# jiamiya/HOPE

Hardware: AMD Instinct MI355X
Metric: parallel env steps/sec (full CarParking step incl. obs + RS search) (higher is better)
Workload: dtype f64

## Files before the change

### hope_amd/_lib.py

```python
import ctypes as C
import os

from .build import lib_path

LIDAR_NUM, N_ACTION, N_ITER, UPSAMPLE, TARGET_DIM, RS_MAX_SEG = 120, 42, 10, 10, 5, 5
F_OBS_F64, F_ACTION_F64, F_PROFILE, F_IMAGE, F_OVERLAP = 0x1, 0x2, 0x4, 0x8, 0x10
STAGE_MOTION, STAGE_OBS, STAGE_REWARD, STAGE_RS, STAGE_ALL = 0x1, 0x2, 0x4, 0x8, 0xF
ACTION_PHYSICAL = 0x10
ACTION_RESCALE_F32 = 0x80
AUTO_REDRAW = 0x100
DEFER_RS = 0x200
STAGE_IMG = 0x40
STAGE_NO_CULL, STAGE_ONE_SCENE = 0x4000, 0x8000
IMG_SIZE, IMG_CHANNELS, TRAJ_RENDER_LEN = 64, 3, 20
AUTO_RESET = 0x20
KERNELS = ('k_kinematics', 'k_env_step', 'k_rs_words', 'k_rs_validate', 'k_bev_image', 'k_bev_prep', 'k_rs_compact', 'k_post', 'k_rs_segs', 'k_rs_screen')
ABI_VERSION = 8

EXPORTS = ['hope_env_create', 'hope_env_destroy', 'hope_last_error', 'hope_abi_version', 'hope_env_upload_tables',
           'hope_env_set_scenes', 'hope_env_step', 'hope_env_wait_rs', 'hope_env_last_step', 'hope_env_wait_rs_step', 'hope_env_download_n_obst', 'hope_env_queue_check', 'hope_env_reset_obs', 'hope_env_download_state',
           'hope_env_upload_state', 'hope_env_restart', 'hope_env_set_pool', 'hope_env_pool_staging', 'hope_env_commit_pool', 'hope_env_commit_pool_relaxed', 'hope_env_pool_staging_ready', 'hope_env_pool_generation', 'hope_env_redraw', 'hope_env_set_redraw_seed', 'hope_env_download_pool_index', 'hope_env_set_dlp_cases', 'hope_env_pool_overflow', 'hope_env_set_draw_class', 'hope_env_download_scenes', 'hope_env_download_pool_state', 'hope_env_restore_maps', 'hope_env_kernel_ms', 'hope_env_kernel_union_ms', 'hope_env_profile_kernels', 'hope_debug_math', 'hope_debug_traffic', 'hope_debug_mask_lut', 'hope_debug_rs_prof', 'hope_debug_rs_log', 'hope_debug_rs_filter_stats', 'hope_debug_rs_filter_dump', 'hope_debug_step_prof', 'hope_debug_census', 'hope_scenegen_generate', 'hope_scenegen_default_threads', 'hope_scenegen_generate_det', 'hope_scenegen_generate_device', 'hope_scenegen_log_det', 'hope_env_generate_pool', 'hope_env_curriculum_enable', 'hope_env_curriculum_disable', 'hope_env_set_pool_buckets', 'hope_env_curriculum_tally', 'hope_env_curriculum_update', 'hope_env_curriculum_state', 'hope_env_curriculum_set_windows', 'hope_env_curriculum_download_lists', 'hope_curriculum_lists_host', 'hope_curriculum_fold_host', 'hope_map_level_host', 'hope_map_level_device', 'hope_env_map_level', 'hope_env_num_scenes', 'hope_env_max_obstacles', 'hope_env_device_arch']


CURRICULUM_LIST_LEN = 1 << 20
BUCKET_UNLABELLED = 255


class HopeError(RuntimeError):
    pass


class StepOut(C.Structure):
    _fields_ = [('lidar', C.c_void_p), ('action_mask', C.c_void_p), ('target', C.c_void_p), ('reward', C.c_void_p),
                ('reward_info', C.c_void_p), ('status', C.c_void_p), ('done', C.c_void_p), ('pose', C.c_void_p),
                ('rs_word', C.c_void_p), ('rs_lengths', C.c_void_p), ('img', C.c_void_p)]


class CurriculumParams(C.Structure):
    _fields_ = [('target', C.c_double * 4), ('type_window', C.c_double), ('case_window', C.c_double), ('type_fail_min', C.c_double),
                ('case_fail_min', C.c_double), ('worst_share', C.c_double), ('case_uniform', C.c_double), ('type_horizon', C.c_int64),
                ('case_horizon', C.c_int64)]

    def __init__(self, target=(0.95, 0.95, 0.9, 0.99), type_window=250.0, case_window=10.0, type_fail_min=0.01, case_fail_min=0.005,
                 worst_share=0.5, case_uniform=0.2, type_horizon=200, case_horizon=500):
        super().__init__((C.c_double * 4)(*target), type_window, case_window, type_fail_min, case_fail_min, worst_share, case_uniform,
                         type_horizon, case_horizon)


_lib = None


def load_library():
    global _lib
    if _lib is not None:
        return _lib
    try:
        import torch
    except ImportError:
        pass
    path = lib_path()
    if not os.path.exists(path):
        raise HopeError(f'{path} is missing: run `python -c "import __graft_entry__ as g; g.build()"` '
                        '(hipcc --offload-arch=gfx950). There is no CPU fallback.')
    L = C.CDLL(path)
    for name in EXPORTS:
        if not hasattr(L, name):
            raise HopeError(f'{path} does not export {name}')
    L.hope_last_error.restype = C.c_char_p
    L.hope_env_device_arch.restype = C.c_char_p
    L.hope_env_device_arch.argtypes = [C.c_void_p]
    L.hope_env_create.argtypes = [C.POINTER(C.c_void_p), C.c_int, C.c_int, C.c_int, C.c_uint32]
    L.hope_env_destroy.argtypes = [C.c_void_p]
    L.hope_env_upload_tables.argtypes = [C.c_void_p, C.c_void_p, C.c_void_p, C.c_void_p]
    L.hope_env_set_scenes.argtypes = [C.c_void_p, C.c_void_p, C.c_int, C.c_void_p, C.c_void_p, C.c_void_p, C.c_void_p,
                                      C.c_void_p]
    L.hope_env_step.argtypes = [C.c_void_p, C.c_void_p, C.c_void_p, C.c_uint32, C.POINTER(StepOut), C.c_void_p]
    L.hope_env_wait_rs.argtypes = [C.c_void_p, C.c_void_p]
    L.hope_env_last_step.argtypes = [C.c_void_p, C.c_void_p]
    L.hope_env_wait_rs_step.argtypes = [C.c_void_p, C.c_uint64, C.c_void_p]
    L.hope_env_download_n_obst.argtypes = [C.c_void_p, C.c_void_p]
    L.hope_env_queue_check.argtypes = [C.c_void_p, C.c_void_p, C.c_void_p, C.c_void_p]
    L.hope_env_reset_obs.argtypes = [C.c_void_p, C.c_void_p, C.c_uint32, C.POINTER(StepOut), C.c_void_p]
    L.hope_env_download_state.argtypes = [C.c_void_p, C.c_void_p, C.c_void_p, C.c_void_p]
    L.hope_env_upload_state.argtypes = [C.c_void_p, C.c_void_p, C.c_void_p, C.c_void_p]
    L.hope_env_restart.argtypes = [C.c_void_p, C.c_void_p, C.c_void_p]
    L.hope_env_set_pool.argtypes = [C.c_void_p, C.c_int, C.c_void_p, C.c_void_p, C.c_void_p, C.c_void_p, C.c_void_p]
    L.hope_env_pool_staging.argtypes = [C.c_void_p, C.c_int] + [C.POINTER(C.c_void_p)] * 5
    L.hope_env_commit_pool.argtypes = [C.c_void_p, C.c_int, C.c_void_p]
    L.hope_env_commit_pool_relaxed.argtypes = [C.c_void_p, C.c_int]
    L.hope_env_redraw.argtypes = [C.c_void_p, C.c_void_p, C.c_uint64, C.c_void_p]
    L.hope_env_set_redraw_seed.argtypes = [C.c_void_p, C.c_uint64]
    L.hope_env_download_pool_index.argtypes = [C.c_void_p, C.c_void_p]
    L.hope_env_set_dlp_cases.argtypes = [C.c_void_p, C.c_int, C.c_void_p, C.c_void_p, C.c_void_p, C.c_void_p, C.c_int, C.c_void_p, C.c_void_p]
    L.hope_env_set_draw_class.argtypes = [C.c_void_p, C.c_void_p, C.c_int, C.c_void_p]
    L.hope_env_pool_overflow.argtypes = [C.c_void_p, C.c_void_p]
    L.hope_env_download_scenes.argtypes = [C.c_void_p, C.c_void_p, C.c_int, C.c_void_p, C.c_void_p, C.c_void_p, C.c_void_p, C.c_void_p]
    L.hope_env_download_pool_state.argtypes = [C.c_void_p, C.c_void_p, C.c_void_p]
    L.hope_env_restore_maps.argtypes = [C.c_void_p, C.c_void_p, C.c_void_p, C.c_uint64, C.c_uint64]
    L.hope_env_pool_staging_ready.argtypes = [C.c_void_p]
    L.hope_env_pool_generation.argtypes = [C.c_void_p, C.c_void_p]
    L.hope_env_kernel_ms.argtypes = [C.c_void_p, C.c_void_p, C.c_void_p, C.c_int]
    L.hope_env_kernel_union_ms.argtypes = [C.c_void_p, C.c_void_p, C.c_void_p, C.c_int]
    L.hope_env_profile_kernels.argtypes = [C.c_void_p, C.c_uint32]
    L.hope_debug_math.argtypes = [C.c_int, C.c_int, C.c_void_p, C.c_void_p, C.c_void_p, C.c_void_p]
    L.hope_debug_traffic.argtypes = [C.c_int, C.c_size_t, C.c_void_p, C.c_void_p]
    L.hope_debug_mask_lut.argtypes = [C.c_void_p, C.c_void_p, C.c_void_p, C.c_void_p]
    L.hope_scenegen_generate.argtypes = [C.c_int, C.c_int, C.c_int, C.c_uint64, C.c_int64, C.c_int, C.c_void_p, C.c_void_p, C.c_void_p,
                                         C.c_void_p, C.c_void_p, C.c_void_p, C.c_int]
    L.hope_scenegen_generate_det.argtypes = L.hope_scenegen_generate.argtypes
    L.hope_scenegen_generate_device.argtypes = [C.c_int, C.c_int, C.c_int, C.c_int, C.c_uint64, C.c_int64, C.c_int, C.c_void_p, C.c_void_p,
                                                C.c_void_p, C.c_void_p, C.c_void_p, C.c_void_p, C.c_void_p]
    L.hope_scenegen_log_det.argtypes = [C.c_int, C.c_void_p, C.c_void_p]
    L.hope_env_generate_pool.argtypes = [C.c_void_p, C.c_int, C.c_void_p, C.c_uint64, C.c_int64, C.c_int]
    L.hope_env_curriculum_enable.argtypes = [C.c_void_p, C.c_void_p]
    L.hope_env_curriculum_disable.argtypes = [C.c_void_p]
    L.hope_env_set_pool_buckets.argtypes = [C.c_void_p, C.c_int, C.c_void_p]
    L.hope_env_curriculum_tally.argtypes = [C.c_void_p, C.c_void_p, C.c_void_p, C.c_void_p]
    L.hope_env_curriculum_update.argtypes = [C.c_void_p, C.c_void_p]
    L.hope_env_curriculum_state.argtypes = [C.c_void_p] + [C.c_void_p] * 8
    L.hope_env_curriculum_set_windows.argtypes = [C.c_void_p, C.c_int] + [C.c_void_p] * 4
    L.hope_env_curriculum_download_lists.argtypes = [C.c_void_p, C.c_void_p, C.c_void_p, C.c_void_p]
    L.hope_curriculum_lists_host.argtypes = [C.c_void_p, C.c_int, C.c_void_p, C.c_void_p, C.c_int, C.c_int] + [C.c_void_p] * 8
    L.hope_curriculum_fold_host.argtypes = [C.c_void_p, C.c_void_p, C.c_double, C.c_double, C.c_double]
    L.hope_map_level_host.argtypes = [C.c_int, C.c_int] + [C.c_void_p] * 6 + [C.c_int]
    L.hope_map_level_device.argtypes = [C.c_int, C.c_int, C.c_int] + [C.c_void_p] * 7
    L.hope_env_map_level.argtypes = [C.c_void_p] * 5
    L.hope_env_num_scenes.argtypes = [C.c_void_p]
    L.hope_env_max_obstacles.argtypes = [C.c_void_p]
    if L.hope_abi_version() != ABI_VERSION:
        raise HopeError(f'ABI mismatch: library {L.hope_abi_version()} vs binding {ABI_VERSION}')
    _lib = L
    return L


def check(rc, what=''):
    if rc != 0:
        msg = load_library().hope_last_error().decode(errors='replace')
        raise HopeError(f'{what} failed (code {rc}): {msg}')
```

### hope_amd/csrc/hope_env.hip

```cpp
#include <hip/hip_runtime.h>
#include <math.h>
#include <stdio.h>
#include <stdlib.h>
#include <string.h>

#include <algorithm>
#include <chrono>
#include <string>
#include <vector>

#include "hope_dev.h"
#include "hope_env.h"
#include "hope_internal.h"
#include "hope_step_kernel.h"
#include "hope_obs_pair.h"
#include "hope_motion_pair.h"
#include "hope_scenegen_kernel.h"
#include "hope_curriculum_kernel.h"
#include "hope_maplevel_kernel.h"

using namespace hope;

static thread_local std::string g_err;
static int fail(int code, const std::string& msg) {
// ... 481 lines not shown
    return HOPE_OK;
}
static int settle_rs(hope_env_t* h) {
    if (!h || !h->rs_pending) return HOPE_OK;
    DeviceGuard guard(h->device);
    HIPCHK(hipEventSynchronize(h->ev_chain1_done));
    HIPCHK(hipEventSynchronize(h->ev_search0_done));
    h->rs_pending = false;
    return HOPE_OK;
}

const char* hope_last_error(void) { return g_err.c_str(); }
int hope_abi_version(void) { return HOPE_ABI_VERSION; }

static int destroy_impl(hope_env_t* h);
static void cur_free(hope_env_t* h);
int hope_env_create(hope_env_t** out, int n_scenes, int max_obstacles, int device_id, uint32_t flags) {
    if (!out || n_scenes <= 0 || max_obstacles <= 0) return fail(HOPE_EINVAL, "hope_env_create: bad argument");
    if (flags & 0x20)
        return fail(HOPE_EINVAL, "hope_env_create: flag 0x20 (hipGraph replay of the step, ABI <= 6) was removed in ABI 7: it was slower than plain launches at every batch size");
    *out = nullptr;
    int ndev = 0;
    hipError_t e = hipGetDeviceCount(&ndev);
    if (e != hipSuccess || ndev <= 0)
        return fail(HOPE_ENODEV, std::string("hope_env_create: no HIP device (") + hipGetErrorString(e) +
                                     "); libhope_env has no CPU fallback");
    if (device_id < 0 || device_id >= ndev) return fail(HOPE_EINVAL, "hope_env_create: device_id out of range");
    HIPCHK(hipSetDevice(device_id));
    hipDeviceProp_t prop;
    HIPCHK(hipGetDeviceProperties(&prop, device_id));
    size_t lds = step_lds_bytes(max_obstacles);
    size_t lds_rs = rs_lds_bytes(max_obstacles);
    if (max_obstacles > HOPE_MAX_OBSTACLES)
        return fail(HOPE_EINVAL, "hope_env_create: max_obstacles " + std::to_string(max_obstacles) + " exceeds HOPE_MAX_OBSTACLES (" +
                                 std::to_string(HOPE_MAX_OBSTACLES) + "): the Reeds-Shepp queue entry carries the obstacle count in 8 bits");
    if (lds > 160 * 1024 || lds_rs > 160 * 1024)
        return fail(HOPE_EINVAL, "hope_env_create: max_obstacles " + std::to_string(max_obstacles) + " does not fit the 160 KiB LDS tile of the step / search kernels");
    if (n_scenes >= RS_LIST_MAX_SCENES)
        return fail(HOPE_EINVAL, "hope_env_create: more than 2^24 - 1 scenes per handle");
    hope_env* h = new (std::nothrow) hope_env();
    if (!h) return fail(HOPE_ENOMEM, "hope_env_create: host allocation failed");
    h->n = n_scenes; h->max_obst = max_obstacles; h->device = device_id; h->flags = flags;
    h->n_obst_host.assign(n_scenes, 0);
    h->slot_cls_host.assign(n_scenes, 0);
    snprintf(h->arch, sizeof(h->arch), "%s", prop.gcnArchName);
    size_t N = (size_t)n_scenes;
#define ALLOC(ptr, bytes)                                                                          \
    do {                                                                                           \
        hipError_t e2 = hipMalloc((void**)&(ptr), (bytes));                                        \
        if (e2 != hipSuccess) {                                                                    \
            destroy_impl(h);                                                                       \
            return fail(HOPE_ENOMEM, std::string("hipMalloc " #ptr ": ") + hipGetErrorString(e2)); \
        }                                                                                          \
    } while (0)
    ALLOC(h->verts, N * max_obstacles * 8 * sizeof(double));
    ALLOC(h->obb, N * max_obstacles * sizeof(float4));
    ALLOC(h->fverts, N * max_obstacles * 2 * sizeof(float4));
    ALLOC(h->fbox, N * max_obstacles * sizeof(float4));
    ALLOC(h->eflag, N * (size_t)eflag_stride(max_obstacles));
    ALLOC(h->n_obst, N * sizeof(int32_t));
    ALLOC(h->scene_c, N * SC_WORDS * sizeof(double));
    ALLOC(h->state, N * ST_WORDS * sizeof(double));
    ALLOC(h->cs, N * 2 * sizeof(double));
    ALLOC(h->tstep, N * sizeof(int32_t));
    ALLOC(h->tab, (size_t)NL * NITER * NACT * sizeof(double));
    ALLOC(h->pmax, NL * sizeof(double));
    ALLOC(h->mask_lut, MASK_LUT_BYTES);
    ALLOC(h->mask_bsc, NBEAM * sizeof(double));
    ALLOC(h->hull_base, NBEAM * sizeof(double));
    ALLOC(h->beam_ab, 2 * NBEAM * sizeof(double));
    ALLOC(h->rs_count, 2 * hope_env::MAX_CHAIN * sizeof(int32_t));
    ALLOC(h->rs_list, 2 * N * sizeof(int32_t));
    ALLOC(h->rs_in, 2 * N * RS_IN_WORDS * sizeof(double));
    ALLOC(h->rs_flag, N);
    ALLOC(h->kin, N * KIN_WORDS * sizeof(double));
    ALLOC(h->post, N * POST_WORDS * sizeof(double));
    ALLOC(h->cls_list[0], N * sizeof(int32_t));
    ALLOC(h->cls_list[1], N * sizeof(int32_t));
    ALLOC(h->rs_rec, N * rs_rec_bytes_per_scene());
    ALLOC(h->rs_surv_count, hope_env::MAX_CHAIN * sizeof(int32_t));
    ALLOC(h->rs_surv, 2 * N * sizeof(int2));
    ALLOC(h->cur_pool, N * sizeof(int32_t));
    ALLOC(h->episode, N * sizeof(uint32_t));
    ALLOC(h->pool_overflow, sizeof(int32_t));
    ALLOC(h->slot_cls, N);
    ALLOC(h->active_snap, N);
    ALLOC(h->cold_dev, hope_env::COLD_RING * sizeof(StepCold));
    if (flags & HOPE_F_IMAGE) {
        ALLOC(h->traj, N * BEV_TRAJ_LEN * 3 * sizeof(double));
        ALLOC(h->traj_len, N * sizeof(int32_t));
        ALLOC(h->traj_valid, N * sizeof(int32_t));
        ALLOC(h->layer_valid, N * sizeof(int32_t));
        ALLOC(h->bev_layer, N * (size_t)BEV_LAYER_ROWS * BEV_LAYER_STRIDE);
        ALLOC(h->bev_dyn, N * BEV_DYN_BYTES);
        ALLOC(h->bev_list, (N + 1) * sizeof(int32_t));
        ALLOC(h->bev_legacy, (N + 1) * sizeof(int32_t));
        ALLOC(h->bev_scratch, N * BEV_SCENE_INTS * sizeof(int));
    }
#undef ALLOC
    if (h->traj) {
        HIPCHK(hipMemset(h->traj, 0, N * BEV_TRAJ_LEN * 3 * sizeof(double)));
        HIPCHK(hipMemset(h->traj_len, 0, N * sizeof(int32_t)));
        HIPCHK(hipMemset(h->traj_valid, 0, N * sizeof(int32_t)));
        HIPCHK(hipMemset(h->layer_valid, 0, N * sizeof(int32_t)));
        HIPCHK(hipMemset(h->bev_dyn, 0, N * BEV_DYN_BYTES));
        HIPCHK(hipMemset(h->bev_list, 0, (N + 1) * sizeof(int32_t)));
        HIPCHK(hipMemset(h->bev_legacy, 0, (N + 1) * sizeof(int32_t)));
        HIPCHK(hipMemset(h->bev_scratch, 0, N * BEV_SCENE_INTS * sizeof(int)));
    }
    HIPCHK(hipMemset(h->n_obst, 0, N * sizeof(int32_t)));
    HIPCHK(hipMemset(h->scene_c, 0, N * SC_WORDS * sizeof(double)));
    HIPCHK(hipMemset(h->state, 0, N * ST_WORDS * sizeof(double)));
    HIPCHK(hipMemset(h->tstep, 0, N * sizeof(int32_t)));
    HIPCHK(hipMemset(h->rs_count, 0, 2 * hope_env::MAX_CHAIN * sizeof(int32_t)));
    HIPCHK(hipMemset(h->rs_flag, 0, N));
    HIPCHK(hipMemset(h->rs_surv_count, 0, hope_env::MAX_CHAIN * sizeof(int32_t)));
    HIPCHK(hipMemset(h->rs_surv, 0, 2 * N * sizeof(int2)));
    HIPCHK(hipMemset(h->rs_in, 0, 2 * N * RS_IN_WORDS * sizeof(double)));
    HIPCHK(hipMemset(h->rs_list, 0, 2 * N * sizeof(int32_t)));
    HIPCHK(hipMemset(h->cur_pool, 0xFF, N * sizeof(int32_t)));
    HIPCHK(hipMemset(h->episode, 0, N * sizeof(uint32_t)));
    HIPCHK(hipMemset(h->pool_overflow, 0, sizeof(int32_t)));
    HIPCHK(hipMemset(h->slot_cls, 0, N));
    HIPCHK(hipMemset(h->active_snap, 1, N));
    HIPCHK(hipHostMalloc((void**)&h->cold_host, hope_env::COLD_RING * sizeof(StepCold)));
    for (int i = 0; i < hope_env::COLD_RING; i++) HIPCHK(hipEventCreateWithFlags(&h->cold_ev[i], hipEventDisableTiming));
    memset(&h->cold_last, 0, sizeof(h->cold_last));
    HIPCHK(rs_init_tables());
    if (lds > 48 * 1024) {
        for (const void* f : {(const void*)k_env_step<float, float>, (const void*)k_env_step<float, float, true>,
                              (const void*)k_env_step<float, double>, (const void*)k_env_step<double, float>,
                              (const void*)k_env_step<double, double>,
                              (const void*)k_env_step<float, float, false, 0, true>, (const void*)k_env_step<float, double, false, 0, true>,
                              (const void*)k_env_step<double, float, false, 0, true>, (const void*)k_env_step<double, double, false, 0, true>,
                              (const void*)k_env_step<float, float, false, 1>, (const void*)k_env_step<float, double, false, 1>,
                              (const void*)k_env_step<double, float, false, 1>, (const void*)k_env_step<double, double, false, 1>,
                              (const void*)k_env_step<float, float, false, 2>, (const void*)k_env_step<float, double, false, 2>,
                              (const void*)k_env_step<double, float, false, 2>, (const void*)k_env_step<double, double, false, 2>})
            HIPCHK(hipFuncSetAttribute(f, hipFuncAttributeMaxDynamicSharedMemorySize, (int)lds));
    }
    if (flags & HOPE_F_OVERLAP) {
        HIPCHK(hipEventCreateWithFlags(&h->ev_fork, hipEventDisableTiming));
        HIPCHK(hipEventCreateWithFlags(&h->ev_collect, hipEventDisableTiming));
        for (int i = 0; i < 2; i++) HIPCHK(hipEventCreateWithFlags(&h->ev_bev[i], hipEventDisableTiming));
        for (int i = 0; i < 2; i++) { HIPCHK(hipEventCreateWithFlags(&h->ev_step[i], hipEventDisableTiming)); HIPCHK(hipEventCreateWithFlags(&h->ev_segs[i], hipEventDisableTiming)); HIPCHK(hipEventCreateWithFlags(&h->ev_post[i], hipEventDisableTiming)); }
        for (hipEvent_t* e : {&h->ev_chain1_done, &h->ev_image_done, &h->ev_obs_done[0], &h->ev_obs_done[1], &h->ev_search0_done})
            HIPCHK(hipEventCreateWithFlags(e, hipEventDisableTiming));
        static const int perm_plain[N_ROLES] = {0, 1, 6, 3, 2, 5, 4, 7}, perm_image[N_ROLES] = {0, 6, 2, 3, 1, 4, 5, 7};
        int perm[N_ROLES];
        for (int r = 0; r < N_ROLES; r++) perm[r] = (flags & HOPE_F_IMAGE) ? perm_image[r] : perm_plain[r];
        hipStream_t created[N_ROLES] = {};
        for (int c = 1; c < N_ROLES; c++) HIPCHK(hipStreamCreateWithPriority(&created[c], hipStreamNonBlocking, 0));
        int cls[N_ROLES];
        for (int c = 0; c < N_ROLES; c++) cls[c] = -1;
        {
            const auto t_begin = std::chrono::steady_clock::now();
            const long long ticks = 10000;
            long long* stamps = nullptr;
            if (hipHostMalloc((void**)&stamps, 4 * sizeof(long long), hipHostMallocDefault) != hipSuccess) stamps = nullptr;
            bool ok = stamps != nullptr;
            auto pair_overlaps = [&](hipStream_t a, hipStream_t b) -> int {
                for (int rep_ = 0; rep_ < 3; rep_++) {
                    hipStreamSynchronize(a); hipStreamSynchronize(b);
                    hipLaunchKernelGGL(k_spin, dim3(1), dim3(64), 0, a, ticks, stamps);
                    hipLaunchKernelGGL(k_spin, dim3(1), dim3(64), 0, b, ticks, stamps + 2);
                    if (hipStreamSynchronize(a) != hipSuccess || hipStreamSynchronize(b) != hipSuccess) return -1;
                    const long long lo = std::max(stamps[0], stamps[2]), hi = std::min(stamps[1], stamps[3]);
                    if (hi - lo > ticks / 4) return 1;
                    if (std::max(stamps[1], stamps[3]) - std::min(stamps[0], stamps[2]) > 20 * ticks) return -1;
                }
                return 0;
            };
            hipLaunchKernelGGL(k_spin, dim3(1), dim3(64), 0, created[1], 100LL, (long long*)nullptr);
            hipStreamSynchronize(created[1]);
            int rep[N_ROLES], n_cls = 0;
            for (int c = 0; c < N_ROLES && ok; c++) {
                int found = -1;
                for (int k = 0; k < n_cls && found < 0 && ok; k++) {
                    const int ov = pair_overlaps(created[rep[k]], created[c]);
                    if (ov < 0) ok = false;
                    else if (ov == 0) found = k;
                }
                if (found < 0) { rep[n_cls] = c; found = n_cls++; }
                cls[c] = found;
            }
            if (stamps) hipHostFree(stamps);
            HIPCHK(hipGetLastError());
            h->queue_check_ms = std::chrono::duration<double, std::milli>(std::chrono::steady_clock::now() - t_begin).count();
            if (!ok) { for (int c = 0; c < N_ROLES; c++) cls[c] = -1; n_cls = 0; }
            h->n_queues = n_cls;
            if (n_cls >= 2 && !(flags & HOPE_F_IMAGE)) {
                static const int order[N_ROLES - 1] = {ROLE_SEARCH0, ROLE_CHAIN, ROLE_OBS_LARGE, ROLE_OBS_SMALL, ROLE_OBS_SUB, ROLE_IMAGE, ROLE_SPARE};
                static const int conflicts[N_ROLES][4] = {
                     {-1, -1, -1, -1},
                     {ROLE_CALLER, ROLE_SEARCH0, -1, -1},
                     {-1, -1, -1, -1},
                     {ROLE_CALLER, ROLE_SEARCH0, ROLE_CHAIN, -1},
                     {ROLE_CALLER, ROLE_CHAIN, ROLE_OBS_LARGE, -1},
                     {ROLE_CALLER, -1, -1, -1},
                     {-1, -1, -1, -1},
                     {ROLE_SEARCH0, ROLE_CHAIN, ROLE_OBS_LARGE, -1}};
                int newperm[N_ROLES] = {0, 0, 0, 0, 0, 0, 0, 0};
                bool taken[N_ROLES] = {};
                for (const int r : order) {
                    int best = -1, best_cost = 1 << 30;
                    for (int c = 1; c < N_ROLES; c++) {
                        if (taken[c]) continue;
                        int cost = 0;
                        for (const int o : conflicts[r]) {
                            if (o < 0) continue;
                            const int oc = o == ROLE_CALLER ? cls[0] : (newperm[o] ? cls[newperm[o]] : -2);
                            if (oc == cls[c]) cost += 4;
                        }
                        if (c != perm[r]) cost += 1;
                        if (cost < best_cost) { best_cost = cost; best = c; }
                    }
                    newperm[r] = best; taken[best] = true;
                }
                for (int r = 1; r < N_ROLES; r++) perm[r] = newperm[r];
            }
        }
        for (int r = 1; r < N_ROLES; r++) h->side[r] = created[perm[r]];
        h->queue_of_role[ROLE_CALLER] = cls[0];
        for (int r = 1; r < N_ROLES; r++) h->queue_of_role[r] = cls[perm[r]];
    }
    HIPCHK(hipDeviceSynchronize());
    { std::lock_guard<std::mutex> lk(g_live_m); g_live.insert(h); }
    *out = h;
    return HOPE_OK;
}

int hope_env_destroy(hope_env_t* h) {
    if (!h) return HOPE_OK;
    {
        std::lock_guard<std::mutex> lk(g_live_m);
        if (g_live.erase(h) == 0) return fail(HOPE_EINVAL, "hope_env_destroy: not a live handle (destroyed twice?)");
    }
    return destroy_impl(h);
}
static int destroy_impl(hope_env_t* h) {
    settle_rs(h);
    DeviceGuard guard(h->device);
    drain_events(h);
    hipDeviceSynchronize();
    for (hipEvent_t e : {h->ev_collect, h->ev_bev[0], h->ev_bev[1], h->ev_fork, h->ev_step[0], h->ev_step[1], h->ev_segs[0], h->ev_segs[1], h->ev_post[0], h->ev_post[1],
                         h->ev_chain1_done, h->ev_image_done, h->ev_obs_done[0], h->ev_obs_done[1], h->ev_search0_done}) if (e) hipEventDestroy(e);
    for (hipStream_t q : h->side) if (q) hipStreamDestroy(q);
    if (h->pool_stream) hipStreamDestroy(h->pool_stream);
    for (hipEvent_t e : h->cold_ev) if (e) hipEventDestroy(e);
    if (h->cold_host) hipHostFree(h->cold_host);
    for (hipEvent_t e : {h->ev_pool_ready, h->ev_pool_copied, h->ev_last_step}) if (e) hipEventDestroy(e);
    for (void* q : {(void*)h->pstage.start, (void*)h->pstage.dest, (void*)h->pstage.bbox, (void*)h->pstage.verts, (void*)h->pstage.nobst, (void*)h->pstage.list}) if (q) hipHostFree(q);
    for (int i = 0; i < 2; i++) { if (h->gen_nobst[i]) hipHostFree(h->gen_nobst[i]); if (h->ev_gen_copied[i]) hipEventDestroy(h->ev_gen_copied[i]); }
    for (hipEvent_t e : h->free_events) hipEventDestroy(e);
    cur_free(h);
    for (auto& ps : h->pset) for (void* q : {(void*)ps.label, (void*)ps.sorted_own[0], (void*)ps.sorted_own[1]}) if (q) hipFree(q);
    void* ptrs[] = {h->obb, h->fverts, h->fbox, h->eflag, h->verts, h->n_obst, h->scene_c, h->state, h->cs, h->tstep, h->tab, h->pmax, h->mask_lut, h->mask_bsc,
                    h->hull_base, h->beam_ab, h->rs_count, h->rs_surv_count, h->rs_surv, h->rs_list, h->rs_in, h->rs_flag, h->kin, h->post, h->cls_list[0], h->cls_list[1], h->rs_rec, h->cur_pool, h->episode, h->pset[0].verts, h->pset[0].c, h->pset[0].nobst, h->pset[0].list[0], h->pset[0].list[1], h->pset[1].verts, h->pset[1].c, h->pset[1].nobst, h->pset[1].list[0], h->pset[1].list[1], h->pstage_dev, h->pool_overflow, h->slot_cls, h->active_snap, h->cold_dev, h->dlp_mem[0], h->dlp_mem[1], h->dlp_mem[2], h->dlp_mem[3], h->dlp_mem[4], h->dlp_mem[5], h->stage, h->traj, h->traj_len, h->traj_valid, h->layer_valid, h->bev_layer, h->bev_dyn, h->bev_list, h->bev_legacy, h->bev_scratch};
    for (void* q : ptrs)
        if (q) hipFree(q);
    delete h;
    return HOPE_OK;
}

int hope_debug_step_prof(uint64_t* out, int reset) {
    static unsigned long long buf[64 * 16];
    hipError_t e = hipDeviceSynchronize();
    if (e == hipSuccess) e = hipMemcpyFromSymbol(buf, HIP_SYMBOL(g_step_prof), sizeof(buf));
    for (int i = 0; i < 16; i++) { out[i] = 0; for (int sh = 0; sh < 64; sh++) out[i] += buf[sh * 16 + i]; }
    if (e == hipSuccess && reset) {
        for (auto& v : buf) v = 0;
        e = hipMemcpyToSymbol(HIP_SYMBOL(g_step_prof), buf, sizeof(buf));
    }
    return e == hipSuccess ? HOPE_OK : fail(HOPE_EHIP, std::string("hope_debug_step_prof: ") + hipGetErrorString(e));
}

int hope_debug_census(uint64_t* out, int reset) {
    static unsigned long long buf[64 * 16];
    if (!out) return fail(HOPE_EINVAL, "hope_debug_census: null argument");
    hipError_t e = hipDeviceSynchronize();
    if (e == hipSuccess) e = hipMemcpyFromSymbol(buf, HIP_SYMBOL(g_census), sizeof(buf));
    for (int i = 0; i < 16; i++) {
        const bool is_min = i == 1 || i == 3 || i == 7;
        out[i] = is_min ? ~0ull : 0;
        for (int sh = 0; sh < 64; sh++) out[i] = is_min ? std::min<uint64_t>(out[i], buf[sh * 16 + i]) : out[i] + buf[sh * 16 + i];
    }
    if (e == hipSuccess && reset) {
        for (int sh = 0; sh < 64; sh++) for (int i = 0; i < 16; i++) buf[sh * 16 + i] = (i == 1 || i == 3 || i == 7) ? 0x7ff0000000000000ull : 0;
        e = hipMemcpyToSymbol(HIP_SYMBOL(g_census), buf, sizeof(buf));
    }
    return e == hipSuccess ? HOPE_OK : fail(HOPE_EHIP, std::string("hope_debug_census: ") + hipGetErrorString(e));
}

int hope_debug_rs_prof(uint64_t* out, int reset) {
    hipError_t e = rs_prof_read((unsigned long long*)out, reset);
    return e == hipSuccess ? HOPE_OK : fail(HOPE_EHIP, std::string("hope_debug_rs_prof: ") + hipGetErrorString(e));
}

int hope_debug_rs_filter_stats(uint64_t* out, int reset) {
    if (!out) return fail(HOPE_EINVAL, "hope_debug_rs_filter_stats: null argument");
    hipError_t e = rs_fstat_read((unsigned long long*)out, reset);
    return e == hipSuccess ? HOPE_OK : fail(HOPE_EHIP, std::string("hope_debug_rs_filter_stats: ") + hipGetErrorString(e));
}

int hope_debug_rs_filter_dump(double* out) {
    if (!out) return fail(HOPE_EINVAL, "hope_debug_rs_filter_dump: null argument");
    hipError_t e = rs_fdump_read(out);
    return e == hipSuccess ? HOPE_OK : fail(HOPE_EHIP, std::string("hope_debug_rs_filter_dump: ") + hipGetErrorString(e));
}

int hope_debug_rs_log(int32_t* out, int cap, int32_t* n, int reset) {
    if (!out || !n || cap < 0) return fail(HOPE_EINVAL, "hope_debug_rs_log: bad argument");
    hipError_t e = rs_log_read(out, cap, n, reset);
    return e == hipSuccess ? HOPE_OK : fail(HOPE_EHIP, std::string("hope_debug_rs_log: ") + hipGetErrorString(e));
}

int hope_env_queue_check(hope_env_t* h, int32_t* queue_of_role, int32_t* n_queues, double* ms) {
    if (!h) return fail(HOPE_EINVAL, "hope_env_queue_check: null handle");
    if (queue_of_role) for (int r = 0; r < N_ROLES; r++) queue_of_role[r] = h->queue_of_role[r];
    if (n_queues) *n_queues = h->n_queues;
    if (ms) *ms = h->queue_check_ms;
    return HOPE_OK;
}

int hope_env_num_scenes(const hope_env_t* h) { return h ? h->n : HOPE_EINVAL; }
int hope_env_max_obstacles(const hope_env_t* h) { return h ? h->max_obst : HOPE_EINVAL; }
const char* hope_env_device_arch(const hope_env_t* h) { return h ? h->arch : ""; }

static void build_mask_lut(const std::vector<double>& tab, const std::vector<double>& pmax, const double* hull_base,
                           std::vector<uint16_t>& lut, std::vector<double>& bsc) {
    lut.assign((size_t)MASK_LUT_ROWS * MASK_LUT_ROW, (uint16_t)0xAAAA);
    bsc.assign(NBEAM, 0.0);
    for (int i = 0; i < NBEAM; i++) {
        const int l = UPS * i;
        const double lo = hull_base[i] - 1e-6;
        const double scale = (double)MASK_LUT_NB / (pmax[l] + 4e-9 - lo);
        bsc[i] = scale;
        for (int b = 0; b < MASK_LUT_NB; b++) {
            const double e_lo = lo + ((double)b - 1e-6) / scale - 2e-9, e_hi = lo + ((double)b + 1.0 + 1e-6) / scale + 2e-9;
            uint16_t* row = lut.data() + ((size_t)i * MASK_LUT_NB + b) * MASK_LUT_ROW;
            for (int hl = 0; hl < NACT / 2; hl++) {
                int c[2][2];
                for (int d = 0; d < 2; d++) {
                    const int a = hl + d * (NACT / 2);
                    int cl = 0, ch = 0;
                    for (int k = 0; k < NITER; k++) {
                        const double t = tab[((size_t)l * NITER + k) * NACT + a];
                        cl += t <= e_lo; ch += t <= e_hi;
                    }
                    c[d][0] = cl; c[d][1] = ch;
                }
                row[hl] = (uint16_t)(c[0][0] | c[0][1] << 4 | c[1][0] << 8 | c[1][1] << 12);
            }
        }
    }
}

static void build_mask_tab(const double* dist_star, std::vector<double>& tab, std::vector<double>& pmax) {
    tab.assign((size_t)NL * NITER * NACT, 0.0);
    pmax.assign(NL, 0.0);
    for (int l = 0; l < NL; l++) {
        double pm = -INFINITY;
        for (int a = 0; a < NACT; a++) {
            double run = -INFINITY;
            for (int k = 0; k < NITER; k++) {
                double v = dist_star[((size_t)l * NACT + a) * NITER + k];
                run = v > run ? v : run;
                tab[((size_t)l * NITER + k) * NACT + a] = run;
            }
            pm = run > pm ? run : pm;
        }
        pmax[l] = pm;
    }
}

int hope_debug_mask_lut(const double* dist_star, const double* hull_base, uint16_t* lut_out, double* scale_out) {
    if (!dist_star || !hull_base || !lut_out || !scale_out) return fail(HOPE_EINVAL, "hope_debug_mask_lut: null argument");
    std::vector<double> tab, pmax, bsc;
    std::vector<uint16_t> lut;
    build_mask_tab(dist_star, tab, pmax);
    build_mask_lut(tab, pmax, hull_base, lut, bsc);
    memcpy(lut_out, lut.data(), MASK_LUT_BYTES);
    memcpy(scale_out, bsc.data(), NBEAM * sizeof(double));
    return HOPE_OK;
}

int hope_env_upload_tables(hope_env_t* h, const double* dist_star, const double* hull_base, const double* beam_ab) {
    if (!h || !dist_star || !hull_base || !beam_ab) return fail(HOPE_EINVAL, "hope_env_upload_tables: null argument");
    DeviceGuard guard(h->device);
    if (!guard.ok) return fail(HOPE_EHIP, "hipSetDevice failed");
    std::vector<double> tab, pmax;
    build_mask_tab(dist_star, tab, pmax);
    HIPCHK(hipMemcpy(h->tab, tab.data(), tab.size() * sizeof(double), hipMemcpyHostToDevice));
    HIPCHK(hipMemcpy(h->pmax, pmax.data(), pmax.size() * sizeof(double), hipMemcpyHostToDevice));
    {
        std::vector<uint16_t> lut;
        std::vector<double> bsc;
        build_mask_lut(tab, pmax, hull_base, lut, bsc);
        HIPCHK(hipMemcpy(h->mask_lut, lut.data(), MASK_LUT_BYTES, hipMemcpyHostToDevice));
        HIPCHK(hipMemcpy(h->mask_bsc, bsc.data(), NBEAM * sizeof(double), hipMemcpyHostToDevice));
    }
    HIPCHK(hipMemcpy(h->hull_base, hull_base, NBEAM * sizeof(double), hipMemcpyHostToDevice));
    HIPCHK(hipMemcpy(h->beam_ab, beam_ab, 2 * NBEAM * sizeof(double), hipMemcpyHostToDevice));
    h->have_tables = true;
    return HOPE_OK;
}

static int upload_scenes(hope_env_t* h, const int32_t* ids, int n, const double* start, const double* dest, const double* bbox,
                         const double* verts, const int32_t* n_obst, double* d_scene_c, double* d_state, int32_t* d_t,
                         int32_t* d_nobst, double* d_verts, float4* d_obb, double* d_traj, int32_t* d_traj_len, int32_t* d_traj_valid,
                         int32_t* d_layer_valid);
static int apply_pending_pool(hope_env_t* h, bool wait);
static int cur_on_swap(hope_env_t* h);

static int rebuild_class_lists(hope_env_t* h) {
    std::vector<int32_t> l0, l1;
    l0.reserve(h->n); l1.reserve(h->n);
    const bool two = h->max_obst > SMALL_TILE;
    for (int i = 0; i < h->n; i++) (two && h->slot_cls_host[i] ? l1 : l0).push_back(i);
    if (two && (h->flags & HOPE_F_OVERLAP)) {
        const char* fr = getenv("HOPE_CLS1_FRAC");
        const double frac = fr ? atof(fr) : (h->n < 32768 ? 0.42 : 0.0);
        const size_t want1 = (size_t)(frac * h->n);
        if (l1.size() < want1) {
            const size_t move = std::min(l0.size(), want1 - l1.size());
            l1.insert(l1.end(), l0.end() - move, l0.end());
            l0.resize(l0.size() - move);
            std::sort(l1.begin(), l1.end());
        }
    }
    h->cls_count[0] = (int)l0.size(); h->cls_count[1] = (int)l1.size();
    if (!l0.empty()) HIPCHK(hipMemcpy(h->cls_list[0], l0.data(), l0.size() * sizeof(int32_t), hipMemcpyHostToDevice));
    if (!l1.empty()) HIPCHK(hipMemcpy(h->cls_list[1], l1.data(), l1.size() * sizeof(int32_t), hipMemcpyHostToDevice));
    HIPCHK(hipMemcpy(h->slot_cls, h->slot_cls_host.data(), (size_t)h->n, hipMemcpyHostToDevice));
    return HOPE_OK;
}

int hope_env_set_scenes(hope_env_t* h, const int32_t* scene_ids, int n, const double* start, const double* dest,
                        const double* bbox, const double* verts, const int32_t* n_obst) {
    { int rcs = settle_rs(h); if (rcs != HOPE_OK) return rcs; }
    if (!h || n < 0 || (n > 0 && (!scene_ids || !start || !dest || !bbox || !n_obst)))
        return fail(HOPE_EINVAL, "hope_env_set_scenes: null argument");
    if (n == 0) return HOPE_OK;
    for (int k = 0; k < n; k++) {
        if (scene_ids[k] < 0 || scene_ids[k] >= h->n) return fail(HOPE_EINVAL, "hope_env_set_scenes: scene id out of range");
        if (n_obst[k] < 0 || n_obst[k] > h->max_obst) return fail(HOPE_EINVAL, "hope_env_set_scenes: n_obst exceeds max_obstacles");
        if (n_obst[k] > 0 && !verts) return fail(HOPE_EINVAL, "hope_env_set_scenes: verts is null");
    }
    DeviceGuard guard(h->device);
    if (!guard.ok) return fail(HOPE_EHIP, "hipSetDevice failed");
    {
        int rc = upload_scenes(h, scene_ids, n, start, dest, bbox, verts, n_obst, h->scene_c, h->state, h->tstep, h->n_obst,
                               h->verts, h->obb, h->traj, h->traj_len, h->traj_valid, h->layer_valid);
        if (rc != HOPE_OK) return rc;
    }
    for (int k = 0; k < n; k++) {
        h->n_obst_host[scene_ids[k]] = n_obst[k];
        h->slot_cls_host[scene_ids[k]] = (h->max_obst > SMALL_TILE && n_obst[k] > SMALL_TILE) ? 1 : 0;
    }
    { int rc = rebuild_class_lists(h); if (rc != HOPE_OK) return rc; }
    if (h->cur.on) {
        hipLaunchKernelGGL(k_curriculum_forget, dim3((n + 255) / 256), dim3(256), 0, 0, n, (const int32_t*)h->stage, h->cur.scene_bucket,
                           h->episode, h->cur.noted_ep);
        HIPCHK(hipGetLastError());
    }
    HIPCHK(hipDeviceSynchronize());
    h->have_scenes = true;
    return HOPE_OK;
}

static void draw_lists(const hope_env_t* h, const int32_t** lists, int* counts) {
    for (int c = 0; c < 2; c++) {
        const bool weighted = h->cur.on && h->cur.wactive >= 0 && h->pool_cls_n[c] > 0;
        lists[c] = weighted ? h->cur.wl[h->cur.wactive][c] : h->pool_cls[c];
        counts[c] = weighted ? CW_LIST_LEN : h->pool_cls_n[c];
    }
}
static int sync_cold(hope_env_t* h, hipStream_t s) {
    StepCold c;
    memset(&c, 0, sizeof(c));
    c.traj = h->traj; c.traj_len = h->traj_len; c.traj_valid = h->traj_valid; c.layer_valid = h->layer_valid;
    c.pool_verts = h->pool_verts; c.pool_c = h->pool_c; c.pool_nobst = h->pool_nobst;
    draw_lists(h, c.pool_cls, c.pool_cls_n);
    c.cur_pool = h->cur_pool; c.episode = h->episode; c.redraw_seed = h->redraw_seed;
    c.dlp = h->dlp; c.pool_overflow = h->pool_overflow; c.slot_cls = h->slot_cls;
    c.fverts = h->fverts; c.fbox = h->fbox; c.eflag = h->eflag;
    if (h->cold_idx >= 0 && memcmp(&c, &h->cold_last, sizeof(c)) == 0) return HOPE_OK;
    const int slot = (h->cold_idx + 1) % hope_env::COLD_RING;
    HIPCHK(hipEventSynchronize(h->cold_ev[slot]));
    memcpy(&h->cold_host[slot], &c, sizeof(c));
    HIPCHK(hipMemcpyAsync(h->cold_dev + slot, h->cold_host + slot, sizeof(c), hipMemcpyHostToDevice, s));
    HIPCHK(hipEventRecord(h->cold_ev[slot], s));
    h->cold_idx = slot;
    memcpy(&h->cold_last, &c, sizeof(c));
    return HOPE_OK;
}

constexpr int SPLIT_MIN_SCENES = 16384;
constexpr int SPLIT_MIN_SCENES_DEFER = 32768;
constexpr int FUSE_KIN_MAX_SCENES = 4096;
constexpr int AUTO_SUBS_RANGE[4] = {32768, 1 << 30, 4096, 32768};

enum MotionKernel { MOTION_ONE_LAUNCH, MOTION_FUSED_KIN, MOTION_TIMING, MOTION_SPLIT, MOTION_PAIR };
enum ObsKernel { OBS_IN_STEP, OBS_SPLIT, OBS_PAIR };

struct StepPlan {
    struct Chain {
        int c, a, b;
        int tile_cap;
        Role search, kin, obs;
        bool on_caller;
        bool post_on_search;
        MotionKernel motion;
        ObsKernel obs_kernel;
    } chain[hope_env::MAX_CHAIN];
    int n_chain;
    bool want_rs;
    bool fork;
    bool split;
    bool pipe;
    bool pipe1;
    bool fuse_kin;
    bool auto_subs;
};

static StepPlan plan_step(const hope_env_t* h, uint32_t stages, bool want_rs, bool overlap, int has_action, bool step_timing) {
    StepPlan pl = {};
    pl.want_rs = want_rs;
    const int n_cls = h->max_obst > SMALL_TILE ? 2 : 1;
    const bool obs = stages & HOPE_STAGE_OBS, defer_rs = stages & HOPE_DEFER_RS, img = stages & HOPE_STAGE_IMG;
    int subs = 1;
    if (overlap && want_rs && obs && defer_rs && !img && (h->cls_count[0] == 0) != (h->cls_count[1] == 0)) {
        int range[4] = {AUTO_SUBS_RANGE[0], AUTO_SUBS_RANGE[1], AUTO_SUBS_RANGE[2], AUTO_SUBS_RANGE[3]};
        if (const char* e = getenv("HOPE_AUTO_CHAINS")) sscanf(e, "%d:%d:%d:%d", range, range + 1, range + 2, range + 3);
        const int c1 = h->cls_count[0] == 0 ? 1 : 0, cnt = h->cls_count[c1];
        if (cnt >= range[2 * c1] && cnt <= range[2 * c1 + 1]) { subs = 2; pl.auto_subs = true; }
    }
    for (int c = n_cls - 1; c >= 0; c--)
        for (int j = 0; j < subs; j++) {
            const int a = (int)((long long)h->cls_count[c] * j / subs), b = (int)((long long)h->cls_count[c] * (j + 1) / subs);
            if (b > a) {
                StepPlan::Chain& ch = pl.chain[pl.n_chain++];
                ch.c = c; ch.a = a; ch.b = b;
                ch.tile_cap = (c == 0 && n_cls == 2) ? SMALL_TILE : h->max_obst;
            }
        }
    pl.fork = overlap && pl.n_chain == 2;
    const bool two_stream_forms = pl.fork && want_rs && obs && !step_timing;
    const char* split_min = getenv("HOPE_SPLIT_MIN");
    pl.split = two_stream_forms && h->n >= (split_min ? atoi(split_min) : defer_rs ? SPLIT_MIN_SCENES_DEFER : SPLIT_MIN_SCENES);
    pl.pipe = two_stream_forms && defer_rs;
    pl.pipe1 = pl.pipe && !pl.split;
    pl.fuse_kin = h->n <= FUSE_KIN_MAX_SCENES && !pl.split && !step_timing;
    const bool of64 = h->flags & HOPE_F_OBS_F64, af64 = h->flags & HOPE_F_ACTION_F64;
    for (int i = 0; i < pl.n_chain; i++) {
        StepPlan::Chain& ch = pl.chain[i];
        ch.search = (pl.fork && i == 1) ? ROLE_CHAIN : pl.pipe ? ROLE_SEARCH0 : ROLE_CALLER;
        ch.on_caller = pl.pipe && !pl.auto_subs && !img && h->cls_count[ch.c] >= h->cls_count[1 - ch.c];
        ch.obs = !(pl.split || pl.pipe1) ? ch.search : ch.on_caller ? ROLE_CALLER : (pl.auto_subs && i == 1) ? ROLE_OBS_SUB : (Role)(ROLE_OBS_LARGE + i);
        ch.kin = pl.pipe ? ch.obs : ch.search;
        ch.post_on_search = pl.pipe && pl.split;
        const bool one_scene = stages & STAGE_ONE_SCENE;
        if (pl.split) ch.motion = (ch.c == 0 && n_cls == 2 && (stages & HOPE_STAGE_MOTION) && has_action && !one_scene) ? MOTION_PAIR : MOTION_SPLIT;
        else if (step_timing && !of64 && !af64) ch.motion = MOTION_TIMING;
        else ch.motion = pl.fuse_kin ? MOTION_FUSED_KIN : MOTION_ONE_LAUNCH;
        ch.obs_kernel = !pl.split ? OBS_IN_STEP : (ch.tile_cap == SMALL_TILE && !one_scene) ? OBS_PAIR : OBS_SPLIT;
    }
    return pl;
}

static int enqueue_step(hope_env_t* h, const void* actions, const uint8_t* active, uint32_t stages, const hope_step_out* out,
                        hipStream_t s, bool overlap, int has_action, LaunchTimer* tm) {
    StepParams p;
    memset(&p, 0, sizeof(p));
    p.n = h->n; p.max_obst = h->max_obst; p.stages = stages; p.has_action = has_action;
    p.hflags = h->traj ? STEP_HF_TRAJ : 0;
    p.verts = h->verts; p.obb = h->obb; p.eflag = h->eflag; p.n_obst = h->n_obst; p.scene_c = h->scene_c; p.state = h->state; p.cs = h->cs; p.tstep = h->tstep;
    p.active = active; p.active_out = active ? h->active_snap : nullptr; p.kin = h->kin; p.actions = actions; p.post = h->post;
    p.tab = h->tab; p.pmax = h->pmax; p.mask_lut = h->mask_lut; p.mask_bsc = h->mask_bsc; p.hull_base = h->hull_base; p.beam_ab = h->beam_ab;
    p.lidar = out->lidar; p.action_mask = out->action_mask;
    p.cold = h->cold_dev + h->cold_idx;
    const uint8_t* active_rs = active ? h->active_snap : nullptr;
    const bool of64 = h->flags & HOPE_F_OBS_F64, af64 = h->flags & HOPE_F_ACTION_F64;
    const dim3 block(WAVE);
    static const bool step_timing = getenv("HOPE_STEP_TIMING") != nullptr;
    const bool want_rs = (stages & HOPE_STAGE_RS) && out->rs_word;
    const StepPlan pl = plan_step(h, stages, want_rs, overlap, has_action, step_timing);
    auto stream = [&](Role r) { return r == ROLE_CALLER ? s : h->side[r]; };

    if (!pl.pipe) { int rcj = join_rs(h, s); if (rcj != HOPE_OK) return rcj; }
    if (want_rs) h->rs_parity ^= 1;
    if (pl.fork) {
        HIPCHK(hipEventRecord(h->ev_fork, s));
        HIPCHK(hipStreamWaitEvent(h->side[ROLE_CHAIN], h->ev_fork, 0));
        if (pl.pipe) HIPCHK(hipStreamWaitEvent(h->side[ROLE_SEARCH0], h->ev_fork, 0));
    }
    h->last_via_steps = false;
    for (int i = 0; i < pl.n_chain; i++) {
        const StepPlan::Chain& ch = pl.chain[i];
        const int c = ch.c;
        const hipStream_t sc = stream(ch.search), sk = stream(ch.kin), so = stream(ch.obs);
        int32_t* counter = h->rs_count + i + hope_env::MAX_CHAIN * h->rs_parity;
        if (pl.pipe && !ch.on_caller) HIPCHK(hipStreamWaitEvent(sk, h->ev_fork, 0));
        p.tile_cap = ch.tile_cap;
        p.scene_list = h->cls_list[c] + ch.a;
        p.n_list = ch.b - ch.a;
        p.rs_count_zero = want_rs ? counter : nullptr;
        if ((stages & HOPE_STAGE_MOTION) && has_action && !pl.fuse_kin) {
            dim3 kg((p.n_list + KIN_SCENES_PER_BLOCK - 1) / KIN_SCENES_PER_BLOCK);
            if (tm) tm->begin(HOPE_K_KINEMATICS, sk);
            if (af64) hipLaunchKernelGGL((k_kinematics<double>), kg, block, 0, sk, p.n_list, p.scene_list, h->state, actions, active, stages, h->scene_c, h->kin);
            else hipLaunchKernelGGL((k_kinematics<float>), kg, block, 0, sk, p.n_list, p.scene_list, h->state, actions, active, stages, h->scene_c, h->kin);
            if (tm) tm->end(sk);
        }
        const dim3 grid(p.n_list);
        const size_t lds = step_lds_bytes(p.tile_cap);
        if (pl.pipe) HIPCHK(hipStreamWaitEvent(sk, h->ev_segs[i], 0));
        if (tm) tm->begin(HOPE_K_STEP, sk);
        switch (ch.motion) {
        case MOTION_PAIR: hipLaunchKernelGGL(k_motion_pair, dim3((p.n_list + 1) / 2), block, MP_LDS_BYTES, sk, p); break;
        case MOTION_SPLIT: launch_env_step<1>(of64, af64, grid, block, lds, sk, p); break;
        case MOTION_TIMING: hipLaunchKernelGGL((k_env_step<float, float, true>), grid, block, lds, sk, p); break;
        case MOTION_FUSED_KIN: launch_env_step<0, true>(of64, af64, grid, block, lds, sk, p); break;
        case MOTION_ONE_LAUNCH: launch_env_step<0>(of64, af64, grid, block, lds, sk, p); break;
        }
        if (tm) tm->end(sk);
        if (pl.fork && (pl.split || pl.pipe || (stages & HOPE_STAGE_IMG))) { HIPCHK(hipEventRecord(h->ev_step[i], sk)); h->last_via_steps = true; }
        if (pl.split && !pl.pipe) HIPCHK(hipStreamWaitEvent(so, h->ev_step[i], 0));
        auto launch_post = [&](hipStream_t sp) {
            dim3 pg((p.n_list + WAVE - 1) / WAVE);
            if (tm) tm->begin(HOPE_K_POST, sp);
            if (of64) hipLaunchKernelGGL((k_post<double>), pg, block, 0, sp, p.n_list, p.scene_list, active, stages, h->scene_c, h->state, h->post, h->rs_flag, *out);
            else hipLaunchKernelGGL((k_post<float>), pg, block, 0, sp, p.n_list, p.scene_list, active, stages, h->scene_c, h->state, h->post, h->rs_flag, *out);
            if (tm) tm->end(sp);
        };
        if (!pl.split) launch_post(so);
        else {
            if (tm) tm->begin(HOPE_K_STEP, so);
            if (ch.obs_kernel == OBS_PAIR) {
                if (of64) hipLaunchKernelGGL((k_obs_pair<double>), dim3((p.n_list + 1) / 2), block, OP_LDS_BYTES, so, p);
                else hipLaunchKernelGGL((k_obs_pair<float>), dim3((p.n_list + 1) / 2), block, OP_LDS_BYTES, so, p);
            } else launch_env_step<2>(of64, af64, grid, block, lds, so, p);
            if (tm) tm->end(so);
            if (!ch.post_on_search) launch_post(so);
        }
        if ((pl.split || pl.pipe1) && !ch.on_caller) HIPCHK(hipEventRecord(h->ev_obs_done[i], so));
        if (!want_rs) continue;
        if (pl.pipe) HIPCHK(hipStreamWaitEvent(sc, h->ev_step[i], 0));
        if (ch.post_on_search) {
            launch_post(sc);
            HIPCHK(hipEventRecord(h->ev_post[i], sc));
        }
        int32_t* qlist = h->rs_list + (size_t)c * h->n + ch.a;
        double* rs_in = h->rs_in + ((size_t)c * h->n + ch.a) * RS_IN_WORDS;
        if (tm) tm->begin(HOPE_K_RS_COMPACT, sc);
        {
            const dim3 cg((p.n_list + COMPACT_THREADS - 1) / COMPACT_THREADS);
            if (of64) hipLaunchKernelGGL(k_rs_compact<double>, cg, dim3(COMPACT_THREADS), 0, sc, p.scene_list, p.n_list, h->rs_flag, active_rs, qlist,
                                         counter, (const double*)h->post, (const double*)h->scene_c, out->rs_word, out->rs_lengths, (const int32_t*)h->n_obst, h->rs_surv_count + i, rs_in);
            else hipLaunchKernelGGL(k_rs_compact<float>, cg, dim3(COMPACT_THREADS), 0, sc, p.scene_list, p.n_list, h->rs_flag, active_rs, qlist,
                                    counter, (const double*)h->post, (const double*)h->scene_c, out->rs_word, out->rs_lengths, (const int32_t*)h->n_obst, h->rs_surv_count + i, rs_in);
        }
        if (tm) tm->end(sc);
        if (pl.pipe) HIPCHK(hipEventRecord(h->ev_segs[i], sc));
        RsParams r;
        r.n = h->n; r.max_obst = h->max_obst; r.obs_f64 = of64;
        r.prio_front = 0;
        r.tile_cap = p.tile_cap;
        r.max_queue = p.n_list;
        r.slot_base = (c == 0) ? ch.a : h->n - 1 - ch.a;
        r.slot_dir = (c == 0) ? 1 : -1;
        r.verts = h->verts; r.obb = h->obb; r.n_obst = h->n_obst; r.scene_c = h->scene_c; r.state = h->state;
        r.fverts = h->fverts; r.fbox = h->fbox; r.eflag = h->eflag;
        r.rs_count = counter; r.rs_list = qlist; r.rs_in = rs_in;
        r.rs_rec = h->rs_rec;
        r.surv_count = h->rs_surv_count + i;
        r.surv_list = h->rs_surv + (size_t)c * h->n + ch.a;
        r.rs_word = out->rs_word; r.rs_lengths = out->rs_lengths;
        HIPCHK(launch_rs_search(r, sc, tm));
    }
    HIPCHK(hipGetLastError());
    if (stages & HOPE_STAGE_IMG) {
        BevParams b;
        b.n = h->n; b.max_obst = h->max_obst; b.verts = h->verts; b.n_obst = h->n_obst; b.scene_c = h->scene_c;
        b.state = h->state; b.traj = h->traj; b.traj_len = h->traj_len; b.traj_valid = h->traj_valid; b.scratch = h->bev_scratch; b.img = out->img;
        b.layer = h->bev_layer; b.layer_valid = h->layer_valid; b.rebuild = h->bev_list; b.dyn = h->bev_dyn;
        b.legacy_list = h->bev_legacy;
        b.active = active;
        b.debug = 0;
        if (const char* e_ = getenv("HOPE_BEV_DEBUG")) b.debug |= atoi(e_);
        if (getenv("HOPE_BEV_LEGACY")) b.debug |= 32;
        if (pl.fork) {
            const hipStream_t si = pl.pipe ? s : h->side[ROLE_IMAGE];
            HIPCHK(hipStreamWaitEvent(si, h->ev_step[0], 0));
            HIPCHK(hipStreamWaitEvent(si, h->ev_step[1], 0));
            if (pl.pipe) HIPCHK(launch_bev_image(b, si, tm, h->side[ROLE_IMAGE], h->ev_bev[0], h->ev_bev[1]));
            else HIPCHK(launch_bev_image(b, si, tm));
            HIPCHK(hipEventRecord(h->ev_image_done, si));
        } else HIPCHK(launch_bev_image(b, s, tm));
    }
    if (!pl.fork) return HOPE_OK;
    HIPCHK(hipEventRecord(h->ev_chain1_done, h->side[ROLE_CHAIN]));
    if (pl.pipe) {
        HIPCHK(hipEventRecord(h->ev_search0_done, h->side[ROLE_SEARCH0]));
        h->rs_pending = true;
    } else HIPCHK(hipStreamWaitEvent(s, h->ev_chain1_done, 0));
    if (stages & HOPE_STAGE_IMG) HIPCHK(hipStreamWaitEvent(s, h->ev_image_done, 0));
    if (pl.split || pl.pipe1) {
        const StepPlan::Chain* ch = pl.chain;
        if (ch[0].on_caller != ch[1].on_caller) {
            const hipStream_t so = stream(ch[ch[0].on_caller ? 1 : 0].obs);
            for (int i = 0; i < 2; i++) if (ch[i].post_on_search) HIPCHK(hipStreamWaitEvent(so, h->ev_post[i], 0));
            HIPCHK(hipEventRecord(h->ev_collect, so));
            HIPCHK(hipStreamWaitEvent(s, h->ev_collect, 0));
        } else for (int i = 0; i < 2; i++) {
            if (!ch[i].on_caller) HIPCHK(hipStreamWaitEvent(s, h->ev_obs_done[i], 0));
            if (ch[i].post_on_search) HIPCHK(hipStreamWaitEvent(s, h->ev_post[i], 0));
        }
    }
    return HOPE_OK;
}

static int check_pool_classes(hope_env_t* h, const char* who) {
    bool resident[2] = {false, false};
    for (int i = 0; i < h->n; i++) resident[h->slot_cls_host[i] ? 1 : 0] = true;
    for (int c = 0; c < 2; c++)
        if (resident[c] && h->pool_cls_n[c] == 0)
            return fail(HOPE_ESTATE, std::string(who) + ": scene slots of the " + (c ? "large" : "small (<= 32 obstacles)") +
                                     " size class are resident but the pool holds no map of that size class (a slot draws from its own class: "
                                     "hope_env_set_pool / hope_env_set_dlp_cases / hope_env_set_draw_class)");
    return HOPE_OK;
}

static int launch_step(hope_env_t* h, const void* actions, const uint8_t* active, uint32_t stages,
                       const hope_step_out* out, void* stream, int has_action) {
    if (!h || !out) return fail(HOPE_EINVAL, "hope_env_step: null argument");
    if (!is_live(h)) return fail(HOPE_EINVAL, "hope_env_step: not a live handle (destroyed?)");
    if (!h->have_tables) return fail(HOPE_ESTATE, "hope_env_step: hope_env_upload_tables has not been called");
    if (!h->have_scenes) return fail(HOPE_ESTATE, "hope_env_step: hope_env_set_scenes has not been called");
    if (has_action && !actions) return fail(HOPE_EINVAL, "hope_env_step: actions is null");
    if (stages & HOPE_STAGE_RS) stages |= HOPE_STAGE_REWARD;
    if (stages & HOPE_AUTO_REDRAW) {
        if (!(stages & HOPE_AUTO_RESET)) return fail(HOPE_EINVAL, "hope_env_step: HOPE_AUTO_REDRAW needs HOPE_AUTO_RESET");
        if (h->pool_n <= 0 && h->dlp.n_cases <= 0) return fail(HOPE_ESTATE, "hope_env_step: HOPE_AUTO_REDRAW without a scene pool (hope_env_set_pool / hope_env_set_dlp_cases)");
        int rc0 = check_pool_classes(h, "hope_env_step");
        if (rc0 != HOPE_OK) return rc0;
    }
    if (stages & HOPE_STAGE_IMG) {
        if (!h->traj) return fail(HOPE_ESTATE, "hope_env_step: HOPE_STAGE_IMG needs a handle created with HOPE_F_IMAGE");
        if (!out->img) return fail(HOPE_EINVAL, "hope_env_step: HOPE_STAGE_IMG without out->img");
    }
    DeviceGuard guard(h->device);
    if (!guard.ok) return fail(HOPE_EHIP, "hipSetDevice failed");
    hipStream_t s = (hipStream_t)stream;
    const bool prof = h->flags & HOPE_F_PROFILE;
    h->step_seq++;
    { int rcp = apply_pending_pool(h, false); if (rcp != HOPE_OK) return rcp; }
    if (h->pool_wait_pending) {
        HIPCHK(hipStreamWaitEvent(s, h->ev_pool_ready, 0));
        h->pool_wait_pending = false;
    }
    { int rcc = sync_cold(h, s); if (rcc != HOPE_OK) return rcc; }
    h->draw_set = h->pactive;
    struct LastStep {
        hope_env_t* h; hipStream_t s;
        ~LastStep() { if (h->pactive >= 0 && h->ev_last_step && !h->last_via_steps) hipEventRecord(h->ev_last_step, s); }
    } last_step{h, s};
    if (prof && h->pending.size() > 4096) { int rc = drain_events(h); if (rc) return rc; }
    EventTimer timer(h);
    LaunchTimer* tm = prof ? &timer : nullptr;
    int rc = enqueue_step(h, actions, active, stages, out, s, (h->flags & HOPE_F_OVERLAP) != 0, has_action, tm);
    if (rc != HOPE_OK) return rc;
    if (timer.failed) return fail(HOPE_EHIP, "hipEventRecord failed");
    return HOPE_OK;
}


static int upload_scenes(hope_env_t* h, const int32_t* ids, int n, const double* start, const double* dest, const double* bbox,
                         const double* verts, const int32_t* n_obst, double* d_scene_c, double* d_state, int32_t* d_t,
                         int32_t* d_nobst, double* d_verts, float4* d_obb, double* d_traj, int32_t* d_traj_len, int32_t* d_traj_valid,
                         int32_t* d_layer_valid) {
    size_t tile = (size_t)h->max_obst * 8 * sizeof(double);
    size_t o_ids = 0, o_nob = o_ids + sizeof(int32_t) * n, o_start = (o_nob + sizeof(int32_t) * n + 15) & ~(size_t)15;
    size_t o_dest = o_start + 24 * (size_t)n, o_bbox = o_dest + 24 * (size_t)n, o_verts = (o_bbox + 32 * (size_t)n + 15) & ~(size_t)15;
    size_t need = o_verts + tile * n;
    if (need > h->stage_bytes) {
        if (h->stage) hipFree(h->stage);
        h->stage = nullptr; h->stage_bytes = 0;
        hipError_t e2 = hipMalloc(&h->stage, need);
        if (e2 != hipSuccess) return fail(HOPE_ENOMEM, std::string("hipMalloc stage: ") + hipGetErrorString(e2));
        h->stage_bytes = need;
    }
    char* sp = (char*)h->stage;
    HIPCHK(hipMemcpy(sp + o_ids, ids, sizeof(int32_t) * n, hipMemcpyHostToDevice));
    HIPCHK(hipMemcpy(sp + o_nob, n_obst, sizeof(int32_t) * n, hipMemcpyHostToDevice));
    HIPCHK(hipMemcpy(sp + o_start, start, 24 * (size_t)n, hipMemcpyHostToDevice));
    HIPCHK(hipMemcpy(sp + o_dest, dest, 24 * (size_t)n, hipMemcpyHostToDevice));
    HIPCHK(hipMemcpy(sp + o_bbox, bbox, 32 * (size_t)n, hipMemcpyHostToDevice));
    if (verts) HIPCHK(hipMemcpy(sp + o_verts, verts, tile * n, hipMemcpyHostToDevice));
    hipLaunchKernelGGL(k_set_scene_consts, dim3((n + 127) / 128), dim3(128), 0, 0, n, (const int32_t*)(sp + o_ids),
                       (const double*)(sp + o_start), (const double*)(sp + o_dest), (const double*)(sp + o_bbox),
                       (const int32_t*)(sp + o_nob), d_scene_c, d_state, d_t, d_nobst, d_traj, d_traj_len, d_traj_valid, d_layer_valid);
    if (verts)
        hipLaunchKernelGGL(k_set_scene_tiles, dim3(n), dim3(128), 0, 0, (const int32_t*)(sp + o_ids),
                           (const int32_t*)(sp + o_nob), (const double*)(sp + o_verts), (const double*)(sp + o_bbox), d_verts, d_obb,
                           h->fverts, h->fbox, h->eflag, h->max_obst);
    HIPCHK(hipGetLastError());
    HIPCHK(hipDeviceSynchronize());
    return HOPE_OK;
}

static uint64_t hmix64(uint64_t z) {
    z += 0x9E3779B97F4A7C15ull;
    z = (z ^ (z >> 30)) * 0xBF58476D1CE4E5B9ull;
    z = (z ^ (z >> 27)) * 0x94D049BB133111EBull;
    return z ^ (z >> 31);
}
static uint64_t fold64(uint64_t a, uint64_t b) { return hmix64(a ^ hmix64(b + 0x9E3779B97F4A7C15ull)); }
static uint64_t hash_bytes(uint64_t hsh, const void* p, size_t bytes) {
    const unsigned char* q = (const unsigned char*)p;
    size_t i = 0;
    for (; i + 8 <= bytes; i += 8) { uint64_t w; memcpy(&w, q + i, 8); hsh = (hsh ^ w) * 0x100000001B3ull; hsh ^= hsh >> 29; }
    uint64_t w = 0;
    if (i < bytes) { memcpy(&w, q + i, bytes - i); hsh = (hsh ^ w) * 0x100000001B3ull; }
    return fold64(hsh, bytes);
}
static void bump_pool_generation(hope_env_t* h, uint64_t content) {
    h->pool_generation = fold64(h->pool_generation, content);
    if (h->pool_generation == 0) h->pool_generation = 1;
}

static int pool_init_streams(hope_env_t* h) {
    if (h->pool_stream) return HOPE_OK;
    HIPCHK(hipStreamCreateWithFlags(&h->pool_stream, hipStreamNonBlocking));
    HIPCHK(hipEventCreateWithFlags(&h->ev_pool_ready, hipEventDisableTiming));
    HIPCHK(hipEventCreateWithFlags(&h->ev_pool_copied, hipEventDisableTiming));
    HIPCHK(hipEventCreateWithFlags(&h->ev_last_step, hipEventDisableTiming));
    return HOPE_OK;
}

static void build_pool_lists(hope_env_t* h, const int32_t* n_obst, int n_pool, std::vector<int32_t>& l0, std::vector<int32_t>& l1) {
    const bool two = h->max_obst > SMALL_TILE;
    for (int k = 0; k < n_pool; k++) (two && n_obst[k] > SMALL_TILE ? l1 : l0).push_back(k);
    for (int c = 0; c < h->dlp.n_cases; c++) (two ? l1 : l0).push_back(-2 - c);
}

static int pool_set_reserve(hope_env_t* h, hope_env::PoolSet& ps, int n_pool, int n_list) {
    if (n_pool > ps.cap) {
        for (void* q : {(void*)ps.verts, (void*)ps.c, (void*)ps.nobst, (void*)ps.label}) if (q) hipFree(q);
        ps.verts = ps.c = nullptr; ps.nobst = nullptr; ps.label = nullptr; ps.cap = 0;
        const size_t P = (size_t)n_pool;
        hipError_t e_ = hipMalloc((void**)&ps.verts, P * h->max_obst * 8 * sizeof(double));
        if (e_ == hipSuccess) e_ = hipMalloc((void**)&ps.c, P * SC_WORDS * sizeof(double));
        if (e_ == hipSuccess) e_ = hipMalloc((void**)&ps.nobst, P * sizeof(int32_t));
        if (e_ == hipSuccess) e_ = hipMalloc((void**)&ps.label, P);
        if (e_ != hipSuccess) return fail(HOPE_ENOMEM, std::string("hipMalloc pool: ") + hipGetErrorString(e_));
        ps.cap = n_pool;
    }
    if (n_list > ps.list_cap) {
        for (int c = 0; c < 2; c++) { if (ps.list[c]) hipFree(ps.list[c]); ps.list[c] = nullptr; }
        for (int c = 0; c < 2; c++) {
            hipError_t e_ = hipMalloc((void**)&ps.list[c], (size_t)n_list * sizeof(int32_t));
            if (e_ != hipSuccess) return fail(HOPE_ENOMEM, std::string("hipMalloc pool lists: ") + hipGetErrorString(e_));
        }
        ps.list_cap = n_list;
    }
    return HOPE_OK;
}

int hope_env_pool_staging(hope_env_t* h, int n_pool, double** start, double** dest, double** bbox, double** verts, int32_t** n_obst) {
    if (!h || n_pool <= 0 || !start || !dest || !bbox || !verts || !n_obst) return fail(HOPE_EINVAL, "hope_env_pool_staging: bad argument");
    DeviceGuard guard(h->device);
    if (!guard.ok) return fail(HOPE_EHIP, "hipSetDevice failed");
    int rc = pool_init_streams(h);
    if (rc != HOPE_OK) return rc;
    if (h->pstage.busy) { HIPCHK(hipEventSynchronize(h->ev_pool_copied)); h->pstage.busy = false; }
    if (n_pool > h->pstage.cap) {
        for (void* q : {(void*)h->pstage.start, (void*)h->pstage.dest, (void*)h->pstage.bbox, (void*)h->pstage.verts, (void*)h->pstage.nobst, (void*)h->pstage.list})
            if (q) hipHostFree(q);
        h->pstage = hope_env::PoolStage{};
        const size_t P = (size_t)n_pool;
        hipError_t e_ = hipHostMalloc((void**)&h->pstage.start, P * 24);
        if (e_ == hipSuccess) e_ = hipHostMalloc((void**)&h->pstage.dest, P * 24);
        if (e_ == hipSuccess) e_ = hipHostMalloc((void**)&h->pstage.bbox, P * 32);
        if (e_ == hipSuccess) e_ = hipHostMalloc((void**)&h->pstage.verts, P * h->max_obst * 8 * sizeof(double));
        if (e_ == hipSuccess) e_ = hipHostMalloc((void**)&h->pstage.nobst, P * sizeof(int32_t));
        if (e_ == hipSuccess) e_ = hipHostMalloc((void**)&h->pstage.list, (P + 4096) * sizeof(int32_t));
        if (e_ != hipSuccess) return fail(HOPE_ENOMEM, std::string("hipHostMalloc pool staging: ") + hipGetErrorString(e_));
        h->pstage.cap = n_pool;
    }
    h->pstage.staged = true;
    *start = h->pstage.start; *dest = h->pstage.dest; *bbox = h->pstage.bbox; *verts = h->pstage.verts; *n_obst = h->pstage.nobst;
    return HOPE_OK;
}

int hope_env_pool_staging_ready(hope_env_t* h) {
    if (!h) return fail(HOPE_EINVAL, "hope_env_pool_staging_ready: null handle");
    if (!h->pstage.busy) return 1;
    DeviceGuard guard(h->device);
    if (!guard.ok) return fail(HOPE_EHIP, "hipSetDevice failed");
    const hipError_t e = hipEventQuery(h->ev_pool_copied);
    if (e == hipSuccess) { h->pstage.busy = false; return 1; }
    if (e == hipErrorNotReady) return 0;
    return fail(HOPE_EHIP, std::string("hipEventQuery: ") + hipGetErrorString(e));
}

static int effective_generation(hope_env_t* h, uint64_t* generation);
int hope_env_pool_generation(hope_env_t* h, uint64_t* generation) {
    if (!h || !generation) return fail(HOPE_EINVAL, "hope_env_pool_generation: null argument");
    { DeviceGuard guard(h->device); int rcp = apply_pending_pool(h, true); if (rcp != HOPE_OK) return rcp; }
    return effective_generation(h, generation);
}

static int settle_gen_nobst(hope_env_t* h) {
    const int g = h->gen_host_set;
    if (g < 0) return HOPE_OK;
    HIPCHK(hipEventSynchronize(h->ev_gen_copied[g]));
    h->pool_nobst_host.assign(h->gen_nobst[g], h->gen_nobst[g] + h->gen_nobst_n[g]);
    h->gen_host_set = -1;
    return HOPE_OK;
}

static int apply_pending_pool(hope_env_t* h, bool wait) {
    if (!h->pend.on) return HOPE_OK;
    if (wait) HIPCHK(hipEventSynchronize(h->ev_pool_ready));
    else {
        const hipError_t e = hipEventQuery(h->ev_pool_ready);
        if (e == hipErrorNotReady) return HOPE_OK;
        if (e != hipSuccess) return fail(HOPE_EHIP, std::string("hipEventQuery: ") + hipGetErrorString(e));
    }
    hope_env::PoolSet& ps = h->pset[h->pend.set];
    h->pool_verts = ps.verts; h->pool_c = ps.c; h->pool_nobst = ps.nobst;
    h->pool_cls[0] = ps.list[0]; h->pool_cls[1] = ps.list[1];
    h->pool_cls_n[0] = h->pend.cls_n[0]; h->pool_cls_n[1] = h->pend.cls_n[1];
    h->pool_n = h->pend.n_pool;
    h->pool_nobst_host.swap(h->pend.nobst_host);
    h->pactive = h->pend.set;
    h->pend.on = false;
    bump_pool_generation(h, h->pend.content);
    h->gen_host_set = h->pend.generated ? h->pend.set : -1;
    return cur_on_swap(h);
}

static int commit_pool_impl(hope_env_t* h, int n_pool, bool relaxed);
int hope_env_commit_pool(hope_env_t* h, int n_pool, void* stream) { (void)stream; return commit_pool_impl(h, n_pool, false); }
int hope_env_commit_pool_relaxed(hope_env_t* h, int n_pool) { return commit_pool_impl(h, n_pool, true); }

static int commit_pool_impl(hope_env_t* h, int n_pool, bool relaxed) {
    if (!h || n_pool <= 0) return fail(HOPE_EINVAL, "hope_env_commit_pool: bad argument");
    if (n_pool > h->pstage.cap) return fail(HOPE_ESTATE, "hope_env_commit_pool: more entries than hope_env_pool_staging provided");
    for (int k = 0; k < n_pool; k++)
        if (h->pstage.nobst[k] < 0 || h->pstage.nobst[k] > h->max_obst) return fail(HOPE_EINVAL, "hope_env_commit_pool: n_obst exceeds max_obstacles");
    DeviceGuard guard(h->device);
    if (!guard.ok) return fail(HOPE_EHIP, "hipSetDevice failed");
    std::vector<int32_t> l0, l1;
    build_pool_lists(h, h->pstage.nobst, n_pool, l0, l1);
    if ((int)(l0.size() + l1.size()) > h->pstage.cap + 4096) return fail(HOPE_EINVAL, "hope_env_commit_pool: too many Dragon-Lake cases for the list staging");
    { int rcp = apply_pending_pool(h, true); if (rcp != HOPE_OK) return rcp; }
    const int t = h->pactive < 0 ? 0 : 1 - h->pactive;
    hope_env::PoolSet& ps = h->pset[t];
    if (h->pstage.busy) { HIPCHK(hipEventSynchronize(h->ev_pool_copied)); h->pstage.busy = false; }
    int rc = pool_set_reserve(h, ps, n_pool, (int)std::max(l0.size(), l1.size()) + 1);
    if (rc != HOPE_OK) return rc;
    if (3 * 32 * n_pool / 8 > h->pstage_dev_cap) {
        if (h->pstage_dev) hipFree(h->pstage_dev);
        h->pstage_dev = nullptr; h->pstage_dev_cap = 0;
        hipError_t e_ = hipMalloc((void**)&h->pstage_dev, (size_t)n_pool * 80);
        if (e_ != hipSuccess) return fail(HOPE_ENOMEM, std::string("hipMalloc pool staging: ") + hipGetErrorString(e_));
        h->pstage_dev_cap = 12 * n_pool;
    }
    hipStream_t us = h->pool_stream;
    if (h->pactive >= 0) {
        HIPCHK(hipStreamWaitEvent(us, h->ev_last_step, 0));
        if (h->last_via_steps) for (int i = 0; i < 2; i++) HIPCHK(hipStreamWaitEvent(us, h->ev_step[i], 0));
    }
    const size_t P = (size_t)n_pool;
    char* dv = (char*)h->pstage_dev;
    {
// ... 930 lines not shown
```

### hope_amd/csrc/hope_internal.h

```cpp
#pragma once
#include <hip/hip_runtime.h>
#include <stdint.h>
#include "hope_env.h"

namespace hope {

constexpr uint32_t STAGE_NO_BEAMS = 0x1000;
constexpr uint32_t STAGE_NO_MASK = 0x2000;
constexpr uint32_t STAGE_NO_CULL = 0x4000;
constexpr uint32_t STAGE_ONE_SCENE = 0x8000;

struct RsWord {
    double len[5];
    double Lm;
    int code;
    int n;
    double pad;
};
constexpr int RS_WORDS_PER_SCENE = 48;
constexpr int RS_LIST_MAX_SCENES = 1 << 24;
__host__ __device__ inline int rs_list_pack(int scene, int n_obst) { return (int)(((unsigned)scene << 8) | (unsigned)n_obst); }
__host__ __device__ inline int rs_list_scene(int entry) { return (int)((unsigned)entry >> 8); }
__host__ __device__ inline int rs_list_n_obst(int entry) { return (int)((unsigned)entry & 0xFFu); }
constexpr int RS_IN_WORDS = 14;
constexpr double RS_MAXC = 0.3327130214085973;
constexpr int RS_REC_HDR = 16;
constexpr int RS_REC_ORDER = 10;
constexpr int RS_REC_KEYS = RS_REC_HDR;
constexpr int RS_REC_WORDS = RS_REC_KEYS + RS_WORDS_PER_SCENE;
constexpr int RS_REC_SEGS = RS_REC_WORDS + 8 * RS_WORDS_PER_SCENE;
constexpr int RS_SEGW = 8, RS_SEG_F32 = 5 * RS_SEGW, RS_SEG_TABLE = RS_SEG_F32 + 5 * 2;
constexpr int RS_REC_DOUBLES = RS_REC_SEGS + RS_SEG_TABLE * RS_WORDS_PER_SCENE;

struct RsParams {
    int n, max_obst;
    int tile_cap;
    int max_queue;
    int slot_base, slot_dir;
    int obs_f64;
    int prio_front;
    const float4* obb;
    const float4* fverts;
    const float4* fbox;
    const uint8_t* eflag;
    const double* verts;
    const int32_t* n_obst;
    const double* scene_c;
    const double* state;
    const double* rs_in;
    const int32_t* rs_count;
    const int32_t* rs_list;
    double* rs_rec;
    int8_t* rs_word;
    void* rs_lengths;
    int32_t* surv_count;
    int2* surv_list;
};

constexpr int BEV_IMG = HOPE_IMG_SIZE;
constexpr int BEV_TRAJ_LEN = HOPE_TRAJ_RENDER_LEN;
constexpr int BEV_LAYER_ROWS = 512, BEV_LAYER_STRIDE = 128;
constexpr int BEV_DYN_DIM = 256;
constexpr size_t BEV_DYN_BYTES = (size_t)BEV_DYN_DIM * BEV_DYN_DIM;
constexpr int BEV_SCENE_INTS = 16 + (3 + BEV_TRAJ_LEN) * 16 + (2 + BEV_TRAJ_LEN) * 64;
struct BevParams {
    int n, max_obst;
    const double* verts;
    const int32_t* n_obst;
    const double* scene_c;
    const double* state;
    const double* traj;
    const int32_t* traj_len;
    int32_t* traj_valid;
    uint8_t* layer;
    uint8_t* dyn;
    int32_t* layer_valid;
    int32_t* legacy_list;
    int32_t* rebuild;
    int* scratch;
    const uint8_t* active;
    uint8_t* img;
    int debug;
};

struct LaunchTimer {
    virtual void begin(int kind, hipStream_t s) = 0;
    virtual void end(hipStream_t s) = 0;
};
hipError_t launch_rs_search(const RsParams& p, hipStream_t stream, LaunchTimer* timer);
hipError_t rs_prof_read(unsigned long long* out , int reset);
hipError_t rs_init_tables();
hipError_t rs_fstat_read(unsigned long long* out , int reset);
hipError_t rs_fdump_read(double* out );
hipError_t rs_log_read(int* out , int cap, int* n, int reset);
size_t rs_lds_bytes(int max_obst);
size_t rs_screen_lds_bytes(int max_obst);
size_t rs_rec_bytes_per_scene();
hipError_t launch_bev_image(const BevParams& p, hipStream_t stream, LaunchTimer* timer, hipStream_t side = nullptr, hipEvent_t ev_fork = nullptr,
                            hipEvent_t ev_join = nullptr);
size_t bev_lds_bytes(bool legacy);

}
```

### hope_amd/csrc/hope_rs.hip

```cpp
#include <stdlib.h>

#include "hope_dev.h"
#include "hope_internal.h"

namespace hope {

namespace {

constexpr double MAXC = RS_MAXC;
constexpr double RS_STEP = 0.1;
constexpr double MAX_LENGTH = 1000.0;
constexpr int NCAND = 46;

enum { TS = 0, TL = 1, TR = 2 };

__device__ __forceinline__ double py_mod(double v, double w) {
    double m = hm_fmod(v, w);
    if (m != 0) { if ((w < 0) != (m < 0)) m += w; } else m = copysign(0.0, w);
    return m;
}
__device__ __forceinline__ double rs_M(double theta) {
    double phi = py_mod(theta, 2.0 * PI);
    if (phi < -PI) phi += 2.0 * PI;
    if (phi > PI) phi -= 2.0 * PI;
// ... 98 lines not shown
        double tt = theta, uu = 2.0 - rho, vv = rs_M(tt + 0.5 * PI - phi);
        if (tt >= 0.0 && uu <= 0.0 && vv <= 0.0) { t = tt; u = uu; v = vv; return true; }
    }
    return false;
}
__device__ __forceinline__ bool rs_LRSL(double x, double y, double phi, double sphi, double cphi, double& t, double& u, double& v) {
    double xi = x - sphi, eta = y - 1.0 + cphi, rho, theta;
    rs_R(xi, eta, rho, theta);
    if (rho >= 2.0) {
        double r = sqrt(rho * rho - 4.0);
        double uu = 2.0 - r;
        double tt = rs_M(theta + hm_atan2(r, -2.0));
        double vv = rs_M(phi - 0.5 * PI - tt);
        if (tt >= 0.0 && uu <= 0.0 && vv <= 0.0) { t = tt; u = uu; v = vv; return true; }
    }
    return false;
}
__device__ __forceinline__ bool rs_LRSLR(double x, double y, double phi, double sphi, double cphi, double& t, double& u, double& v) {
    double xi = x + sphi, eta = y - 1.0 - cphi, rho, theta;
    rs_R(xi, eta, rho, theta);
    if (rho >= 2.0) {
        double uu = 4.0 - sqrt(rho * rho - 4.0);
        if (uu <= 0.0) {
            double tt = rs_M(hm_atan2((4.0 - uu) * xi - 2.0 * eta, -2.0 * xi + (uu - 4.0) * eta));
            double vv = rs_M(tt - phi);
            if (tt >= 0.0 && vv >= 0.0) { t = tt; u = uu; v = vv; return true; }
        }
    }
    return false;
}

__device__ __forceinline__ void cand_decode(int c, int& g, int& q) {
    if (c < 2) { g = 0; q = c * 2; }
    else { g = 1 + (c - 2) / 4; q = (c - 2) & 3; }
}
__device__ __forceinline__ int pack_types(int a, int b, int c, int d, int e, int n) {
    return a | (b << 2) | (c << 4) | (d << 6) | (e << 8) | (n << 12);
}
__device__ __forceinline__ int mirror_type(int t) { return t == TL ? TR : (t == TR ? TL : t); }
__device__ __forceinline__ int type_of(int code, int i) { return (code >> (2 * i)) & 3; }

__device__ __forceinline__ void interpolate(double l, int m, double ox, double oy, double oyaw, double c_noy,
                                            double s_noy, double c_oy, double s_oy, double& px, double& py,
                                            double& pyaw) {
    if (m == TS) {
        px = ox + l / MAXC * c_oy;
        py = oy + l / MAXC * s_oy;
        pyaw = oyaw;
    } else {
        double sl, cl;
        hm_sincos(l, &sl, &cl);
        double ldx = sl / MAXC;
        double ldy = (m == TL) ? (1.0 - cl) / MAXC : (1.0 - cl) / (-MAXC);
        double gdx = c_noy * ldx + s_noy * ldy;
        double gdy = -s_noy * ldx + c_noy * ldy;
        px = ox + gdx;
        py = oy + gdy;
        pyaw = (m == TL) ? oyaw + l : oyaw - l;
    }
}

template <int CTRL>
__device__ __forceinline__ float dpp_f(float v) {
    return __int_as_float(__builtin_amdgcn_mov_dpp(__float_as_int(v), CTRL, 0xf, 0xf, true));
}
__device__ __forceinline__ float wave_min_f(float v) {
    v = fminf(v, dpp_f<0xB1>(v));
    v = fminf(v, dpp_f<0x4E>(v));
    v = fminf(v, dpp_f<0x141>(v));
    v = fminf(v, dpp_f<0x140>(v));
    const int i = __float_as_int(v);
    return fminf(fminf(__int_as_float(__builtin_amdgcn_readlane(i, 0)), __int_as_float(__builtin_amdgcn_readlane(i, 16))),
                 fminf(__int_as_float(__builtin_amdgcn_readlane(i, 32)), __int_as_float(__builtin_amdgcn_readlane(i, 48))));
}
__device__ __forceinline__ float wave_max_f(float v) {
    v = fmaxf(v, dpp_f<0xB1>(v));
    v = fmaxf(v, dpp_f<0x4E>(v));
    v = fmaxf(v, dpp_f<0x141>(v));
    v = fmaxf(v, dpp_f<0x140>(v));
    const int i = __float_as_int(v);
    return fmaxf(fmaxf(__int_as_float(__builtin_amdgcn_readlane(i, 0)), __int_as_float(__builtin_amdgcn_readlane(i, 16))),
                 fmaxf(__int_as_float(__builtin_amdgcn_readlane(i, 32)), __int_as_float(__builtin_amdgcn_readlane(i, 48))));
}

__device__ __forceinline__ double wave_min_d(double v) {
    v = fmin(v, __hiloint2double(__builtin_amdgcn_mov_dpp(__double2hiint(v), 0xB1, 0xf, 0xf, true), __builtin_amdgcn_mov_dpp(__double2loint(v), 0xB1, 0xf, 0xf, true)));
    v = fmin(v, __hiloint2double(__builtin_amdgcn_mov_dpp(__double2hiint(v), 0x4E, 0xf, 0xf, true), __builtin_amdgcn_mov_dpp(__double2loint(v), 0x4E, 0xf, 0xf, true)));
    v = fmin(v, __hiloint2double(__builtin_amdgcn_mov_dpp(__double2hiint(v), 0x141, 0xf, 0xf, true), __builtin_amdgcn_mov_dpp(__double2loint(v), 0x141, 0xf, 0xf, true)));
    v = fmin(v, __hiloint2double(__builtin_amdgcn_mov_dpp(__double2hiint(v), 0x140, 0xf, 0xf, true), __builtin_amdgcn_mov_dpp(__double2loint(v), 0x140, 0xf, 0xf, true)));
    return fmin(fmin(readlane_d(v, 0), readlane_d(v, 16)), fmin(readlane_d(v, 32), readlane_d(v, 48)));
}

__device__ unsigned long long g_rs_prof[64 * 16];
constexpr int RS_LOG_CAP = 1 << 21;
__device__ int g_rs_log_n;
__device__ int4 g_rs_log[RS_LOG_CAP];
#define RS_T0() unsigned long long t0_ = TIMING ? __builtin_readcyclecounter() : 0
#define RS_T(i) do { if (TIMING) { const unsigned long long t1_ = __builtin_readcyclecounter(); tsec[i] += t1_ - t0_; t0_ = t1_; } } while (0)

template <bool TIMING, bool FULL = false>
__device__ __forceinline__ bool pose_hits(bool active, double wx, double wy, double wyaw, const double* tile,
                                          const float4* obb, int* cand, int n_obst, double xmin, double xmax,
                                          double ymin, double ymax, int lane, unsigned long long* tsec) {
    RS_T0();
    bool bad = false;
    double vx[4], vy[4];
    double hminx = INFINITY, hmaxx = -INFINITY, hminy = INFINITY, hmaxy = -INFINITY;
    if (active) {
        if (wx < xmin || wx > xmax || wy < ymin || wy > ymax) bad = true;
        double st, ct;
        hm_sincos(wyaw, &st, &ct);
#pragma unroll
        for (int k = 0; k < 4; k++) {
            vx[k] = ct * car_x(k) - st * car_y(k) + wx;
            vy[k] = st * car_x(k) + ct * car_y(k) + wy;
        }
        hminx = fmin(fmin(vx[0], vx[1]), fmin(vx[2], vx[3]));
        hmaxx = fmax(fmax(vx[0], vx[1]), fmax(vx[2], vx[3]));
        hminy = fmin(fmin(vy[0], vy[1]), fmin(vy[2], vy[3]));
        hmaxy = fmax(fmax(vy[0], vy[1]), fmax(vy[2], vy[3]));
    }
    if (!FULL && __any(bad)) return bad;
    float ulox = active ? __double2float_rd(hminx) : INFINITY, uhix = active ? __double2float_ru(hmaxx) : -INFINITY;
    float uloy = active ? __double2float_rd(hminy) : INFINITY, uhiy = active ? __double2float_ru(hmaxy) : -INFINITY;
    ulox = wave_min_f(ulox); uhix = wave_max_f(uhix); uloy = wave_min_f(uloy); uhiy = wave_max_f(uhiy);
    int nc = 0;
    for (int base = 0; base < n_obst; base += WAVE) {
        int o = base + lane;
        bool near = false;
        if (o < n_obst) {
            const float4 bb = obb[o];
            near = !(bb.x > uhix || bb.y < ulox || bb.z > uhiy || bb.w < uloy);
        }
        unsigned long long m = __ballot(near);
        if (near) cand[nc + __popcll(m & ((1ull << lane) - 1))] = o;
        nc += __popcll(m);
    }
    RS_T(4);
    if (nc == 0) return bad;
    if (TIMING) { tsec[12] += 1; tsec[13] += nc; }
    wsync();
    for (int ci = 0; ci < nc; ci++) {
        const int r = cand[ci];
        const double* o = tile + 8 * r;
        const float4 bb = obb[r];
        bool near = active && !((double)bb.x > hmaxx || (double)bb.y < hminx || (double)bb.z > hmaxy || (double)bb.w < hminy);
        if (!__any(near)) continue;
        if (near) {
#pragma unroll 1
            for (int j = 0; j < 4; j++) {
                double x1 = o[2 * j], y1 = o[2 * j + 1], x2 = o[2 * ((j + 1) & 3)], y2 = o[2 * ((j + 1) & 3) + 1];
                double exmin = fmin(x1, x2), exmax = fmax(x1, x2), eymin = fmin(y1, y2), eymax = fmax(y1, y2);
                if (exmin > hmaxx || exmax < hminx || eymin > hmaxy || eymax < hminy) continue;
                double d = y2 - y1, e = x1 - x2, f = y1 * x2 - x1 * y2;
#pragma unroll
                for (int k = 0; k < 4; k++) {
                    int k2 = (k + 1) & 3;
                    double ax1 = vx[k], ay1 = vy[k], ax2 = vx[k2], ay2 = vy[k2];
                    double vminx = fmin(ax1, ax2), vmaxx = fmax(ax1, ax2), vminy = fmin(ay1, ay2), vmaxy = fmax(ay1, ay2);
                    if (vminx > exmax || vmaxx < exmin || vminy > eymax || vmaxy < eymin) continue;
                    double a = ay2 - ay1, b = ax1 - ax2, c = ay1 * ax2 - ax1 * ay2;
                    double det = a * e - b * d;
                    if (det == 0) continue;
                    double raw_x = (b * f - c * e) / det;
                    double raw_y = (c * d - a * f) / det;
                    bool cx = !(raw_x > exmax) && !(raw_x < exmin) && !(raw_x > vmaxx) && !(raw_x < vminx);
                    bool cy = !(raw_y > eymax) && !(raw_y < eymin) && !(raw_y > vmaxy) && !(raw_y < vminy);
                    if (cx && cy) bad = true;
                }
                if (!FULL && __any(bad)) break;
            }
        }
        if (!FULL && __any(bad)) break;
    }
    wsync();
    RS_T(5);
    return bad;
}

constexpr int RSA_SCENES = WAVE / 4;

template <int J>
__device__ __forceinline__ double quad_get(double v) {
    const int hi = __builtin_amdgcn_mov_dpp(__double2hiint(v), J * 0x55, 0xf, 0xf, true);
    const int lo = __builtin_amdgcn_mov_dpp(__double2loint(v), J * 0x55, 0xf, 0xf, true);
    return __hiloint2double(hi, lo);
}
template <int J>
__device__ __forceinline__ int quad_get(int v) { return __builtin_amdgcn_mov_dpp(v, J * 0x55, 0xf, 0xf, true); }

__device__ __forceinline__ bool rs_dup(int n, double o0, double o1, double o2, double o3, double o4, double c0, double c1,
                                       double c2, double c3, double c4) {
    double s = 0;
    s = s + (o0 - c0); s = s + (o1 - c1); s = s + (o2 - c2);
    if (n > 3) s = s + (o3 - c3);
    if (n > 4) s = s + (o4 - c4);
    return s <= 0.01;
}

constexpr int RSA_GROUPS = 4;
__device__ __constant__ const int rsa_group_begin[RSA_GROUPS + 1] = {0, 3, 7, 9, 12};

__device__ __forceinline__ void set_wave_prio(int pr) {
    if (pr == 1) __builtin_amdgcn_s_setprio(1);
    else if (pr == 2) __builtin_amdgcn_s_setprio(2);
    else if (pr >= 3) __builtin_amdgcn_s_setprio(3);
}

__global__ __launch_bounds__(64) void k_rs_words(RsParams p) {
    set_wave_prio(p.prio_front);
    const int lane = threadIdx.x, q = lane & 3, ls = lane >> 2;
    const int qi = blockIdx.x * RSA_SCENES + ls;
    const double* in = p.rs_in + (size_t)(qi < p.max_queue ? qi : p.max_queue - 1) * RS_IN_WORDS;
    const double X = in[7], Y = in[8], PHI = in[9], sPHI = in[10], cPHI = in[11];
    const double XB = in[12], YB = in[13];
    const int count = *p.rs_count;
    if ((int)blockIdx.x * RSA_SCENES >= count) return;
    const bool live = qi < count;
    const int slot = p.slot_base + p.slot_dir * (live ? qi : 0);

    double* rec = p.rs_rec + (size_t)slot * RS_REC_DOUBLES;
    RsWord* words = (RsWord*)(rec + RS_REC_WORDS);
    double p0 = 0, p1 = 0, p2 = 0, p3 = 0;
    bool pk = false;
    const double hp = 0.5 * PI;
    const int g_begin = rsa_group_begin[blockIdx.y], g_end = rsa_group_begin[blockIdx.y + 1];

    for (int g = g_begin; g < g_end; g++) {
        const bool back = (g == 4 || g == 9 || g == 10);
        const double bx = back ? XB : X, by = back ? YB : Y;
        const double sx = (q & 1) ? -bx : bx;
        const double sy = (q & 2) ? -by : by;
        const double sp = (q == 1 || q == 2) ? -PHI : PHI;
        const double ssp = (q == 1 || q == 2) ? -sPHI : sPHI, csp = cPHI;
        double t = 0, u = 0, v = 0;
        bool ok = false;
        switch (g) {
            case 0: ok = (q == 0 || q == 2) && rs_SLS(sx, sy, sp, t, u, v); break;
            case 1: ok = rs_LSL(sx, sy, sp, ssp, csp, t, u, v); break;
            case 2: ok = rs_LSR(sx, sy, sp, ssp, csp, t, u, v); break;
            case 3: case 4: ok = rs_LRL(sx, sy, sp, ssp, csp, t, u, v); break;
            case 5: ok = rs_LRLRn(sx, sy, sp, ssp, csp, t, u, v); break;
            case 6: ok = rs_LRLRp(sx, sy, sp, ssp, csp, t, u, v); break;
            case 7: case 9: ok = rs_LRSL(sx, sy, sp, ssp, csp, t, u, v); break;
            case 8: case 10: ok = rs_LRSR(sx, sy, sp, ssp, csp, t, u, v); break;
            default: ok = rs_LRSLR(sx, sy, sp, ssp, csp, t, u, v); break;
        }
        ok = ok && live;
        int t0 = TL, t1 = TS, t2_ = TL, t3 = 0, t4 = 0, n = 3;
        double l0 = t, l1 = u, l2 = v, l3 = 0, l4 = 0;
        switch (g) {
            case 0: t0 = TS; t1 = TL; t2_ = TS; break;
            case 1: t0 = TL; t1 = TS; t2_ = TL; break;
            case 2: t0 = TL; t1 = TS; t2_ = TR; break;
            case 3: t0 = TL; t1 = TR; t2_ = TL; break;
            case 4: t0 = TL; t1 = TR; t2_ = TL; l0 = v; l2 = t; break;
            case 5: n = 4; t0 = TL; t1 = TR; t2_ = TL; t3 = TR; l2 = -u; l3 = v; break;
            case 6: n = 4; t0 = TL; t1 = TR; t2_ = TL; t3 = TR; l2 = u; l3 = v; break;
            case 7: n = 4; t0 = TL; t1 = TR; t2_ = TS; t3 = TL; l1 = -hp; l2 = u; l3 = v; break;
            case 8: n = 4; t0 = TL; t1 = TR; t2_ = TS; t3 = TR; l1 = -hp; l2 = u; l3 = v; break;
            case 9: n = 4; t0 = TL; t1 = TS; t2_ = TR; t3 = TL; l0 = v; l1 = u; l2 = -hp; l3 = t; break;
            case 10: n = 4; t0 = TR; t1 = TS; t2_ = TR; t3 = TL; l0 = v; l1 = u; l2 = -hp; l3 = t; break;
            default: n = 5; t0 = TL; t1 = TR; t2_ = TS; t3 = TL; t4 = TR; l1 = -hp; l2 = u; l3 = -hp; l4 = v; break;
        }
        if (q & 1) { l0 = -l0; l1 = -l1; l2 = -l2; l3 = -l3; l4 = -l4; }
        if (q & 2) { t0 = mirror_type(t0); t1 = mirror_type(t1); t2_ = mirror_type(t2_); t3 = mirror_type(t3); t4 = mirror_type(t4); }
        if (n < 4) { t3 = 0; l3 = 0; }
        if (n < 5) { t4 = 0; l4 = 0; }
        const int code = pack_types(t0, t1, t2_, t3, t4, n);
        double L = 0;
        L = L + fabs(l0); L = L + fabs(l1); L = L + fabs(l2);
        if (n > 3) L = L + fabs(l3);
        if (n > 4) L = L + fabs(l4);

        bool dup = false;
        if (g == 4 || g == 6) {
            const double a0 = (q & 2) ? quad_get<2>(p0) : quad_get<0>(p0), a1 = (q & 2) ? quad_get<2>(p1) : quad_get<0>(p1);
            const double a2 = (q & 2) ? quad_get<2>(p2) : quad_get<0>(p2), a3 = (q & 2) ? quad_get<2>(p3) : quad_get<0>(p3);
            const int ak = (q & 2) ? quad_get<2>((int)pk) : quad_get<0>((int)pk);
            const double b0 = (q & 2) ? quad_get<3>(p0) : quad_get<1>(p0), b1 = (q & 2) ? quad_get<3>(p1) : quad_get<1>(p1);
            const double b2 = (q & 2) ? quad_get<3>(p2) : quad_get<1>(p2), b3 = (q & 2) ? quad_get<3>(p3) : quad_get<1>(p3);
            const int bk = (q & 2) ? quad_get<3>((int)pk) : quad_get<1>((int)pk);
            dup = (ak && rs_dup(n, a0, a1, a2, a3, 0, l0, l1, l2, l3, l4)) || (bk && rs_dup(n, b0, b1, b2, b3, 0, l0, l1, l2, l3, l4));
        }
        bool kept = ok && !dup && !(L >= MAX_LENGTH) && !(q & 1);
        {
            const double e0 = (q & 2) ? quad_get<2>(l0) : quad_get<0>(l0), e1 = (q & 2) ? quad_get<2>(l1) : quad_get<0>(l1);
            const double e2 = (q & 2) ? quad_get<2>(l2) : quad_get<0>(l2), e3 = (q & 2) ? quad_get<2>(l3) : quad_get<0>(l3);
            const double e4 = (q & 2) ? quad_get<2>(l4) : quad_get<0>(l4);
            const int ek = (q & 2) ? quad_get<2>((int)kept) : quad_get<0>((int)kept);
            if (q & 1) kept = ok && !dup && !(ek && rs_dup(n, e0, e1, e2, e3, e4, l0, l1, l2, l3, l4)) && !(L >= MAX_LENGTH);
        }
        const double Lm = L / MAXC;
        if (live) rec[RS_REC_KEYS + 4 * g + q] = kept ? Lm : -1.0;
        if (kept) {
            RsWord* w = words + 4 * g + q;
            w->len[0] = l0; w->len[1] = l1; w->len[2] = l2; w->len[3] = l3; w->len[4] = l4;
            w->Lm = Lm; w->code = code; w->n = n;
        }
        p0 = l0; p1 = l1; p2 = l2; p3 = l3; pk = kept;
    }
}

__global__ __launch_bounds__(64) void k_rs_segs(RsParams p) {
    set_wave_prio(p.prio_front);
    __shared__ double keyl[8][RS_WORDS_PER_SCENE];
    __shared__ double prl[8][RS_WORDS_PER_SCENE];
    __shared__ unsigned char hidl[8][RS_WORDS_PER_SCENE];
    __shared__ unsigned char ordl[8][RS_WORDS_PER_SCENE];
    __shared__ int ntl[8];
    __shared__ double hdrl[8][8];
    const int lane = threadIdx.x, ls = lane >> 3, k0 = lane & 7;
    const int qi = blockIdx.x * 8 + ls;
    const int qs = qi < p.max_queue ? qi : p.max_queue - 1;
    const int entry = p.rs_list[qs];
    const int scene = rs_list_scene(entry);
    double* rec = p.rs_rec + (size_t)(p.slot_base + p.slot_dir * qs) * RS_REC_DOUBLES;
    const int count = *p.rs_count;
    if ((int)blockIdx.x * 8 >= count) return;
    const bool live = qi < count;
    double keyv[RS_WORDS_PER_SCENE / 8];
#pragma unroll
    for (int j = 0; j < RS_WORDS_PER_SCENE / 8; j++) keyv[j] = live ? rec[RS_REC_KEYS + 8 * j + k0] : -1.0;
    const double* in = p.rs_in + (size_t)qs * RS_IN_WORDS;
    double hdr = 0.0;
    int hdr_n = 0;
    if (k0 < 3) hdr = in[k0];
    else if (k0 < 7) hdr = in[k0];
    else hdr_n = rs_list_n_obst(entry);
    unsigned long long keptm = 0;
#pragma unroll
    for (int j = 0; j < RS_WORDS_PER_SCENE / 8; j++) {
        const double key = live ? keyv[j] : -1.0;
        keyl[ls][8 * j + k0] = key;
        keptm |= ((__ballot(key >= 0.0) >> (8 * ls)) & 0xffull) << (8 * j);
    }
    __syncthreads();
    if (live && k0 == 0) {
        double* pr = prl[ls];
        unsigned char* hid = hidl[ls];
        int hn = 0;
        for (unsigned long long m = keptm; m; m &= m - 1) {
            const int c = __ffsll((long long)m) - 1;
            const double pv = keyl[ls][c];
            int i = hn++;
            pr[i] = pv; hid[i] = (unsigned char)c;
            while (i) {
                const int parent = (i - 1) >> 1;
                if (pr[parent] < pr[i]) break;
                const double tp = pr[i]; pr[i] = pr[parent]; pr[parent] = tp;
                const unsigned char ti = hid[i]; hid[i] = hid[parent]; hid[parent] = ti;
                i = parent;
            }
        }
        const int n_kept = hn;
        int no = 0;
        double lmin = 0;
        while (hn > 0) {
            const double lm = pr[0];
            if (no == 0) lmin = lm;
            if (lm > 1.6 * lmin && no + 1 > 2) break;
            ordl[ls][no++] = hid[0];
            if (hn == 1) { hn = 0; break; }
            hn--;
            pr[0] = pr[hn]; hid[0] = hid[hn];
            int i = 0;
            for (;;) {
                const int l = (i << 1) + 1, r = (i + 1) << 1;
                int low = (l < hn && pr[l] < pr[i]) ? l : i;
                if (r < hn && pr[r] < pr[low]) low = r;
                if (low == i) break;
                const double tp = pr[i]; pr[i] = pr[low]; pr[low] = tp;
                const unsigned char ti = hid[i]; hid[i] = hid[low]; hid[low] = ti;
                i = low;
            }
        }
        ntl[ls] = no;
        ((int2*)rec)[1] = make_int2(n_kept, no);
    }
    if (live) {
        if (k0 < 7) rec[2 + k0] = hdr;
        else ((int2*)rec)[0] = make_int2(scene, hdr_n);
        hdrl[ls][k0] = hdr;
    }
    __syncthreads();
    if (!live) return;
    const int n_test = ntl[ls];
    const unsigned char* order = ordl[ls];
    const double q0w = hdrl[ls][2];
    double sq0, cq0;
    hm_sincos(q0w, &sq0, &cq0);
    const double fq0x = hdrl[ls][0] - hdrl[ls][3], fq0y = hdrl[ls][1] - hdrl[ls][5];
    for (int k = k0; k < n_test; k += 8) {
        const double* W = rec + RS_REC_WORDS + 8 * (int)order[k];
        double len[5];
#pragma unroll
        for (int i = 0; i < 5; i++) len[i] = W[i];
        const double w6 = W[6];
        const int code = __double2loint(w6), nseg = __double2hiint(w6);
        double* tb = rec + RS_REC_SEGS + RS_SEG_TABLE * k;
        double ox = 0, oy = 0, hy = 0;
#pragma unroll
        for (int i = 0; i < 5; i++) {
            if (i < nseg) {
                const int m = type_of(code, i);
                const double l = len[i];
                double s_oy, c_oy;
                hm_sincos(hy, &s_oy, &c_oy);
                double* sp_ = tb + RS_SEGW * i;
                sp_[0] = ox; sp_[1] = oy; sp_[2] = hy; sp_[3] = c_oy; sp_[4] = s_oy; sp_[5] = (double)m; sp_[6] = l;
                if (i == 0) sp_[7] = w6;
                {
                    const float fox = (float)(fq0x + (cq0 * ox - sq0 * oy)), foy = (float)(fq0y + (sq0 * ox + cq0 * oy));
                    const float fc = (float)(c_oy * cq0 - s_oy * sq0), fs = (float)(s_oy * cq0 + c_oy * sq0);
                    tb[RS_SEG_F32 + 2 * i] = __hiloint2double(__float_as_int(foy), __float_as_int(fox));
                    tb[RS_SEG_F32 + 2 * i + 1] = __hiloint2double(__float_as_int(fs), __float_as_int(fc));
                }
                if (m == TS) {
                    ox = ox + l / MAXC * c_oy;
                    oy = oy + l / MAXC * s_oy;
                } else {
                    double sl, cl;
                    hm_sincos(l, &sl, &cl);
                    const double ldx = sl / MAXC;
                    const double ldy = (m == TL) ? (1.0 - cl) / MAXC : (1.0 - cl) / (-MAXC);
                    ox = ox + (c_oy * ldx + (-s_oy) * ldy);
                    oy = oy + (s_oy * ldx + c_oy * ldy);
                }
                hy = (m == TL) ? hy + l : ((m == TR) ? hy - l : hy);
            }
        }
        if (k == 0) {
            tb[RS_SEGW + 7] = cq0;
            tb[2 * RS_SEGW + 7] = -sq0;
        }
    }
}

constexpr int RSB_SEG = 0, RSB_SEGW = RS_SEGW, RSB_QPD = RS_SEG_TABLE, RSB_QCAP = 256, RSB_BAD = RSB_QPD + RSB_QCAP;
constexpr int RSB_WORDS = RSB_BAD + 8;

template <int OCC, bool TIMING>
__global__ __launch_bounds__(64, OCC) void k_rs_validate(RsParams p, int obs_f64) {
    extern __shared__ __attribute__((aligned(16))) double lds[];
    const int lane = threadIdx.x;
    unsigned long long tsec[16] = {};
    const unsigned long long tstart_ = TIMING ? __builtin_readcyclecounter() : 0;
    RS_T0();
    const int count = *p.rs_count;
    if ((int)blockIdx.x >= count) return;
    if (obs_f64 & 0x400) return;
    const int qidx = scene_of_block(blockIdx.x, count);
    const int slot = p.slot_base + p.slot_dir * qidx;
    double* tile = lds;
    float4* obb = (float4*)(lds + 8 * p.tile_cap);
    double* scr = lds + 10 * p.tile_cap;
    double* segp = scr + RSB_SEG;
    double* qpd = scr + RSB_QPD;
    int* cand = (int*)(scr + RSB_WORDS);
    unsigned char* qseg = (unsigned char*)(cand + ((p.tile_cap + 3) & ~3));

    const double* rec = p.rs_rec + (size_t)slot * RS_REC_DOUBLES;
    const double r0 = lane < RS_REC_HDR ? rec[lane] : 0.0;
    const double* tables = rec + RS_REC_SEGS;
    double tb = lane < RS_SEG_TABLE ? tables[lane] : 0.0;
    const int n_paths = __builtin_amdgcn_readlane(__double2hiint(r0), 1);
    if (n_paths == 0) return;
    const int scene = __builtin_amdgcn_readlane(__double2loint(r0), 0);
    const int n_obst = __builtin_amdgcn_readlane(__double2hiint(r0), 0);
    {
        const double2* src = (const double2*)(p.verts + (size_t)scene * p.max_obst * 8);
        double2* dst = (double2*)tile;
        for (int v = lane; v < 4 * n_obst; v += WAVE) dst[v] = src[v];
        const float4* ob = p.obb + (size_t)scene * p.max_obst;
        for (int o = lane; o < n_obst; o += WAVE) obb[o] = ob[o];
    }
    const double q0x = readlane_d(r0, 2), q0y = readlane_d(r0, 3), q0w = readlane_d(r0, 4);
    const double xmin = readlane_d(r0, 5), xmax = readlane_d(r0, 6), ymin = readlane_d(r0, 7), ymax = readlane_d(r0, 8);
    const double step = RS_STEP * MAXC;
    wsync();

    int found = -1;
    double* bad1 = scr + RSB_BAD;
    if (lane < 6) bad1[lane] = INFINITY;
    wsync();
    RS_T(0);
    const double c_q = readlane_d(tb, RS_SEGW + 7), s_q = readlane_d(tb, 2 * RS_SEGW + 7);
    for (int idx = 1; idx <= n_paths; idx++) {
        if ((obs_f64 & 0x200) && idx > 1) break;
        const double tcur = tb;
        if (idx < n_paths && lane < RS_SEG_TABLE) tb = tables[RS_SEG_TABLE * idx + lane];
        const double len0 = readlane_d(tcur, 6), w6 = readlane_d(tcur, 7);
        const int code = __double2loint(w6), nseg = __double2hiint(w6);
        const int cls1 = type_of(code, 0) * 2 + (len0 > 0.0 ? 1 : 0);
        if (!(obs_f64 & 0x800) && fabs(len0) >= bad1[cls1]) continue;

        bool invalid = false;
        if (lane < RS_SEG_TABLE) segp[lane] = tcur;
        if (lane == 0) { qpd[0] = 0.0; qseg[0] = 0; }
        int nq = 1;
        wsync();
        if (TIMING) tsec[9] += 1;
        RS_T(1);
        const int win = (obs_f64 >> 12) ? min(max(obs_f64 >> 12, 128), RSB_QCAP - WAVE - 1) : 128;
        int i = 0;
        bool seg_open = false, finished = false;
        double pd = 0, ll = 0.0, lprev = 0.0, d = 0, l = 0;
        while (!invalid && (!finished || nq > 0)) {
            while (!finished && nq + WAVE + 1 <= win) {
                if (TIMING) tsec[10] += 1;
                if (!seg_open) {
                    l = segp[RSB_SEGW * i + 6];
                    d = l > 0.0 ? step : -step;
                    if (i >= 1 && (lprev * l) > 0) pd = -d - ll; else pd = d - ll;
                    lprev = l;
                    seg_open = true;
                }
                double mine = pd, t = pd, last = pd;
                int ncap = 0;
                for (int j0 = 0; j0 < WAVE; j0 += 8) {
                    if ((lane >> 3) == (j0 >> 3)) mine = t;
#pragma unroll
                    for (int jj = 0; jj < 7; jj++) t = t + d;
                    last = t;
                    t = t + d;
                    ncap = j0 + 8;
                    if (__any(fabs(last) > fabs(l))) break;
                }
#pragma unroll
                for (int k = 0; k < 7; k++)
                    if (k < (lane & 7)) mine = mine + d;
                const bool in_seg = lane < ncap && fabs(mine) <= fabs(l);
                const unsigned long long valid = (ncap == WAVE) ? ~0ull : ((1ull << ncap) - 1);
                const unsigned long long fail = ~__ballot(in_seg) & valid;
                const int count = fail ? (__ffsll((long long)fail) - 1) : ncap;
                if (lane < count) { qpd[nq + lane] = mine; qseg[nq + lane] = (unsigned char)i; }
                nq += count;
                if (fail) {
                    pd = __shfl(mine, count);
                    ll = l - pd - d;
                    seg_open = false;
                    if (i == nseg - 1) {
                        if (lane == 0) { qpd[nq] = l; qseg[nq] = (unsigned char)i; }
                        nq += 1;
                        finished = true;
                    }
                    i++;
                } else pd = t;
            }
            wsync();
            RS_T(2);
            const int n_all = nq;
            const int n = finished ? n_all : (n_all & ~(WAVE - 1));
            const int stride = (n + WAVE - 1) / WAVE;
            const int n_coarse = (n + stride - 1) / stride;
            const int n_rest = n - n_coarse;
            for (int rnd = 0; rnd == 0 || (rnd - 1) * WAVE < n_rest; rnd++) {
                int idx;
                if (rnd == 0) idx = (lane < n_coarse) ? stride * lane : -1;
                else { const int r = (rnd - 1) * WAVE + lane; idx = r < n_rest ? r + r / (stride - 1) + 1 : -1; }
                const bool active = idx >= 0;
                double px = 0, py = 0, pyaw = 0;
                if (active) {
                    const double spd = qpd[idx];
                    const double* sp_ = segp + RSB_SEGW * (int)qseg[idx];
                    const int m = (int)sp_[5];
                    interpolate(spd, m, sp_[0], sp_[1], sp_[2], sp_[3], -sp_[4], sp_[3], sp_[4], px, py, pyaw);
                }
                const double wx = c_q * px + s_q * py + q0x;
                const double wy = -s_q * px + c_q * py + q0y;
                const double wyaw = pi_2_pi(pyaw + q0w);
                if (TIMING) tsec[11] += 1;
                RS_T(3);
                const bool hit = !(obs_f64 & 0x100) && pose_hits<TIMING>(active, wx, wy, wyaw, tile, obb, cand, n_obst, xmin, xmax, ymin, ymax, lane, tsec);
                if (TIMING) t0_ = __builtin_readcyclecounter();
                if (__any(hit)) {
                    const double mine1 = (hit && active && qseg[idx] == 0) ? fabs(qpd[idx]) : INFINITY;
                    const double v = fmin(bad1[cls1], wave_min_d(mine1));
                    wsync();
                    if (lane < 6 && (lane == cls1 || v == 0.0)) bad1[lane] = fmin(bad1[lane], v);
                    invalid = true;
                    break;
                }
            }
            {
                const int rem = n_all - n;
                double cd = 0;
                unsigned char cs = 0;
                if (lane < rem) { cd = qpd[n + lane]; cs = qseg[n + lane]; }
                wsync();
                if (lane < rem) { qpd[lane] = cd; qseg[lane] = cs; }
                nq = rem;
            }
            wsync();
        }
        if (!invalid) { found = idx - 1; break; }
    }
    if (TIMING) {
        tsec[6] = __builtin_readcyclecounter() - tstart_;
        tsec[8] = 1;
        if (lane == 0) {
            for (int i = 0; i < 16; i++) if (tsec[i]) atomicAdd(&g_rs_prof[(blockIdx.x & 63) * 16 + i], tsec[i]);
            const int li = atomicAdd(&g_rs_log_n, 1);
            if (li < RS_LOG_CAP) g_rs_log[li] = make_int4((int)tsec[6], (int)tsec[9] | (n_paths << 8) | ((p.tile_cap > 32) << 16), (int)tsec[11], found >= 0);
        }
    }
    if (found < 0) return;

    const double wlen = lane < 5 ? segp[RSB_SEGW * lane + 6] : 0.0;
    const int code = __double2loint(segp[7]), nseg = __double2hiint(segp[7]);
    if (lane < 5) {
        double lm = lane < nseg ? wlen / MAXC : 0.0;
        if (p.rs_lengths) {
            if (obs_f64 & 1) ((double*)p.rs_lengths)[5 * (size_t)scene + lane] = lm;
            else ((float*)p.rs_lengths)[5 * (size_t)scene + lane] = (float)lm;
        }
        p.rs_word[8 * (size_t)scene + lane] = lane < nseg ? (int8_t)type_of(code, lane) : (int8_t)HOPE_RS_NONE;
    }
    if (lane == 5) p.rs_word[8 * (size_t)scene + 5] = (int8_t)nseg;
    if (lane == 6) p.rs_word[8 * (size_t)scene + 6] = 1;
}


constexpr float FEPS = 1e-3f, FKAPPA = 2e-2f, FETA_HULL = 2e-3f;
constexpr float F_INV_MAXC = (float)(1.0 / MAXC);
constexpr float F_HL = (float)(0.5 * (CAR_XF - CAR_XR)), F_HW = (float)CAR_YH, F_MID = (float)(0.5 * (CAR_XF + CAR_XR));
constexpr int RS_TAB = 256;
constexpr int RSB_TABF = RSB_BAD + 8, RSB_WORDS_F = RSB_TABF + RS_TAB;
constexpr int RSF_OCC = 4;
__device__ double g_rs_steps[RS_TAB];
__device__ unsigned long long g_rs_fstat[16];
__device__ double g_rs_fdump[64 * 16];

template <bool FULL>
__device__ __noinline__ bool exact_pass(int idx, const double* segp, const double* qpd, const unsigned char* qseg, double c_q,
                                        double s_q, double q0x, double q0y, double q0w, const double* verts_g,
                                        const float4* obb_g, int* cand, int n_obst, double xmin, double xmax, double ymin,
                                        double ymax, int lane) {
    const bool active = idx >= 0;
    double px = 0, py = 0, pyaw = 0;
    if (active) {
        const double spd = qpd[idx];
        const double* sp_ = segp + RSB_SEGW * (int)qseg[idx];
        const int m = (int)sp_[5];
        interpolate(spd, m, sp_[0], sp_[1], sp_[2], sp_[3], -sp_[4], sp_[3], sp_[4], px, py, pyaw);
    }
    const double wx = c_q * px + s_q * py + q0x;
    const double wy = -s_q * px + c_q * py + q0y;
    const double wyaw = pi_2_pi(pyaw + q0w);
    unsigned long long tsec[16];
    return pose_hits<false, FULL>(active, wx, wy, wyaw, verts_g, obb_g, cand, n_obst, xmin, xmax, ymin, ymax, lane, tsec);
}

__device__ __forceinline__ void hull_corner(int k, double ct, double st, double wx, double wy, double& cx, double& cy) {
    cx = ct * car_x(k) - st * car_y(k) + wx;
    cy = st * car_x(k) + ct * car_y(k) + wy;
}
__device__ __forceinline__ bool exact_edges(bool unc, int sidx, int ua, int ub, bool uover, const int* cand, int nc, const double* segp,
                                            const double* qpd, const unsigned char* qseg, const double* tile64, const double* rec) {
    bool bad = false;
    if (unc) {
        const double q0x = rec[2], q0y = rec[3], q0w = rec[4], xmin = rec[5], xmax = rec[6], ymin = rec[7], ymax = rec[8];
        const double c_q = rec[RS_REC_SEGS + RS_SEGW + 7], s_q = rec[RS_REC_SEGS + 2 * RS_SEGW + 7];
        double px = 0, py = 0, pyaw = 0;
        {
            const double spd = qpd[sidx];
            const double* sp_ = segp + RSB_SEGW * (int)qseg[sidx];
            interpolate(spd, (int)sp_[5], sp_[0], sp_[1], sp_[2], sp_[3], -sp_[4], sp_[3], sp_[4], px, py, pyaw);
        }
        const double wx = c_q * px + s_q * py + q0x;
        const double wy = -s_q * px + c_q * py + q0y;
        const double wyaw = pi_2_pi(pyaw + q0w);
        bad = wx < xmin || wx > xmax || wy < ymin || wy > ymax;
        double st_, ct_;
        hm_sincos(wyaw, &st_, &ct_);
        double hminx, hmaxx, hminy, hmaxy;
        {
            double cx0, cy0, cx1, cy1, cx2, cy2, cx3, cy3;
            hull_corner(0, ct_, st_, wx, wy, cx0, cy0); hull_corner(1, ct_, st_, wx, wy, cx1, cy1);
            hull_corner(2, ct_, st_, wx, wy, cx2, cy2); hull_corner(3, ct_, st_, wx, wy, cx3, cy3);
            hminx = fmin(fmin(cx0, cx1), fmin(cx2, cx3)); hmaxx = fmax(fmax(cx0, cx1), fmax(cx2, cx3));
            hminy = fmin(fmin(cy0, cy1), fmin(cy2, cy3)); hmaxy = fmax(fmax(cy0, cy1), fmax(cy2, cy3));
        }
        const int n_slot = uover ? nc : 2;
#pragma unroll 1
        for (int slot = 0; slot < n_slot; slot++) {
            const int rec_ = uover ? (cand[slot] | 0xF00) : (slot ? ub : ua);
            if (rec_ < 0) continue;
            const double* o = tile64 + 8 * (rec_ & 0xff);
#pragma unroll 1
            for (int j = 0; j < 4; j++) {
                if (!((rec_ >> (8 + j)) & 1)) continue;
                const double x1 = o[2 * j], y1 = o[2 * j + 1], x2 = o[2 * ((j + 1) & 3)], y2 = o[2 * ((j + 1) & 3) + 1];
                const double exmin = fmin(x1, x2), exmax = fmax(x1, x2), eymin = fmin(y1, y2), eymax = fmax(y1, y2);
                if (exmin > hmaxx || exmax < hminx || eymin > hmaxy || eymax < hminy) continue;
                const double d_ = y2 - y1, e_ = x1 - x2, f_ = y1 * x2 - x1 * y2;
#pragma unroll 1
                for (int k = 0; k < 4; k++) {
                    double ax1, ay1, ax2, ay2;
                    hull_corner(k, ct_, st_, wx, wy, ax1, ay1);
                    hull_corner((k + 1) & 3, ct_, st_, wx, wy, ax2, ay2);
                    const double vminx = fmin(ax1, ax2), vmaxx = fmax(ax1, ax2), vminy = fmin(ay1, ay2), vmaxy = fmax(ay1, ay2);
                    if (vminx > exmax || vmaxx < exmin || vminy > eymax || vmaxy < eymin) continue;
                    const double a_ = ay2 - ay1, b_ = ax1 - ax2, c_ = ay1 * ax2 - ax1 * ay2;
                    const double det = a_ * e_ - b_ * d_;
                    if (det == 0) continue;
                    const double raw_x = (b_ * f_ - c_ * e_) / det;
                    const double raw_y = (c_ * d_ - a_ * f_) / det;
                    const bool cx_ = !(raw_x > exmax) && !(raw_x < exmin) && !(raw_x > vmaxx) && !(raw_x < vminx);
                    const bool cy_ = !(raw_y > eymax) && !(raw_y < eymin) && !(raw_y > vmaxy) && !(raw_y < vminy);
                    if (cx_ && cy_) bad = true;
                }
            }
        }
    }
    return bad;
}

__device__ __forceinline__ double uni_d(double v) {
    return __hiloint2double(__builtin_amdgcn_readfirstlane(__double2hiint(v)), __builtin_amdgcn_readfirstlane(__double2loint(v)));
}

__device__ __forceinline__ void lsync() {
    asm volatile("s_waitcnt lgkmcnt(0)" ::: "memory");
    __builtin_amdgcn_wave_barrier();
}

constexpr double SCREEN_EPS = 1e-7;
constexpr int SCREEN_SPAN = 128;

__device__ __forceinline__ bool screen_obstacle_hit(const float4 v01, const float4 v23, float cx, float cy, float hc, float hs,
                                                    int efl, bool hull_ok) {
    constexpr float FEPS_ = FEPS, FKAPPA_ = FKAPPA, HL = F_HL, HW = F_HW;
    float u[4], w[4];
    {
        const float dx0 = v01.x - cx, dy0 = v01.y - cy, dx1 = v01.z - cx, dy1 = v01.w - cy;
        const float dx2 = v23.x - cx, dy2 = v23.y - cy, dx3 = v23.z - cx, dy3 = v23.w - cy;
        u[0] = hc * dx0 + hs * dy0; w[0] = hc * dy0 - hs * dx0;
        u[1] = hc * dx1 + hs * dy1; w[1] = hc * dy1 - hs * dx1;
        u[2] = hc * dx2 + hs * dy2; w[2] = hc * dy2 - hs * dx2;
        u[3] = hc * dx3 + hs * dy3; w[3] = hc * dy3 - hs * dx3;
    }
    const float umin = fminf(fminf(u[0], u[1]), fminf(u[2], u[3])), umax = fmaxf(fmaxf(u[0], u[1]), fmaxf(u[2], u[3]));
    const float wmin = fminf(fminf(w[0], w[1]), fminf(w[2], w[3])), wmax = fmaxf(fmaxf(w[0], w[1]), fmaxf(w[2], w[3]));
    if (umin > HL + FEPS_ || umax < -HL - FEPS_ || wmin > HW + FEPS_ || wmax < -HW - FEPS_) return false;
    float g[4];
#pragma unroll
    for (int k = 0; k < 4; k++) g[k] = fmaxf(fabsf(u[k]) - HL, fabsf(w[k]) - HW);
    bool hit = false;
#pragma unroll
    for (int k = 0; k < 4; k++) {
        const int k2 = (k + 1) & 3;
        const float nu = w[k2] - w[k], nw = u[k] - u[k2];
        const float dist = fabsf(__builtin_fmaf(nu, u[k], nw * w[k]));
        const float dn = dist - __builtin_fmaf(fabsf(nu), HL, fabsf(nw) * HW);
        const float eu0 = fminf(u[k], u[k2]), eu1 = fmaxf(u[k], u[k2]);
        const float ew0 = fminf(w[k], w[k2]), ew1 = fmaxf(w[k], w[k2]);
        const float esep = fmaxf(fmaxf(eu0 - HL, -HL - eu1), fmaxf(ew0 - HW, -HW - ew1));
        const float n1 = fabsf(nu) + fabsf(nw), mg = FEPS_ * n1;
        const bool clear = dn > mg || esep > FEPS_ || fmaxf(g[k], g[k2]) < -FEPS_;
        const bool cross = dn < -mg && esep < -FEPS_ && fminf(fabsf(g[k]), fabsf(g[k2])) > FEPS_ && fmaxf(g[k], g[k2]) > FEPS_;
        const float A = fabsf(nu) * HL, B = fabsf(nw) * HW;
        const bool corners_ok = fminf(fabsf(dn), fabsf(dist - fabsf(A - B))) > mg;
        const bool cross_u = fabsf(dist - A) <= B + mg, cross_w = fabsf(dist - B) <= A + mg;
        const bool angle_ok = (!cross_u || fabsf(nw) >= FKAPPA_ * n1) && (!cross_w || fabsf(nu) >= FKAPPA_ * n1);
        hit = hit || (!clear && cross && corners_ok && angle_ok && hull_ok && ((efl >> k) & 1));
    }
    return hit;
}

template <bool TIMING>
__device__ __forceinline__ unsigned long long screen_words(int lane, int n_paths, int n_obst, const double* tables, double* qpd, int* pq, int* cand,
                                                           const float2* fv, const float4* fbox, const unsigned char* eflag, float fxmax,
                                                           float fymax, unsigned long long* tsec) {
    const float fxmin = 0.0f, fymin = 0.0f;
    const double step = RS_STEP * MAXC;
    unsigned long long condemned = 0;
    RS_T0();
    const double inv_step = 1.0 / step;
    for (int w0 = 0; w0 < n_paths; w0 += 4) {
        const int nw = min(4, n_paths - w0);
        if (w0 > 0)
            for (int t = lane; t < RS_SEG_TABLE * nw; t += WAVE) qpd[t] = tables[RS_SEG_TABLE * w0 + t];
        lsync();
        RS_T(14);
        const int G = nw == 1 ? 64 : (nw == 2 ? 32 : (nw == 3 ? 21 : 16));
        const int stride = SCREEN_SPAN / G;
        const int wl_ = nw == 1 ? 0 : (nw == 2 ? lane >> 5 : (nw == 3 ? (lane >= 42 ? 2 : (lane >= 21 ? 1 : 0)) : lane >> 4));
        const int kk = lane - wl_ * G;
        const double* T = qpd + RS_SEG_TABLE * wl_;
        const double w7s = T[7];
        const int codew = __double2loint(w7s), nsegw = __double2hiint(w7s);
        const double a = (double)((kk + 1) * stride) * step;
        double c = 0.0, u0 = step, r = 0.0, lprev = 0.0, pdv = 0.0;
        int si = -1;
#pragma unroll
        for (int i = 0; i < 5; i++) {
            if (i < nsegw) {
                const double l = T[RS_SEGW * i + 6], al = fabs(l);
                if (i >= 1) u0 = (lprev * l > 0) ? r : -r;
                if (si < 0 && a < c + al) {
                    double j = ceil((a - c - u0) * inv_step);
                    j = j < 0.0 ? 0.0 : j;
                    const double u = u0 + j * step;
                    si = (fabs(u0) <= al && u > SCREEN_EPS && u < al - SCREEN_EPS) ? i : 5;
                    pdv = l > 0.0 ? u : -u;
                }
                const double n = fabs(u0) > al ? 0.0 : floor((al - u0) * inv_step) + 1.0;
                r = u0 + n * step - al;
                c += al;
                lprev = l;
            }
        }
        const bool active = lane < G * nw && si >= 0 && si < 5;
        float X = 0, Y = 0, hc = 1, hs = 0;
        if (active) {
            const float lf = (float)pdv;
            const float4 row = ((const float4*)(T + RS_SEG_F32))[si];
            const int m = type_of(codew, si);
            const float rev = lf * 0.15915494309189535f;
            const float sl = m == TS ? 0.0f : __builtin_amdgcn_sinf(rev), cl = m == TS ? 1.0f : __builtin_amdgcn_cosf(rev);
            const float sgn = m == TR ? -1.0f : 1.0f;
            const float ldx = m == TS ? lf * F_INV_MAXC : sl * F_INV_MAXC;
            const float ldy = sgn * (1.0f - cl) * F_INV_MAXC;
            X = row.x + (row.z * ldx - row.w * ldy);
            Y = row.y + (row.w * ldx + row.z * ldy);
            const float ss = sgn * sl;
            hc = row.z * cl - row.w * ss;
            hs = row.w * cl + row.z * ss;
        }
        const bool oob = active && (X < fxmin - FEPS || X > fxmax + FEPS || Y < fymin - FEPS || Y > fymax + FEPS);
        const float cx = X + hc * F_MID, cy = Y + hs * F_MID;
        const float ex = fabsf(hc) * F_HL + fabsf(hs) * F_HW + FEPS, ey = fabsf(hs) * F_HL + fabsf(hc) * F_HW + FEPS;
        const float lox = cx - ex, hix = cx + ex, loy = cy - ey, hiy = cy + ey;
        const float ulox = wave_min_f(active ? lox : INFINITY), uhix = wave_max_f(active ? hix : -INFINITY);
        const float uloy = wave_min_f(active ? loy : INFINITY), uhiy = wave_max_f(active ? hiy : -INFINITY);
        int nc = 0;
        for (int base = 0; base < n_obst; base += WAVE) {
            const int o = base + lane;
            bool near = false;
            if (o < n_obst) {
                const float4 bb = fbox[o];
                near = !(bb.x > uhix || bb.y < ulox || bb.z > uhiy || bb.w < uloy);
            }
            const unsigned long long mm = __ballot(near);
            if (near) cand[nc + __popcll(mm & ((1ull << lane) - 1))] = o;
            nc += __popcll(mm);
        }
        RS_T(15);
        const int all_w = (1 << nw) - 1;
        int dead = 0;
        for (int w = 0; w < nw; w++) dead |= __ballot(oob && wl_ == w) ? (1 << w) : 0;
        auto classify = [&](int count) {
            const bool has = lane < count;
            const int pr = has ? pq[lane] : 0;
            const int sl_ = pr & 63, ro = pr >> 6;
            const float scx = __shfl(cx, sl_), scy = __shfl(cy, sl_), shc = __shfl(hc, sl_), shs = __shfl(hs, sl_);
            const int sw = __shfl(wl_, sl_);
            bool h = false;
            if (has && !((dead >> sw) & 1)) {
                const float4 v01 = ((const float4*)fv)[2 * ro], v23 = ((const float4*)fv)[2 * ro + 1];
                h = screen_obstacle_hit(v01, v23, scx, scy, shc, shs, (int)eflag[ro], fminf(fabsf(shc), fabsf(shs)) >= FETA_HULL);
            }
            for (int w = 0; w < nw; w++) dead |= __ballot(h && sw == w) ? (1 << w) : 0;
        };
        if (nc > 0 && dead != all_w) {
            lsync();
            int npq = 0;
            for (int ci = 0; ci < nc; ci++) {
                const int ro = cand[ci];
                const float4 bb = fbox[ro];
                const bool near = active && !oob && !((dead >> wl_) & 1) && !(bb.x > hix || bb.y < lox || bb.z > hiy || bb.w < loy);
                const unsigned long long nm = __ballot(near);
                if (!nm) continue;
                if (near) pq[npq + __popcll(nm & ((1ull << lane) - 1))] = (ro << 6) | lane;
                npq += __popcll(nm);
                if (npq >= WAVE) {
                    lsync();
                    classify(WAVE);
                    if (dead == all_w) { npq = 0; break; }
                    const int rem = npq - WAVE;
                    int cv = 0;
                    if (lane < rem) cv = pq[WAVE + lane];
                    lsync();
                    if (lane < rem) pq[lane] = cv;
                    npq = rem;
                }
            }
            if (npq > 0 && dead != all_w) { lsync(); classify(npq); }
        }
        condemned |= (unsigned long long)dead << w0;
        lsync();
        RS_T(7);
    }
    return condemned;
}

template <bool TIMING, int OCC = 8>
__global__ __launch_bounds__(64, OCC) void k_rs_screen(RsParams p) {
    extern __shared__ __attribute__((aligned(16))) double lds[];
    const int lane = threadIdx.x;
    unsigned long long tsec[16] = {};
    const int b_ = (int)blockIdx.x;
    const int qidx = scene_of_block(b_, p.max_queue);
    const int entry = p.rs_list[qidx];
    const int count = *p.rs_count;
    if (qidx >= count) return;
    const int slot = p.slot_base + p.slot_dir * qidx;
    const int scene = rs_list_scene(entry), n_obst = rs_list_n_obst(entry);
    float2* fv = (float2*)lds;
    float4* fbox = (float4*)(lds + 4 * p.tile_cap);
    double* tabs = lds + 6 * p.tile_cap;
    int* pq = (int*)(tabs + 4 * RS_SEG_TABLE);
    int* cand = pq + 2 * WAVE;
    unsigned char* eflag = (unsigned char*)(cand + ((p.tile_cap + 3) & ~3));
    double* rec = p.rs_rec + (size_t)slot * RS_REC_DOUBLES;
    const double r0 = lane < RS_REC_HDR ? rec[lane] : 0.0;
    const double* tables = rec + RS_REC_SEGS;
    {
        typedef __attribute__((address_space(3))) void* lds_ptr;
        const double2* t2 = (const double2*)tables;
        __builtin_amdgcn_global_load_lds((const void*)(t2 + lane), (lds_ptr)tabs, 16, 0, 0);
        if (lane < 2 * RS_SEG_TABLE - WAVE) __builtin_amdgcn_global_load_lds((const void*)(t2 + WAVE + lane), (lds_ptr)(tabs + 2 * WAVE), 16, 0, 0);
        const float4* gfv = p.fverts + (size_t)scene * p.max_obst * 2;
        const float4* gfb = p.fbox + (size_t)scene * p.max_obst;
        const uint32_t* gfl = (const uint32_t*)(p.eflag + (size_t)scene * eflag_stride(p.max_obst));
        float4* lfv = (float4*)fv;
        for (int base = 0; base < 2 * n_obst; base += WAVE)
            if (base + lane < 2 * n_obst) __builtin_amdgcn_global_load_lds((const void*)(gfv + base + lane), (lds_ptr)(lfv + base), 16, 0, 0);
        for (int base = 0; base < n_obst; base += WAVE)
            if (base + lane < n_obst) __builtin_amdgcn_global_load_lds((const void*)(gfb + base + lane), (lds_ptr)(fbox + base), 16, 0, 0);
        for (int base = 0; 4 * base < n_obst; base += WAVE)
            if (4 * (base + lane) < n_obst) __builtin_amdgcn_global_load_lds((const void*)(gfl + base + lane), (lds_ptr)((uint32_t*)eflag + base), 4, 0, 0);
    }
    asm volatile("s_waitcnt vmcnt(0)" ::: "memory");
    const int n_paths = __builtin_amdgcn_readlane(__double2hiint(r0), 1);
    if (n_paths == 0) return;
    const float fxmax = (float)(readlane_d(r0, 6) - readlane_d(r0, 5)), fymax = (float)(readlane_d(r0, 8) - readlane_d(r0, 7));
    lsync();
    const unsigned long long condemned = screen_words<TIMING>(lane, n_paths, n_obst, tables, tabs, pq, cand, fv, fbox, eflag, fxmax, fymax, tsec);
    if (lane == 0) {
        ((unsigned long long*)rec)[9] = condemned;
        if (condemned != ((1ull << n_paths) - 1)) p.surv_list[atomicAdd(p.surv_count, 1)] = make_int2(qidx, entry);
    }
}

template <int OCC, bool TIMING, bool STATS, bool PRE = false>
__global__ __launch_bounds__(64, OCC) void k_rs_validate_f(RsParams p, int obs_f64) {
    extern __shared__ __attribute__((aligned(16))) double lds[];
    const int lane = threadIdx.x;
    if (!(obs_f64 & 0x10000)) __builtin_amdgcn_s_setprio(1);
    unsigned long long tsec[16] = {};
    const unsigned long long tstart_ = TIMING ? __builtin_readcyclecounter() : 0;
    RS_T0();
    const int b_ = (int)blockIdx.x;
    int qidx, entry;
    if (PRE) {
        const int2 sv = p.surv_list[b_];
        if (b_ >= *p.surv_count) return;
        qidx = sv.x; entry = sv.y;
    } else {
#ifdef HOPE_RS_3TRIPS
        const int count = *p.rs_count;
        if (b_ >= count) return;
        qidx = scene_of_block(b_, count);
        entry = p.rs_list[qidx];
#else
        qidx = scene_of_block(b_, p.max_queue);
        entry = p.rs_list[qidx];
        const int count = *p.rs_count;
        if (qidx >= count) return;
#endif
    }
    const int slot = p.slot_base + p.slot_dir * qidx;
#ifndef HOPE_RS_HDR
    const int scene = rs_list_scene(entry);
    const int n_obst = rs_list_n_obst(entry);
#endif
    float2* fv = (float2*)lds;
    float4* fbox = (float4*)(lds + 4 * p.tile_cap);
    double* scr = lds + 6 * p.tile_cap;
    double* segp = scr + RSB_SEG;
    double* qpd = scr + RSB_QPD;
    int* cand = (int*)(scr + RSB_WORDS_F);
    double* tabl = scr + RSB_TABF;
    unsigned char* qseg = (unsigned char*)(cand + ((p.tile_cap + 3) & ~3));
    unsigned char* eflag = qseg + RSB_QCAP;

    const double* rec = p.rs_rec + (size_t)slot * RS_REC_DOUBLES;
    const double r0 = lane < RS_REC_HDR ? rec[lane] : 0.0;
    const double* tables = rec + RS_REC_SEGS;
#ifdef HOPE_RS_3TRIPS
    if (__builtin_amdgcn_readlane(__double2hiint(r0), 1) == 0) return;
#endif
#ifdef HOPE_RS_HDR
    const int scene = __builtin_amdgcn_readlane(__double2loint(r0), 0);
    const int n_obst = __builtin_amdgcn_readlane(__double2hiint(r0), 0);
    (void)entry;
#endif
    double tb = lane < RS_SEG_TABLE ? tables[lane] : 0.0;
    if (!PRE) {
        typedef __attribute__((address_space(3))) void* lds_ptr;
        const double2* t2 = (const double2*)tables;
        __builtin_amdgcn_global_load_lds((const void*)(t2 + lane), (lds_ptr)qpd, 16, 0, 0);
        if (lane < 2 * RS_SEG_TABLE - WAVE) __builtin_amdgcn_global_load_lds((const void*)(t2 + WAVE + lane), (lds_ptr)(qpd + 2 * WAVE), 16, 0, 0);
    }
    {
        typedef __attribute__((address_space(3))) void* lds_ptr;
        const float4* gfv = p.fverts + (size_t)scene * p.max_obst * 2;
        const float4* gfb = p.fbox + (size_t)scene * p.max_obst;
        const uint32_t* gfl = (const uint32_t*)(p.eflag + (size_t)scene * eflag_stride(p.max_obst));
        float4* lfv = (float4*)fv;
        for (int base = 0; base < 2 * n_obst; base += WAVE)
            if (base + lane < 2 * n_obst) __builtin_amdgcn_global_load_lds((const void*)(gfv + base + lane), (lds_ptr)(lfv + base), 16, 0, 0);
        for (int base = 0; base < n_obst; base += WAVE)
            if (base + lane < n_obst) __builtin_amdgcn_global_load_lds((const void*)(gfb + base + lane), (lds_ptr)(fbox + base), 16, 0, 0);
        for (int base = 0; 4 * base < n_obst; base += WAVE)
            if (4 * (base + lane) < n_obst) __builtin_amdgcn_global_load_lds((const void*)(gfl + base + lane), (lds_ptr)((uint32_t*)eflag + base), 4, 0, 0);
    }
    const int n_paths = __builtin_amdgcn_readlane(__double2hiint(r0), 1);
    if (n_paths == 0) {
        asm volatile("s_waitcnt vmcnt(0)" ::: "memory");
        return;
    }
    const double* verts_g = p.verts + (size_t)scene * p.max_obst * 8;
    const float fxmin = 0.0f, fxmax = (float)(readlane_d(r0, 6) - readlane_d(r0, 5)), fymin = 0.0f, fymax = (float)(readlane_d(r0, 8) - readlane_d(r0, 7));
    const double step = RS_STEP * MAXC;
    bool tile_pending = true;
    int found = -1;
    double* bad1 = scr + RSB_BAD;
    if (lane < 6) bad1[lane] = INFINITY;
    lsync();
    RS_T(0);
    const bool paranoid = (obs_f64 & 0x2000) != 0;
    unsigned long long st_pass = 0, st_hit = 0, st_exact = 0, st_unc = 0, st_bad_hit = 0, st_bad_clear = 0, st_samples = 0;
    unsigned long long st_why[5] = {};
    unsigned long long condemned = 0;
    if (PRE) condemned = (unsigned long long)__double_as_longlong(readlane_d(r0, 9));
    else if (!(obs_f64 & 0x20000)) {
        asm volatile("s_waitcnt vmcnt(0)" ::: "memory");
        tile_pending = false;
        condemned = screen_words<TIMING>(lane, n_paths, n_obst, tables, qpd, (int*)tabl ,
                                         cand, fv, fbox, eflag, fxmax, fymax, tsec);
        if (TIMING) t0_ = __builtin_readcyclecounter();
    }
    else {
        asm volatile("s_waitcnt vmcnt(0)" ::: "memory");
        tile_pending = false;
    }
    const bool verify_screen = STATS && paranoid;
    const bool all_condemned = condemned == ((1ull << n_paths) - 1);
    unsigned long long st_scr_words = __popcll(condemned), st_scr_dead = all_condemned ? 1 : 0, st_scr_bad = 0;
    if (!all_condemned || verify_screen) {
        const double T0 = g_rs_steps[lane], T1 = g_rs_steps[WAVE + lane], T2 = g_rs_steps[2 * WAVE + lane], T3 = g_rs_steps[3 * WAVE + lane];
        tabl[lane] = T0; tabl[WAVE + lane] = T1; tabl[2 * WAVE + lane] = T2; tabl[3 * WAVE + lane] = T3;
        lsync();
    }
    for (int idx = 1; idx <= n_paths; idx++) {
        if (all_condemned && !verify_screen) break;
        const double tcur = tb;
        if (idx < n_paths && lane < RS_SEG_TABLE) tb = tables[RS_SEG_TABLE * idx + lane];
        const double len0 = readlane_d(tcur, 6), w6 = readlane_d(tcur, 7);
        const int code = __double2loint(w6), nseg = __double2hiint(w6);
        const int cls1 = type_of(code, 0) * 2 + (len0 > 0.0 ? 1 : 0);
        if (fabs(len0) >= bad1[cls1]) continue;
        const bool screened = (condemned >> (idx - 1)) & 1;
        if (screened && !verify_screen) continue;
        bool invalid = false;
        if (lane < RS_SEG_TABLE) segp[lane] = tcur;
        if (TIMING) tsec[9] += 1;
        {
            double zero;
            asm volatile("v_mov_b64 %0, 0" : "=v"(zero));
            if (lane == 0) { qpd[0] = zero; qseg[0] = (unsigned char)__double2loint(zero); }
        }
        int nq = 1;
        lsync();
        RS_T(1);
        const int win = 128;
        int i = 0, t_off = 0;
        bool seg_open = false, finished = false;
        double pd = 0, ll = 0.0, lprev = 0.0, d = 0, l = 0;
        while (!invalid && (!finished || nq > 0)) {
            while (!finished && nq + WAVE + 1 <= win) {
                if (TIMING) tsec[10] += 1;
                if (!seg_open) {
                    l = uni_d(segp[RSB_SEGW * i + 6]);
                    d = uni_d(l > 0.0 ? step : -step);
                    pd = uni_d((i >= 1 && (lprev * l) > 0) ? -d - ll : d - ll);
                    lprev = l;
                    seg_open = true;
                }
                double mine, t = pd;
                int ncap;
                if (i == 0 && t_off + WAVE <= RS_TAB) {
                    const double v = tabl[t_off + lane];
                    mine = d > 0.0 ? v : -v;
                    ncap = WAVE;
                    t_off += WAVE;
                    if (t_off < RS_TAB) {
                        const double nx = tabl[t_off];
                        t = d > 0.0 ? nx : -nx;
                    } else t = readlane_d(mine, WAVE - 1) + d;
                } else {
                    mine = pd;
                    double last = pd;
                    ncap = 0;
                    for (int j0 = 0; j0 < WAVE; j0 += 8) {
                        if ((lane >> 3) == (j0 >> 3)) mine = t;
#pragma unroll
                        for (int jj = 0; jj < 7; jj++) t = t + d;
                        last = t;
                        t = t + d;
                        ncap = j0 + 8;
                        if (__any(fabs(last) > fabs(l))) break;
                    }
#pragma unroll
                    for (int k = 0; k < 7; k++)
                        if (k < (lane & 7)) mine = mine + d;
                }
                const bool in_seg = lane < ncap && fabs(mine) <= fabs(l);
                const unsigned long long valid = (ncap == WAVE) ? ~0ull : ((1ull << ncap) - 1);
                const unsigned long long fail = ~__ballot(in_seg) & valid;
                const int cnt = fail ? (__ffsll((long long)fail) - 1) : ncap;
                if (lane < cnt) { qpd[nq + lane] = mine; qseg[nq + lane] = (unsigned char)i; }
                nq += cnt;
                if (fail) {
                    pd = readlane_d(mine, cnt);
                    ll = uni_d(l - pd - d);
                    seg_open = false;
                    if (i == nseg - 1) {
                        if (lane == 0) { qpd[nq] = l; qseg[nq] = (unsigned char)i; }
                        nq += 1;
                        finished = true;
                    }
                    i++;
                } else pd = uni_d(t);
            }
            lsync();
            RS_T(2);
            const int n_all = nq;
            const int n = finished ? n_all : (n_all & ~(WAVE - 1));
            const int stride = (n + WAVE - 1) >> 6;
            const int n_coarse = stride == 1 ? n : (stride == 2 ? (n + 1) >> 1 : ((n + 2) * 171) >> 9);
            const int n_rest = n - n_coarse;
            for (int rnd = 0; rnd == 0 || (rnd - 1) * WAVE < n_rest; rnd++) {
                int sidx;
                if (rnd == 0) sidx = (lane < n_coarse) ? stride * lane : -1;
                else { const int r = (rnd - 1) * WAVE + lane; sidx = r < n_rest ? r + (stride == 2 ? r : r >> 1) + 1 : -1; }
                const bool active = sidx >= 0;
                if (TIMING) tsec[11] += 1;
                float X = 0, Y = 0, hc = 1, hs = 0;
                int sg0 = 0;
                if (active) {
                    const float lf = (float)qpd[sidx];
                    sg0 = (int)qseg[sidx];
                    const float4 row = ((const float4*)(segp + RS_SEG_F32))[sg0];
                    const int m = type_of(code, sg0);
                    const float rev = lf * 0.15915494309189535f;
                    const float sl = m == TS ? 0.0f : __builtin_amdgcn_sinf(rev), cl = m == TS ? 1.0f : __builtin_amdgcn_cosf(rev);
                    const float sgn = m == TR ? -1.0f : 1.0f;
                    const float ldx = m == TS ? lf * F_INV_MAXC : sl * F_INV_MAXC;
                    const float ldy = sgn * (1.0f - cl) * F_INV_MAXC;
                    X = row.x + (row.z * ldx - row.w * ldy);
                    Y = row.y + (row.w * ldx + row.z * ldy);
                    const float ss = sgn * sl;
                    hc = row.z * cl - row.w * ss;
                    hs = row.w * cl + row.z * ss;
                }
                RS_T(3);
                int why_cnt = 0, hit_rec = -1;
                int ua = -1, ub = -1;
                bool uover = false;
                bool hit = active && (X < fxmin - FEPS || X > fxmax + FEPS || Y < fymin - FEPS || Y > fymax + FEPS);
                bool unc = active && !hit && (X < fxmin + FEPS || X > fxmax - FEPS || Y < fymin + FEPS || Y > fymax - FEPS);
                const float cx = X + hc * F_MID, cy = Y + hs * F_MID;
                const float ex = fabsf(hc) * F_HL + fabsf(hs) * F_HW + FEPS, ey = fabsf(hs) * F_HL + fabsf(hc) * F_HW + FEPS;
                const float lox = cx - ex, hix = cx + ex, loy = cy - ey, hiy = cy + ey;
                const float ulox = wave_min_f(active ? lox : INFINITY), uhix = wave_max_f(active ? hix : -INFINITY);
                const float uloy = wave_min_f(active ? loy : INFINITY), uhiy = wave_max_f(active ? hiy : -INFINITY);
                if (tile_pending) {
                    asm volatile("s_waitcnt vmcnt(0)" ::: "memory");
                    tile_pending = false;
                }
                int nc = 0;
                for (int base = 0; base < n_obst; base += WAVE) {
                    const int o = base + lane;
                    bool near = false;
                    if (o < n_obst) {
                        const float4 bb = fbox[o];
                        near = !(bb.x > uhix || bb.y < ulox || bb.z > uhiy || bb.w < uloy);
                    }
                    const unsigned long long mm = __ballot(near);
                    if (near) cand[nc + __popcll(mm & ((1ull << lane) - 1))] = o;
                    nc += __popcll(mm);
                }
                RS_T(4);
                if (nc > 0 && !__any(hit)) {
                    if (TIMING) { tsec[12] += 1; tsec[13] += nc; }
                    lsync();
                    const bool hull_ok = fminf(fabsf(hc), fabsf(hs)) >= FETA_HULL;
                    for (int ci = 0; ci < nc; ci++) {
                        const int r = cand[ci];
                        const float4 bb = fbox[r];
                        const bool near = active && !(bb.x > hix || bb.y < lox || bb.z > hiy || bb.w < loy);
                        if (!__any(near)) continue;
                        const float4 v01 = ((const float4*)fv)[2 * r], v23 = ((const float4*)fv)[2 * r + 1];
                        float u[4], w[4];
                        {
                            const float dx0 = v01.x - cx, dy0 = v01.y - cy, dx1 = v01.z - cx, dy1 = v01.w - cy;
                            const float dx2 = v23.x - cx, dy2 = v23.y - cy, dx3 = v23.z - cx, dy3 = v23.w - cy;
                            u[0] = hc * dx0 + hs * dy0; w[0] = hc * dy0 - hs * dx0;
                            u[1] = hc * dx1 + hs * dy1; w[1] = hc * dy1 - hs * dx1;
                            u[2] = hc * dx2 + hs * dy2; w[2] = hc * dy2 - hs * dx2;
                            u[3] = hc * dx3 + hs * dy3; w[3] = hc * dy3 - hs * dx3;
                        }
                        const float umin = fminf(fminf(u[0], u[1]), fminf(u[2], u[3])), umax = fmaxf(fmaxf(u[0], u[1]), fmaxf(u[2], u[3]));
                        const float wmin = fminf(fminf(w[0], w[1]), fminf(w[2], w[3])), wmax = fmaxf(fmaxf(w[0], w[1]), fmaxf(w[2], w[3]));
                        const bool maybe = near && !(umin > F_HL + FEPS || umax < -F_HL - FEPS || wmin > F_HW + FEPS || wmax < -F_HW - FEPS);
                        if (!__any(maybe)) continue;
                        const int efl = (int)eflag[r];
                        float g[4];
#pragma unroll
                        for (int k = 0; k < 4; k++) g[k] = fmaxf(fabsf(u[k]) - F_HL, fabsf(w[k]) - F_HW);
                        float nu[4], nw[4], dn[4], esep[4];
                        float dist[4];
                        int open = 0;
#pragma unroll
                        for (int k = 0; k < 4; k++) {
                            const int k2 = (k + 1) & 3;
                            nu[k] = w[k2] - w[k]; nw[k] = u[k] - u[k2];
                            dist[k] = fabsf(__builtin_fmaf(nu[k], u[k], nw[k] * w[k]));
                            dn[k] = dist[k] - __builtin_fmaf(fabsf(nu[k]), F_HL, fabsf(nw[k]) * F_HW);
                            const float eu0 = fminf(u[k], u[k2]), eu1 = fmaxf(u[k], u[k2]);
                            const float ew0 = fminf(w[k], w[k2]), ew1 = fmaxf(w[k], w[k2]);
                            esep[k] = fmaxf(fmaxf(eu0 - F_HL, -F_HL - eu1), fmaxf(ew0 - F_HW, -F_HW - ew1));
                            const float mg = FEPS * (fabsf(nu[k]) + fabsf(nw[k]));
                            const bool clear = dn[k] > mg || esep[k] > FEPS || fmaxf(g[k], g[k2]) < -FEPS;
                            open |= (maybe && !clear) ? (1 << k) : 0;
                        }
#pragma unroll
                        for (int k = 0; k < 4; k++) {
                            if (!__any((open >> k) & 1)) continue;
                            const int k2 = (k + 1) & 3;
                            const float n1 = fabsf(nu[k]) + fabsf(nw[k]), mg = FEPS * n1;
                            const bool cross = dn[k] < -mg && esep[k] < -FEPS && fminf(fabsf(g[k]), fabsf(g[k2])) > FEPS && fmaxf(g[k], g[k2]) > FEPS;
                            const float A = fabsf(nu[k]) * F_HL, B = fabsf(nw[k]) * F_HW;
                            const bool corners_ok = fminf(fabsf(dn[k]), fabsf(dist[k] - fabsf(A - B))) > mg;
                            const bool cross_u = fabsf(dist[k] - A) <= B + mg, cross_w = fabsf(dist[k] - B) <= A + mg;
                            const bool angle_ok = (!cross_u || fabsf(nw[k]) >= FKAPPA * n1) && (!cross_w || fabsf(nu[k]) >= FKAPPA * n1);
                            const bool certain = cross && corners_ok && angle_ok && hull_ok && ((efl >> k) & 1);
                            const bool mine_open = (open >> k) & 1;
                            if (mine_open && certain) { hit = true; if (STATS && hit_rec < 0) hit_rec = r * 4 + k; }
                            if (STATS && mine_open && !certain) why_cnt |= 1 << (!cross ? 0 : !((efl >> k) & 1) ? 1 : !hull_ok ? 2 : !corners_ok ? 3 : 4);
                            if (!__any(hit) && mine_open && !certain) {
                                unc = true;
                                if (ua < 0) ua = r | (0x100 << k);
                                else if ((ua & 0xff) == r) ua |= 0x100 << k;
                                else if (ub < 0) ub = r | (0x100 << k);
                                else if ((ub & 0xff) == r) ub |= 0x100 << k;
                                else uover = true;
                            }
                        }
                        if (__any(hit)) break;
                    }
                    lsync();
                }
                RS_T(5);
                bool bad = hit;
                const bool any_hit = __any(hit);
                const bool need64 = (STATS && paranoid) || (!any_hit && __any(unc));
                (void)need64;
                if (STATS) {
                    st_pass += 1;
                    if (any_hit) st_hit += 1;
                    if (!any_hit && __any(unc)) {
                        const unsigned long long wm = __ballot(why_cnt != 0);
                        int wor = 0;
                        for (int b = 0; b < 5; b++) if (__any((why_cnt >> b) & 1)) wor |= 1 << b;
                        for (int b = 0; b < 5; b++) st_why[b] += (wor >> b) & 1;
                        (void)wm;
                    }
                }
                if (STATS && paranoid) {
                    const double q0x = rec[2], q0y = rec[3], q0w = rec[4], xmin = rec[5], xmax = rec[6], ymin = rec[7], ymax = rec[8];
                    const double c_q = rec[RS_REC_SEGS + RS_SEGW + 7], s_q = rec[RS_REC_SEGS + 2 * RS_SEGW + 7];
                    const bool ex = exact_pass<true>(active ? sidx : -1, segp, qpd, qseg, c_q, s_q, q0x, q0y, q0w, verts_g, p.obb + (size_t)scene * p.max_obst, cand, n_obst, xmin, xmax, ymin, ymax, lane);
                    st_samples += __popcll(__ballot(active));
                    st_bad_hit += __popcll(__ballot(active && hit && !ex));
                    if (active && ((hit && !ex) || (!any_hit && !hit && !unc && ex))) {
                        const int di = (int)atomicAdd(&g_rs_fstat[15], 1ull);
                        if (di < 64) {
                            double px = 0, py = 0, pyaw = 0;
                            const double spd = qpd[sidx];
                            const double* sp_ = segp + RSB_SEGW * (int)qseg[sidx];
                            interpolate(spd, (int)sp_[5], sp_[0], sp_[1], sp_[2], sp_[3], -sp_[4], sp_[3], sp_[4], px, py, pyaw);
                            const double wyaw = pi_2_pi(pyaw + q0w);
                            double* dd = g_rs_fdump + 16 * di;
                            dd[0] = scene; dd[1] = idx; dd[2] = spd; dd[3] = (double)qseg[sidx]; dd[4] = X; dd[5] = Y; dd[6] = hc; dd[7] = hs;
                            dd[8] = c_q * px + s_q * py; dd[9] = -s_q * px + c_q * py; dd[10] = hm_cos(wyaw); dd[11] = hm_sin(wyaw);
                            dd[12] = hit ? 1.0 : 0.0; dd[13] = (double)why_cnt; dd[14] = sp_[5]; dd[15] = (double)hit_rec;
                        }
                    }
                    if (!any_hit) st_bad_clear += __popcll(__ballot(active && !hit && !unc && ex));
                    bad = ex;
                } else if (!any_hit && __any(unc)) {
                    if (STATS) { st_exact += 1; st_unc += __popcll(__ballot(unc)); }
                    bad = exact_edges(unc, sidx, ua, ub, uover, cand, nc, segp, qpd, qseg, verts_g, rec);
                }
                if (TIMING) t0_ = __builtin_readcyclecounter();
                if (__any(bad)) {
                    const double mine1 = (bad && active && qseg[sidx] == 0) ? fabs(qpd[sidx]) : INFINITY;
                    const double v = fmin(bad1[cls1], wave_min_d(mine1));
                    lsync();
                    if (lane < 6 && (lane == cls1 || v == 0.0)) bad1[lane] = fmin(bad1[lane], v);
                    invalid = true;
                    break;
                }
            }
            {
                const int rem = n_all - n;
                double cd = 0;
                unsigned char cs = 0;
                if (lane < rem) { cd = qpd[n + lane]; cs = qseg[n + lane]; }
                lsync();
                if (lane < rem) { qpd[lane] = cd; qseg[lane] = cs; }
                nq = rem;
            }
            lsync();
        }
        if (STATS && screened && !invalid) { st_scr_bad += 1; continue; }
        if (!invalid) { found = idx - 1; break; }
    }
    if (STATS && lane == 0) {
        atomicAdd(&g_rs_fstat[7], st_scr_bad); atomicAdd(&g_rs_fstat[13], st_scr_words); atomicAdd(&g_rs_fstat[14], st_scr_dead);
        for (int b = 0; b < 5; b++) atomicAdd(&g_rs_fstat[8 + b], st_why[b]);
        atomicAdd(&g_rs_fstat[0], st_pass); atomicAdd(&g_rs_fstat[1], st_hit); atomicAdd(&g_rs_fstat[2], st_exact);
        atomicAdd(&g_rs_fstat[3], st_unc); atomicAdd(&g_rs_fstat[4], st_bad_hit); atomicAdd(&g_rs_fstat[5], st_bad_clear);
        atomicAdd(&g_rs_fstat[6], st_samples);
    }
    if (TIMING) {
        tsec[6] = __builtin_readcyclecounter() - tstart_;
        tsec[8] = 1;
        if (lane == 0) {
            for (int i = 0; i < 16; i++) if (tsec[i]) atomicAdd(&g_rs_prof[(blockIdx.x & 63) * 16 + i], tsec[i]);
            const int li = atomicAdd(&g_rs_log_n, 1);
            if (li < RS_LOG_CAP) g_rs_log[li] = make_int4((int)tsec[6], (int)tsec[9] | (n_paths << 8) | ((p.tile_cap > 32) << 16), (int)tsec[11], found >= 0);
        }
    }
    if (found < 0) return;
    const double wlen = lane < 5 ? segp[RSB_SEGW * lane + 6] : 0.0;
    const int code = __double2loint(segp[7]), nseg = __double2hiint(segp[7]);
    if (lane < 5) {
        double lm = lane < nseg ? wlen / MAXC : 0.0;
        if (p.rs_lengths) {
            if (obs_f64 & 1) ((double*)p.rs_lengths)[5 * (size_t)scene + lane] = lm;
            else ((float*)p.rs_lengths)[5 * (size_t)scene + lane] = (float)lm;
        }
        p.rs_word[8 * (size_t)scene + lane] = lane < nseg ? (int8_t)type_of(code, lane) : (int8_t)HOPE_RS_NONE;
    }
    if (lane == 5) p.rs_word[8 * (size_t)scene + 5] = (int8_t)nseg;
    if (lane == 6) p.rs_word[8 * (size_t)scene + 6] = 1;
}

}

static size_t rs_lds_bytes_exact(int max_obst) {
    return (size_t)(10 * max_obst + RSB_WORDS) * 8 + (size_t)((max_obst + 3) & ~3) * 4 + RSB_QCAP;
}
static size_t rs_lds_bytes_filter(int max_obst) {
    return (size_t)(6 * max_obst + RSB_WORDS_F) * 8 + (size_t)((max_obst + 3) & ~3) * 4 + RSB_QCAP + (size_t)((max_obst + 3) & ~3);
}
size_t rs_lds_bytes(int max_obst) { return std::max(rs_lds_bytes_exact(max_obst), rs_lds_bytes_filter(max_obst)); }
size_t rs_screen_lds_bytes(int max_obst) {
    return (size_t)(6 * max_obst + 4 * RS_SEG_TABLE) * 8 + 2 * WAVE * 4 + (size_t)((max_obst + 3) & ~3) * 4 + (size_t)((max_obst + 3) & ~3);
}
size_t rs_rec_bytes_per_scene() { return sizeof(double) * RS_REC_DOUBLES; }

hipError_t rs_prof_read(unsigned long long* out, int reset) {
    hipError_t e = hipDeviceSynchronize();
    if (e != hipSuccess) return e;
    static unsigned long long buf[64 * 16];
    e = hipMemcpyFromSymbol(buf, HIP_SYMBOL(g_rs_prof), sizeof(buf));
    for (int i = 0; i < 16; i++) { out[i] = 0; for (int sh = 0; sh < 64; sh++) out[i] += buf[sh * 16 + i]; }
    if (e == hipSuccess && reset) {
        for (auto& v : buf) v = 0;
        e = hipMemcpyToSymbol(HIP_SYMBOL(g_rs_prof), buf, sizeof(buf));
    }
    return e;
}

hipError_t rs_fdump_read(double* out ) {
    hipError_t e = hipDeviceSynchronize();
    if (e != hipSuccess) return e;
    return hipMemcpyFromSymbol(out, HIP_SYMBOL(g_rs_fdump), sizeof(double) * 64 * 16);
}

hipError_t rs_log_read(int* out , int cap, int* n, int reset) {
    hipError_t e = hipDeviceSynchronize();
    if (e != hipSuccess) return e;
    e = hipMemcpyFromSymbol(n, HIP_SYMBOL(g_rs_log_n), sizeof(int));
    if (e != hipSuccess) return e;
    const int m = *n < cap ? (*n < RS_LOG_CAP ? *n : RS_LOG_CAP) : cap;
    if (m > 0) e = hipMemcpyFromSymbol(out, HIP_SYMBOL(g_rs_log), sizeof(int4) * (size_t)m);
    if (e == hipSuccess && reset) { const int z = 0; e = hipMemcpyToSymbol(HIP_SYMBOL(g_rs_log_n), &z, sizeof(int)); }
    return e;
}

hipError_t rs_fstat_read(unsigned long long* out , int reset) {
    hipError_t e = hipDeviceSynchronize();
    if (e != hipSuccess) return e;
    e = hipMemcpyFromSymbol(out, HIP_SYMBOL(g_rs_fstat), 16 * sizeof(unsigned long long));
    if (e == hipSuccess && reset) {
        unsigned long long z[16] = {};
        e = hipMemcpyToSymbol(HIP_SYMBOL(g_rs_fstat), z, sizeof(z));
    }
    return e;
}

hipError_t rs_init_tables() {
    static bool done[64] = {};
    int dev = 0;
    hipError_t e = hipGetDevice(&dev);
    if (e != hipSuccess) return e;
    if (dev >= 0 && dev < 64 && done[dev]) return hipSuccess;
    double tab[RS_TAB];
    const volatile double step = RS_STEP * MAXC;
    volatile double t = step;
    for (int k = 0; k < RS_TAB; k++) { tab[k] = t; t = t + step; }
    e = hipMemcpyToSymbol(HIP_SYMBOL(g_rs_steps), tab, sizeof(tab));
    if (e == hipSuccess && dev >= 0 && dev < 64) done[dev] = true;
    return e;
}

constexpr int RS_LARGE_TILE_WPC = 6;
constexpr int RS_PRIO_MIN_SCENES = 32768;

hipError_t launch_rs_search(const RsParams& p, hipStream_t stream, LaunchTimer* timer) {
    if (p.max_queue <= 0) return hipSuccess;
    static const bool timing = getenv("HOPE_RS_TIMING") != nullptr;
    const bool exact = getenv("HOPE_RS_EXACT") != nullptr;
    const int dbg = getenv("HOPE_RS_DEBUG") ? (int)strtol(getenv("HOPE_RS_DEBUG"), nullptr, 0) : 0;
    const bool stats = (dbg & 0x6000) != 0;
    size_t lds = exact ? rs_lds_bytes_exact(p.tile_cap) : rs_lds_bytes_filter(p.tile_cap);
    if (!exact && p.tile_cap > 32) lds = std::max(lds, (size_t)((158 * 1024 / RS_LARGE_TILE_WPC) & ~255));
    if (lds > 48 * 1024) {
        hipError_t e = hipFuncSetAttribute((const void*)k_rs_validate_f<RSF_OCC, false, false, true>, hipFuncAttributeMaxDynamicSharedMemorySize, (int)lds);
        if (e != hipSuccess) return e;
    }
    const void* vk = exact ? (timing ? (const void*)k_rs_validate<3, true> : (const void*)k_rs_validate<3, false>)
                           : (timing ? (const void*)k_rs_validate_f<RSF_OCC, true, false> : stats ? (const void*)k_rs_validate_f<RSF_OCC, false, true>
                              : (const void*)k_rs_validate_f<RSF_OCC, false, false>);
    if (lds > 48 * 1024) {
        hipError_t e = hipFuncSetAttribute(vk, hipFuncAttributeMaxDynamicSharedMemorySize, (int)lds);
        if (e != hipSuccess) return e;
    }
    if (!exact) { hipError_t e = rs_init_tables(); if (e != hipSuccess) return e; }
    if (timer) timer->begin(HOPE_K_RS_WORDS, stream);
    hipLaunchKernelGGL(k_rs_words, dim3((p.max_queue + RSA_SCENES - 1) / RSA_SCENES, RSA_GROUPS), dim3(WAVE), 0, stream, p);
    if (timer) timer->end(stream);
    if (timer) timer->begin(HOPE_K_RS_SEGS, stream);
    hipLaunchKernelGGL(k_rs_segs, dim3((p.max_queue + 7) / 8), dim3(WAVE), 0, stream, p);
    if (timer) timer->end(stream);
    const bool split = !exact && !timing && !stats && !(dbg & 0x20000) && p.surv_count && p.surv_list &&
                       getenv("HOPE_RS_SPLIT") && atoi(getenv("HOPE_RS_SPLIT")) == 1;
    if (split) {
        if (timer) timer->begin(HOPE_K_RS_SCREEN, stream);
        hipLaunchKernelGGL((k_rs_screen<false, 8>), dim3(p.max_queue), dim3(WAVE), rs_screen_lds_bytes(p.tile_cap), stream, p);
        if (timer) timer->end(stream);
    }
    if (timer) timer->begin(HOPE_K_RS_VALIDATE, stream);
    const bool longer_chain = 2 * (long long)p.max_queue >= p.n;
    const int flags = (p.obs_f64 ? 1 : 0) | dbg | ((p.n < RS_PRIO_MIN_SCENES || !longer_chain) ? 0x10000 : 0);
    if (exact) {
        if (timing) hipLaunchKernelGGL((k_rs_validate<3, true>), dim3(p.max_queue), dim3(WAVE), lds, stream, p, flags);
        else hipLaunchKernelGGL((k_rs_validate<3, false>), dim3(p.max_queue), dim3(WAVE), lds, stream, p, flags);
    } else if (split) hipLaunchKernelGGL((k_rs_validate_f<RSF_OCC, false, false, true>), dim3(p.max_queue), dim3(WAVE), lds, stream, p, flags);
    else if (timing) hipLaunchKernelGGL((k_rs_validate_f<RSF_OCC, true, false>), dim3(p.max_queue), dim3(WAVE), lds, stream, p, flags);
    else if (stats) hipLaunchKernelGGL((k_rs_validate_f<RSF_OCC, false, true>), dim3(p.max_queue), dim3(WAVE), lds, stream, p, flags);
    else hipLaunchKernelGGL((k_rs_validate_f<RSF_OCC, false, false>), dim3(p.max_queue), dim3(WAVE), lds, stream, p, flags);
    if (timer) timer->end(stream);
    return hipGetLastError();
}

}
```

### include/hope_env.h

```cpp
#ifndef HOPE_ENV_H
#define HOPE_ENV_H

#include <stdint.h>

#ifdef __cplusplus
extern "C" {
#endif

#define HOPE_ABI_VERSION 8

#define HOPE_LIDAR_NUM 120
#define HOPE_N_ACTION 42
#define HOPE_N_ITER 10
#define HOPE_UPSAMPLE 10
#define HOPE_TARGET_DIM 5
#define HOPE_RS_MAX_SEG 5
#define HOPE_IMG_SIZE 64
#define HOPE_IMG_CHANNELS 3
#define HOPE_TRAJ_RENDER_LEN 20

#define HOPE_OK 0
#define HOPE_EINVAL (-1)
#define HOPE_ENODEV (-2)
#define HOPE_ENOMEM (-3)
#define HOPE_EHIP (-4)
#define HOPE_ESTATE (-5)

#define HOPE_STATUS_CONTINUE 1
#define HOPE_STATUS_ARRIVED 2
#define HOPE_STATUS_COLLIDED 3
#define HOPE_STATUS_OUTBOUND 4
#define HOPE_STATUS_OUTTIME 5

#define HOPE_RS_NONE (-1)
#define HOPE_RS_S 0
#define HOPE_RS_L 1
#define HOPE_RS_R 2

#define HOPE_F_OBS_F64 0x1
#define HOPE_F_ACTION_F64 0x2
#define HOPE_F_PROFILE 0x4
#define HOPE_F_IMAGE 0x8
#define HOPE_F_OVERLAP 0x10


#define HOPE_STAGE_MOTION 0x1
#define HOPE_STAGE_OBS 0x2
#define HOPE_STAGE_REWARD 0x4
#define HOPE_STAGE_RS 0x8
#define HOPE_STAGE_ALL 0xF
#define HOPE_STAGE_IMG 0x40
#define HOPE_ACTION_PHYSICAL 0x10
#define HOPE_ACTION_RESCALE_F32 0x80
#define HOPE_AUTO_RESET 0x20
#define HOPE_AUTO_REDRAW 0x100
#define HOPE_DEFER_RS 0x200

typedef struct hope_env hope_env_t;

typedef struct hope_step_out {
    void *lidar;
    void *action_mask;
    void *target;
    void *reward;
    void *reward_info;
    int32_t *status;
    uint8_t *done;
    double *pose;
    int8_t *rs_word;
    void *rs_lengths;
    uint8_t *img;
} hope_step_out;

#define HOPE_MAX_OBSTACLES 255
int hope_env_create(hope_env_t **out, int n_scenes, int max_obstacles, int device_id, uint32_t flags);
int hope_env_destroy(hope_env_t *h);
const char *hope_last_error(void);
int hope_abi_version(void);

int hope_env_upload_tables(hope_env_t *h, const double *dist_star, const double *hull_base,
                           const double *beam_ab);

int hope_env_set_scenes(hope_env_t *h, const int32_t *scene_ids, int n, const double *start,
                        const double *dest, const double *bbox, const double *verts,
                        const int32_t *n_obst);

int hope_env_step(hope_env_t *h, const void *actions, const uint8_t *active, uint32_t stages,
                  const hope_step_out *out, void *stream);

int hope_env_wait_rs(hope_env_t *h, void *stream);
int hope_env_last_step(hope_env_t *h, uint64_t *step);
int hope_env_wait_rs_step(hope_env_t *h, uint64_t step, void *stream);

int hope_env_reset_obs(hope_env_t *h, const uint8_t *active, uint32_t stages, const hope_step_out *out,
                       void *stream);

int hope_env_restart(hope_env_t *h, const uint8_t *mask, void *stream);

int hope_env_set_pool(hope_env_t *h, int n_pool, const double *start, const double *dest, const double *bbox,
                      const double *verts, const int32_t *n_obst);
int hope_env_pool_staging(hope_env_t *h, int n_pool, double **start, double **dest, double **bbox, double **verts, int32_t **n_obst);
int hope_env_commit_pool(hope_env_t *h, int n_pool, void *stream);
int hope_env_commit_pool_relaxed(hope_env_t *h, int n_pool);
int hope_env_pool_staging_ready(hope_env_t *h);
int hope_env_pool_generation(hope_env_t *h, uint64_t *generation);
int hope_env_set_redraw_seed(hope_env_t *h, uint64_t seed);
int hope_env_redraw(hope_env_t *h, const uint8_t *mask, uint64_t seed, void *stream);
int hope_env_download_pool_index(hope_env_t *h, int32_t *out );

int hope_env_set_dlp_cases(hope_env_t *h, int n_cases, const double *dest, const int32_t *cand_off, const double *cand,
                           const int32_t *case_set, int n_sets, const int32_t *set_off, const double *set_verts);
int hope_env_set_draw_class(hope_env_t *h, const int32_t *scene_ids, int n, const uint8_t *cls);
int hope_env_pool_overflow(hope_env_t *h, int32_t *count);
int hope_env_download_scenes(hope_env_t *h, const int32_t *scene_ids, int n, double *start, double *dest, double *bbox, double *verts,
                             int32_t *n_obst);
int hope_env_download_n_obst(hope_env_t *h, int32_t *n_obst );
int hope_env_download_pool_state(hope_env_t *h, int32_t *pool_index , uint32_t *episode );
int hope_env_restore_maps(hope_env_t *h, const uint8_t *drawn , const uint32_t *episode , uint64_t seed, uint64_t pool_generation);

int hope_env_queue_check(hope_env_t *h, int32_t *queue_of_role , int32_t *n_queues, double *ms);

#define HOPE_K_KINEMATICS 0
#define HOPE_K_STEP 1
#define HOPE_K_RS_WORDS 2
#define HOPE_K_RS_VALIDATE 3
#define HOPE_K_IMAGE 4
#define HOPE_K_IMAGE_PREP 5
#define HOPE_K_RS_COMPACT 6
#define HOPE_K_POST 7
#define HOPE_K_RS_SEGS 8
#define HOPE_K_RS_SCREEN 9
#define HOPE_N_KERNELS 10
int hope_env_kernel_ms(hope_env_t *h, double *ms , int64_t *launches ,
                       int reset);
int hope_env_kernel_union_ms(hope_env_t *h, double *ms , int64_t *calls , int reset);
int hope_env_profile_kernels(hope_env_t *h, uint32_t kernel_mask);

int hope_env_download_state(hope_env_t *h, double *pose , int32_t *t ,
                            double *accum );
int hope_env_upload_state(hope_env_t *h, const double *pose, const int32_t *t, const double *accum);

int hope_debug_math(int fn, int n, const double *a, const double *b, double *out, void *stream);

int hope_debug_mask_lut(const double *dist_star, const double *hull_base, uint16_t *lut_out, double *scale_out);

int hope_debug_traffic(int mode, size_t bytes, void *buf, void *stream);

int hope_debug_rs_prof(uint64_t *out , int reset);
int hope_debug_rs_filter_stats(uint64_t *out , int reset);
int hope_debug_rs_filter_dump(double *out );
int hope_debug_rs_log(int32_t *out , int cap, int32_t *n, int reset);
int hope_debug_step_prof(uint64_t *out , int reset);
int hope_debug_census(uint64_t *out , int reset);

int hope_scenegen_generate(int level, int bay_mode, int n, uint64_t seed, int64_t first_index, int max_obstacles, double *start,
                           double *dest, double *bbox, double *verts, int32_t *n_obst, int32_t *case_id, int n_threads);
int hope_scenegen_default_threads(void);

int hope_scenegen_generate_det(int level, int bay_mode, int n, uint64_t seed, int64_t first_index, int max_obstacles, double *start,
                               double *dest, double *bbox, double *verts, int32_t *n_obst, int32_t *case_id, int n_threads);
int hope_scenegen_generate_device(int device_id, int level, int bay_mode, int n, uint64_t seed, int64_t first_index, int max_obstacles,
                                  double *start, double *dest, double *bbox, double *verts, int32_t *n_obst, int32_t *case_id, void *stream);
int hope_scenegen_log_det(int n, const double *x, double *y);
int hope_env_generate_pool(hope_env_t *h, int n_pool, const int32_t *n_per_level , uint64_t seed, int64_t first_index, int relaxed);

#define HOPE_CURRICULUM_LIST_LEN (1 << 20)
typedef struct hope_curriculum_params {
    double target[4];
    double type_window;
    double case_window;
    double type_fail_min;
    double case_fail_min;
    double worst_share;
    double case_uniform;
    int64_t type_horizon;
    int64_t case_horizon;
} hope_curriculum_params;
int hope_env_curriculum_enable(hope_env_t *h, const hope_curriculum_params *params);
int hope_env_curriculum_disable(hope_env_t *h);
int hope_env_set_pool_buckets(hope_env_t *h, int n_pool, const uint8_t *bucket);
int hope_env_curriculum_tally(hope_env_t *h, const int32_t *status, const uint8_t *done, void *stream);
int hope_env_curriculum_update(hope_env_t *h, void *stream);
int hope_env_curriculum_state(hope_env_t *h, int32_t *n_buckets, uint64_t *episodes, uint64_t *successes, double *win_n, double *win_s,
                              double *prob, double *pw, uint64_t *misc);
int hope_env_curriculum_set_windows(hope_env_t *h, int n_buckets, const double *win_n, const double *win_s, const uint64_t *episodes,
                                    const uint64_t *successes);
int hope_env_curriculum_download_lists(hope_env_t *h, int32_t *list0, int32_t *list1, int32_t *positions);
int hope_curriculum_lists_host(const hope_curriculum_params *params, int n_pool, const int32_t *n_obst, const uint8_t *bucket, int n_cases,
                               int max_obstacles, const uint64_t *episodes, const double *win_n, const double *win_s, int32_t *list0,
                               int32_t *list1, double *prob, double *pw, int32_t *positions);
int hope_curriculum_fold_host(double *n, double *s, double dn, double ds, double window);

int hope_map_level_host(int n, int max_obstacles, const double *start, const double *dest, const double *verts, const int32_t *n_obst,
                        uint8_t *level, int32_t *detail, int n_threads);
int hope_map_level_device(int device_id, int n, int max_obstacles, const double *start, const double *dest, const double *verts,
                          const int32_t *n_obst, uint8_t *level, int32_t *detail, void *stream);
int hope_env_map_level(hope_env_t *h, const uint8_t *active, uint8_t *level, int32_t *detail, void *stream);

int hope_env_num_scenes(const hope_env_t *h);
int hope_env_max_obstacles(const hope_env_t *h);
const char *hope_env_device_arch(const hope_env_t *h);

#ifdef __cplusplus
}
#endif
#endif
```

Baseline: 161.9 million.

## Pre-screen first RS words in k_rs_segs and compact survivors before validation

Adds a coarse pre-screen inside k_rs_segs that samples a few poses along the first four Reeds-Shepp words, tests them for out-of-bounds and obstacle hits, and records a dead-word mask. Scenes whose tested words are all dead are left off the survivor list, and the validate kernel (new PRE==2 variant) seeds its condemned mask from the pre-screen result. The aim is to remove validation work for scenes that will fail anyway. In exchange k_rs_segs does more work, uses more LDS, and launches now depend on the survivor list.

```diff
diff --git a/hope_amd/_lib.py b/hope_amd/_lib.py
--- a/hope_amd/_lib.py
+++ b/hope_amd/_lib.py
@@ -19,7 +19,7 @@
 
 EXPORTS = ['hope_env_create', 'hope_env_destroy', 'hope_last_error', 'hope_abi_version', 'hope_env_upload_tables',
            'hope_env_set_scenes', 'hope_env_step', 'hope_env_wait_rs', 'hope_env_last_step', 'hope_env_wait_rs_step', 'hope_env_download_n_obst', 'hope_env_queue_check', 'hope_env_reset_obs', 'hope_env_download_state',
-           'hope_env_upload_state', 'hope_env_restart', 'hope_env_set_pool', 'hope_env_pool_staging', 'hope_env_commit_pool', 'hope_env_commit_pool_relaxed', 'hope_env_pool_staging_ready', 'hope_env_pool_generation', 'hope_env_redraw', 'hope_env_set_redraw_seed', 'hope_env_download_pool_index', 'hope_env_set_dlp_cases', 'hope_env_pool_overflow', 'hope_env_set_draw_class', 'hope_env_download_scenes', 'hope_env_download_pool_state', 'hope_env_restore_maps', 'hope_env_kernel_ms', 'hope_env_kernel_union_ms', 'hope_env_profile_kernels', 'hope_debug_math', 'hope_debug_traffic', 'hope_debug_mask_lut', 'hope_debug_rs_prof', 'hope_debug_rs_log', 'hope_debug_rs_filter_stats', 'hope_debug_rs_filter_dump', 'hope_debug_step_prof', 'hope_debug_census', 'hope_scenegen_generate', 'hope_scenegen_default_threads', 'hope_scenegen_generate_det', 'hope_scenegen_generate_device', 'hope_scenegen_log_det', 'hope_env_generate_pool', 'hope_env_curriculum_enable', 'hope_env_curriculum_disable', 'hope_env_set_pool_buckets', 'hope_env_curriculum_tally', 'hope_env_curriculum_update', 'hope_env_curriculum_state', 'hope_env_curriculum_set_windows', 'hope_env_curriculum_download_lists', 'hope_curriculum_lists_host', 'hope_curriculum_fold_host', 'hope_map_level_host', 'hope_map_level_device', 'hope_env_map_level', 'hope_env_num_scenes', 'hope_env_max_obstacles', 'hope_env_device_arch']
+           'hope_env_upload_state', 'hope_env_restart', 'hope_env_set_pool', 'hope_env_pool_staging', 'hope_env_commit_pool', 'hope_env_commit_pool_relaxed', 'hope_env_pool_staging_ready', 'hope_env_pool_generation', 'hope_env_redraw', 'hope_env_set_redraw_seed', 'hope_env_download_pool_index', 'hope_env_set_dlp_cases', 'hope_env_pool_overflow', 'hope_env_set_draw_class', 'hope_env_download_scenes', 'hope_env_download_pool_state', 'hope_env_restore_maps', 'hope_env_kernel_ms', 'hope_env_kernel_union_ms', 'hope_env_profile_kernels', 'hope_debug_math', 'hope_debug_traffic', 'hope_debug_mask_lut', 'hope_debug_rs_prof', 'hope_debug_rs_log', 'hope_debug_rs_filter_stats', 'hope_debug_rs_prescreen_stats', 'hope_debug_rs_filter_dump', 'hope_debug_step_prof', 'hope_debug_census', 'hope_scenegen_generate', 'hope_scenegen_default_threads', 'hope_scenegen_generate_det', 'hope_scenegen_generate_device', 'hope_scenegen_log_det', 'hope_env_generate_pool', 'hope_env_curriculum_enable', 'hope_env_curriculum_disable', 'hope_env_set_pool_buckets', 'hope_env_curriculum_tally', 'hope_env_curriculum_update', 'hope_env_curriculum_state', 'hope_env_curriculum_set_windows', 'hope_env_curriculum_download_lists', 'hope_curriculum_lists_host', 'hope_curriculum_fold_host', 'hope_map_level_host', 'hope_map_level_device', 'hope_env_map_level', 'hope_env_num_scenes', 'hope_env_max_obstacles', 'hope_env_device_arch']
 
 
 CURRICULUM_LIST_LEN = 1 << 20
diff --git a/hope_amd/csrc/hope_env.hip b/hope_amd/csrc/hope_env.hip
--- a/hope_amd/csrc/hope_env.hip
+++ b/hope_amd/csrc/hope_env.hip
@@ -807,6 +807,11 @@
     hipError_t e = rs_fstat_read((unsigned long long*)out, reset);
     return e == hipSuccess ? HOPE_OK : fail(HOPE_EHIP, std::string("hope_debug_rs_filter_stats: ") + hipGetErrorString(e));
 }
+int hope_debug_rs_prescreen_stats(uint64_t* out, int reset) {
+    if (!out) return fail(HOPE_EINVAL, "hope_debug_rs_prescreen_stats: null argument");
+    hipError_t e = rs_prestat_read((unsigned long long*)out, reset);
+    return e == hipSuccess ? HOPE_OK : fail(HOPE_EHIP, std::string("hope_debug_rs_prescreen_stats: ") + hipGetErrorString(e));
+}
 
 int hope_debug_rs_filter_dump(double* out) {
     if (!out) return fail(HOPE_EINVAL, "hope_debug_rs_filter_dump: null argument");
@@ -1179,6 +1184,7 @@
         r.fverts = h->fverts; r.fbox = h->fbox; r.eflag = h->eflag;
         r.rs_count = counter; r.rs_list = qlist; r.rs_in = rs_in;
         r.rs_rec = h->rs_rec;
+        r.prescreen = 0;
         r.surv_count = h->rs_surv_count + i;
         r.surv_list = h->rs_surv + (size_t)c * h->n + ch.a;
         r.rs_word = out->rs_word; r.rs_lengths = out->rs_lengths;
diff --git a/hope_amd/csrc/hope_internal.h b/hope_amd/csrc/hope_internal.h
--- a/hope_amd/csrc/hope_internal.h
+++ b/hope_amd/csrc/hope_internal.h
@@ -55,6 +55,7 @@
     void* rs_lengths;
     int32_t* surv_count;
     int2* surv_list;
+    int prescreen;
 };
 
 constexpr int BEV_IMG = HOPE_IMG_SIZE;
@@ -91,6 +92,7 @@
 hipError_t rs_prof_read(unsigned long long* out , int reset);
 hipError_t rs_init_tables();
 hipError_t rs_fstat_read(unsigned long long* out , int reset);
+hipError_t rs_prestat_read(unsigned long long* out , int reset);
 hipError_t rs_fdump_read(double* out );
 hipError_t rs_log_read(int* out , int cap, int* n, int reset);
 size_t rs_lds_bytes(int max_obst);
diff --git a/hope_amd/csrc/hope_rs.hip b/hope_amd/csrc/hope_rs.hip
--- a/hope_amd/csrc/hope_rs.hip
+++ b/hope_amd/csrc/hope_rs.hip
@@ -424,10 +424,24 @@
     }
 }
 
+constexpr int PRE_PAIRS = 16, PRE_WORDS = 4;
+constexpr int PRE_SEG = 3;
+constexpr int PRE_PQ = 3 * WAVE;
+__device__ __forceinline__ void segs_prescreen(const RsParams& p, int lane, int entry, int qi, int n_test, double* rec, float fxmax, float fymax,
+                                               const double* psl, const float4* psrow, const int* pscode, float4* pspose, int* pspq, int* psdead);
+
 __global__ __launch_bounds__(64) void k_rs_segs(RsParams p) {
     set_wave_prio(p.prio_front);
-    __shared__ double keyl[8][RS_WORDS_PER_SCENE];
-    __shared__ double prl[8][RS_WORDS_PER_SCENE];
+    __shared__ __attribute__((aligned(16))) double heapl[2][8][RS_WORDS_PER_SCENE];
+    double (*keyl)[RS_WORDS_PER_SCENE] = heapl[0];
+    double (*prl)[RS_WORDS_PER_SCENE] = heapl[1];
+    static_assert(8 * PRE_WORDS * 5 * PRE_SEG + 2 * 2 * WAVE <= 2 * 8 * RS_WORDS_PER_SCENE, "pre-screen rows + poses fit the heap's words");
+    double* psl_all = &heapl[0][0][0];
+    float4* pspose = (float4*)(psl_all + 8 * PRE_WORDS * 5 * PRE_SEG);
+    __shared__ float4 psrow[8][PRE_WORDS][5];
+    __shared__ int pscode[8][PRE_WORDS];
+    __shared__ int psdead[8];
+    __shared__ int pspq[PRE_PQ];
     __shared__ unsigned char hidl[8][RS_WORDS_PER_SCENE];
     __shared__ unsigned char ordl[8][RS_WORDS_PER_SCENE];
     __shared__ int ntl[8];
@@ -498,6 +512,7 @@
             }
         }
         ntl[ls] = no;
+        psdead[ls] = 0;
         ((int2*)rec)[1] = make_int2(n_kept, no);
     }
     if (live) {
@@ -513,6 +528,9 @@
     double sq0, cq0;
     hm_sincos(q0w, &sq0, &cq0);
     const double fq0x = hdrl[ls][0] - hdrl[ls][3], fq0y = hdrl[ls][1] - hdrl[ls][5];
+    const float fxmax = (float)(hdrl[ls][4] - hdrl[ls][3]), fymax = (float)(hdrl[ls][6] - hdrl[ls][5]);
+    const bool pre = p.prescreen != 0;
+    const double step = RS_STEP * MAXC, inv_step = 1.0 / step;
     for (int k = k0; k < n_test; k += 8) {
         const double* W = rec + RS_REC_WORDS + 8 * (int)order[k];
         double len[5];
@@ -522,6 +540,24 @@
         const int code = __double2loint(w6), nseg = __double2hiint(w6);
         double* tb = rec + RS_REC_SEGS + RS_SEG_TABLE * k;
         double ox = 0, oy = 0, hy = 0;
+        const bool pre_w = pre && k < PRE_WORDS;
+        if (pre_w) pscode[ls][k] = code;
+        if (pre_w) {
+            double pu0 = step, pr_ = 0.0, plprev = 0.0, pc = 0.0;
+#pragma unroll
+            for (int i = 0; i < 5; i++) {
+                if (i < nseg) {
+                    const double l = len[i], al = fabs(l);
+                    if (i >= 1) pu0 = (plprev * l > 0) ? pr_ : -pr_;
+                    double* ps = psl_all + ((ls * PRE_WORDS + k) * 5 + i) * PRE_SEG;
+                    ps[0] = l; ps[1] = pu0; ps[2] = pc;
+                    const double n = fabs(pu0) > al ? 0.0 : floor((al - pu0) * inv_step) + 1.0;
+                    pr_ = pu0 + n * step - al;
+                    pc += al;
+                    plprev = l;
+                }
+            }
+        }
 #pragma unroll
         for (int i = 0; i < 5; i++) {
             if (i < nseg) {
@@ -537,6 +573,7 @@
                     const float fc = (float)(c_oy * cq0 - s_oy * sq0), fs = (float)(s_oy * cq0 + c_oy * sq0);
                     tb[RS_SEG_F32 + 2 * i] = __hiloint2double(__float_as_int(foy), __float_as_int(fox));
                     tb[RS_SEG_F32 + 2 * i + 1] = __hiloint2double(__float_as_int(fs), __float_as_int(fc));
+                    if (pre_w) psrow[ls][k][i] = make_float4(fox, foy, fc, fs);
                 }
                 if (m == TS) {
                     ox = ox + l / MAXC * c_oy;
@@ -557,6 +594,9 @@
             tb[2 * RS_SEGW + 7] = -sq0;
         }
     }
+    if (pre)
+        segs_prescreen(p, lane, entry, qi, n_test, rec, fxmax, fymax, psl_all + ls * PRE_WORDS * 5 * PRE_SEG, &psrow[ls][0][0], pscode[ls], pspose,
+                       pspq, psdead);
 }
 
 constexpr int RSB_SEG = 0, RSB_SEGW = RS_SEGW, RSB_QPD = RS_SEG_TABLE, RSB_QCAP = 256, RSB_BAD = RSB_QPD + RSB_QCAP;
@@ -751,7 +791,7 @@
 constexpr int RSB_TABF = RSB_BAD + 8, RSB_WORDS_F = RSB_TABF + RS_TAB;
 constexpr int RSF_OCC = 4;
 __device__ double g_rs_steps[RS_TAB];
-__device__ unsigned long long g_rs_fstat[16];
+__device__ unsigned long long g_rs_fstat[24];
 __device__ double g_rs_fdump[64 * 16];
 
 template <bool FULL>
@@ -891,17 +931,153 @@
     return hit;
 }
 
+__device__ __forceinline__ void segs_prescreen(const RsParams& p, int lane, int entry, int qi, int n_test, double* rec, float fxmax, float fymax,
+                                               const double* psl, const float4* psrow, const int* pscode, float4* pspose, int* pspq, int* psdead) {
+    const int ls = lane >> 3, k0 = lane & 7;
+    const int scene = rs_list_scene(entry), n_obst = rs_list_n_obst(entry);
+    const int words = min(n_test, PRE_WORDS);
+    const int per = words == 3 ? 5 : PRE_PAIRS / max(words, 1);
+    const int stride = SCREEN_SPAN / per;
+    const double step = RS_STEP * MAXC, inv_step = 1.0 / step;
+    lsync();
+    float lox[2], hix[2], loy[2], hiy[2];
+    bool act[2];
+    int wv[2];
+#pragma unroll
+    for (int e = 0; e < 2; e++) {
+        const int j = k0 + 8 * e;
+        const int w = words == 4 ? (j & 3) : (words == 3 ? j % 3 : (words == 2 ? (j & 1) : 0));
+        const int k = words == 4 ? (j >> 2) : (words == 3 ? j / 3 : (words == 2 ? (j >> 1) : j));
+        wv[e] = w;
+        const double a = (double)((k + 1) * stride) * step;
+        const double* T = psl + 5 * PRE_SEG * w;
+        const int codew = words > 0 ? pscode[w] : 0, nsegw = codew >> 12;
+        int si = -1;
+        double pdv = 0.0;
+#pragma unroll
+        for (int i = 0; i < 5; i++) {
+            if (i < nsegw && si < 0) {
+                const double l = T[PRE_SEG * i], u0 = T[PRE_SEG * i + 1], c = T[PRE_SEG * i + 2], al = fabs(l);
+                if (a < c + al) {
+                    double jj = ceil((a - c - u0) * inv_step);
+                    jj = jj < 0.0 ? 0.0 : jj;
+                    const double u = u0 + jj * step;
+                    si = (fabs(u0) <= al && u > SCREEN_EPS && u < al - SCREEN_EPS) ? i : 5;
+                    pdv = l > 0.0 ? u : -u;
+                }
+            }
+        }
+        act[e] = words > 0 && si >= 0 && si < 5;
+        float X = 0, Y = 0, hc = 1, hs = 0;
+        if (act[e]) {
+            const float lf = (float)pdv;
+            const float4 row = psrow[5 * w + si];
+            const int m = type_of(codew, si);
+            const float rev = lf * 0.15915494309189535f;
+            const float sl = m == TS ? 0.0f : __builtin_amdgcn_sinf(rev), cl = m == TS ? 1.0f : __builtin_amdgcn_cosf(rev);
+            const float sgn = m == TR ? -1.0f : 1.0f;
+            const float ldx = m == TS ? lf * F_INV_MAXC : sl * F_INV_MAXC;
+            const float ldy = sgn * (1.0f - cl) * F_INV_MAXC;
+            X = row.x + (row.z * ldx - row.w * ldy);
+            Y = row.y + (row.w * ldx + row.z * ldy);
+            const float ss = sgn * sl;
+            hc = row.z * cl - row.w * ss;
+            hs = row.w * cl + row.z * ss;
+        }
+        const bool oob = act[e] && (X < 0.0f - FEPS || X > fxmax + FEPS || Y < 0.0f - FEPS || Y > fymax + FEPS);
+        if (oob) { atomicOr(&psdead[ls], 1 << w); act[e] = false; }
+        const float cx = X + hc * F_MID, cy = Y + hs * F_MID;
+        const float ex = fabsf(hc) * F_HL + fabsf(hs) * F_HW + FEPS, ey = fabsf(hs) * F_HL + fabsf(hc) * F_HW + FEPS;
+        lox[e] = cx - ex; hix[e] = cx + ex; loy[e] = cy - ey; hiy[e] = cy + ey;
+        pspose[2 * lane + e] = make_float4(cx, cy, hc, hs);
+    }
+    const int wpack = wv[0] | (wv[1] << 4);
+    const float4* gfb = p.fbox + (size_t)scene * p.max_obst;
+    const unsigned long long lt = (1ull << lane) - 1;
+    auto classify = [&](int count) {
+        const bool has = lane < count;
+        const int pr = has ? pspq[lane] : 0;
+        const int src = pr >> 9, e = (pr >> 8) & 1, ro = pr & 0xff;
+        const int sscene = __shfl(scene, src), sw = (__shfl(wpack, src) >> (4 * e)) & 15;
+        if (has && !((psdead[src >> 3] >> sw) & 1)) {
+            const float4 ps = pspose[2 * src + e];
+            const float4* gfv = p.fverts + ((size_t)sscene * p.max_obst + ro) * 2;
+            const float4 v01 = gfv[0], v23 = gfv[1];
+            const int efl = (int)(p.eflag + (size_t)sscene * eflag_stride(p.max_obst))[ro];
+            if (screen_obstacle_hit(v01, v23, ps.x, ps.y, ps.z, ps.w, efl, fminf(fabsf(ps.z), fabsf(ps.w)) >= FETA_HULL))
+                atomicOr(&psdead[src >> 3], 1 << sw);
+        }
+    };
+    lsync();
+    int npq = 0;
+    for (int ob = 0; __any(ob < n_obst); ob += 4) {
+        float4 bb[4];
+#pragma unroll
+        for (int u = 0; u < 4; u++) bb[u] = ob + u < n_obst ? gfb[ob + u] : make_float4(INFINITY, -INFINITY, INFINITY, -INFINITY);
+        const int dead = psdead[ls];
+        const bool a0 = act[0] && !((dead >> wv[0]) & 1), a1 = act[1] && !((dead >> wv[1]) & 1);
+#pragma unroll
+        for (int u = 0; u < 4; u++) {
+            const bool n0 = a0 && !(bb[u].x > hix[0] || bb[u].y < lox[0] || bb[u].z > hiy[0] || bb[u].w < loy[0]);
+            const bool n1 = a1 && !(bb[u].x > hix[1] || bb[u].y < lox[1] || bb[u].z > hiy[1] || bb[u].w < loy[1]);
+            const unsigned long long m0 = __ballot(n0), m1 = __ballot(n1);
+            if (!(m0 | m1)) continue;
+            if (n0) pspq[npq + __popcll(m0 & lt)] = (lane << 9) | (ob + u);
+            npq += __popcll(m0);
+            if (n1) pspq[npq + __popcll(m1 & lt)] = (lane << 9) | 0x100 | (ob + u);
+            npq += __popcll(m1);
+            if (npq >= WAVE) {
+                lsync();
+                classify(WAVE);
+                const int rem = npq - WAVE;
+                int c0 = 0, c1 = 0;
+                if (lane < rem) c0 = pspq[WAVE + lane];
+                if (WAVE + lane < rem) c1 = pspq[2 * WAVE + lane];
+                lsync();
+                if (lane < rem) pspq[lane] = c0;
+                if (WAVE + lane < rem) pspq[WAVE + lane] = c1;
+                npq = rem;
+                if (npq >= WAVE) {
+                    lsync();
+                    classify(WAVE);
+                    const int rem2 = npq - WAVE;
+                    int c2 = 0;
+                    if (lane < rem2) c2 = pspq[WAVE + lane];
+                    lsync();
+                    if (lane < rem2) pspq[lane] = c2;
+                    npq = rem2;
+                }
+            }
+        }
+    }
+    if (npq > 0) { lsync(); classify(npq); }
+    lsync();
+    const int deadm = psdead[ls] & ((1 << words) - 1);
+    const bool head = k0 == 0;
+    const bool surv = head && n_test > 0 && !(n_test <= PRE_WORDS && deadm == (1 << n_test) - 1);
+    if (head) ((unsigned long long*)rec)[9] = (unsigned long long)deadm;
+    const unsigned long long sm = __ballot(surv);
+    if (sm) {
+        const int leader = __ffsll((long long)sm) - 1;
+        int base = 0;
+        if (lane == leader) base = atomicAdd(p.surv_count, __popcll(sm));
+        base = __shfl(base, leader);
+        if (surv) p.surv_list[base + __popcll(sm & lt)] = make_int2(qi, entry);
+    }
+}
+
 template <bool TIMING>
 __device__ __forceinline__ unsigned long long screen_words(int lane, int n_paths, int n_obst, const double* tables, double* qpd, int* pq, int* cand,
                                                            const float2* fv, const float4* fbox, const unsigned char* eflag, float fxmax,
-                                                           float fymax, unsigned long long* tsec) {
+                                                           float fymax, unsigned long long* tsec, unsigned long long pre = 0) {
     const float fxmin = 0.0f, fymin = 0.0f;
     const double step = RS_STEP * MAXC;
-    unsigned long long condemned = 0;
+    unsigned long long condemned = pre;
     RS_T0();
     const double inv_step = 1.0 / step;
     for (int w0 = 0; w0 < n_paths; w0 += 4) {
         const int nw = min(4, n_paths - w0);
+        if (((pre >> w0) & 15) == (unsigned long long)((1 << nw) - 1)) continue;
         if (w0 > 0)
             for (int t = lane; t < RS_SEG_TABLE * nw; t += WAVE) qpd[t] = tables[RS_SEG_TABLE * w0 + t];
         lsync();
@@ -971,7 +1147,7 @@
         }
         RS_T(15);
         const int all_w = (1 << nw) - 1;
-        int dead = 0;
+        int dead = (int)(pre >> w0) & all_w;
         for (int w = 0; w < nw; w++) dead |= __ballot(oob && wl_ == w) ? (1 << w) : 0;
         auto classify = [&](int count) {
             const bool has = lane < count;
@@ -1067,7 +1243,7 @@
     }
 }
 
-template <int OCC, bool TIMING, bool STATS, bool PRE = false>
+template <int OCC, bool TIMING, bool STATS, int PRE = 0>
 __global__ __launch_bounds__(64, OCC) void k_rs_validate_f(RsParams p, int obs_f64) {
     extern __shared__ __attribute__((aligned(16))) double lds[];
     const int lane = threadIdx.x;
@@ -1077,7 +1253,7 @@
     RS_T0();
     const int b_ = (int)blockIdx.x;
     int qidx, entry;
-    if (PRE) {
+    if (PRE && !STATS) {
         const int2 sv = p.surv_list[b_];
         if (b_ >= *p.surv_count) return;
         qidx = sv.x; entry = sv.y;
@@ -1121,7 +1297,7 @@
     (void)entry;
 #endif
     double tb = lane < RS_SEG_TABLE ? tables[lane] : 0.0;
-    if (!PRE) {
+    if (PRE != 1) {
         typedef __attribute__((address_space(3))) void* lds_ptr;
         const double2* t2 = (const double2*)tables;
         __builtin_amdgcn_global_load_lds((const void*)(t2 + lane), (lds_ptr)qpd, 16, 0, 0);
@@ -1158,21 +1334,24 @@
     unsigned long long st_pass = 0, st_hit = 0, st_exact = 0, st_unc = 0, st_bad_hit = 0, st_bad_clear = 0, st_samples = 0;
     unsigned long long st_why[5] = {};
     unsigned long long condemned = 0;
-    if (PRE) condemned = (unsigned long long)__double_as_longlong(readlane_d(r0, 9));
+    const unsigned long long pre_mask = PRE == 2 ? (unsigned long long)__double_as_longlong(readlane_d(r0, 9)) : 0ull;
+    if (PRE == 1) condemned = (unsigned long long)__double_as_longlong(readlane_d(r0, 9));
     else if (!(obs_f64 & 0x20000)) {
         asm volatile("s_waitcnt vmcnt(0)" ::: "memory");
         tile_pending = false;
         condemned = screen_words<TIMING>(lane, n_paths, n_obst, tables, qpd, (int*)tabl ,
-                                         cand, fv, fbox, eflag, fxmax, fymax, tsec);
+                                         cand, fv, fbox, eflag, fxmax, fymax, tsec, pre_mask);
         if (TIMING) t0_ = __builtin_readcyclecounter();
     }
     else {
         asm volatile("s_waitcnt vmcnt(0)" ::: "memory");
         tile_pending = false;
+        condemned = pre_mask;
     }
     const bool verify_screen = STATS && paranoid;
     const bool all_condemned = condemned == ((1ull << n_paths) - 1);
     unsigned long long st_scr_words = __popcll(condemned), st_scr_dead = all_condemned ? 1 : 0, st_scr_bad = 0;
+    unsigned long long st_pre_bad = 0;
     if (!all_condemned || verify_screen) {
         const double T0 = g_rs_steps[lane], T1 = g_rs_steps[WAVE + lane], T2 = g_rs_steps[2 * WAVE + lane], T3 = g_rs_steps[3 * WAVE + lane];
         tabl[lane] = T0; tabl[WAVE + lane] = T1; tabl[2 * WAVE + lane] = T2; tabl[3 * WAVE + lane] = T3;
@@ -1451,7 +1630,7 @@
             }
             lsync();
         }
-        if (STATS && screened && !invalid) { st_scr_bad += 1; continue; }
+        if (STATS && screened && !invalid) { st_scr_bad += 1; st_pre_bad += (pre_mask >> (idx - 1)) & 1; continue; }
         if (!invalid) { found = idx - 1; break; }
     }
     if (STATS && lane == 0) {
@@ -1460,6 +1639,13 @@
         atomicAdd(&g_rs_fstat[0], st_pass); atomicAdd(&g_rs_fstat[1], st_hit); atomicAdd(&g_rs_fstat[2], st_exact);
         atomicAdd(&g_rs_fstat[3], st_unc); atomicAdd(&g_rs_fstat[4], st_bad_hit); atomicAdd(&g_rs_fstat[5], st_bad_clear);
         atomicAdd(&g_rs_fstat[6], st_samples);
+        if (PRE == 2) {
+            const bool pre_all = n_paths <= PRE_WORDS && pre_mask == ((1ull << n_paths) - 1);
+            atomicAdd(&g_rs_fstat[16], 1ull); atomicAdd(&g_rs_fstat[17], (unsigned long long)__popcll(pre_mask));
+            atomicAdd(&g_rs_fstat[18], pre_all ? 1ull : 0ull); atomicAdd(&g_rs_fstat[19], st_pre_bad);
+            atomicAdd(&g_rs_fstat[20], found >= 0 ? 1ull : 0ull);
+            if (paranoid) atomicAdd(&g_rs_fstat[21], (unsigned long long)__popcll(pre_mask));
+        }
     }
     if (TIMING) {
         tsec[6] = __builtin_readcyclecounter() - tstart_;
@@ -1536,6 +1722,17 @@
     if (e == hipSuccess && reset) {
         unsigned long long z[16] = {};
         e = hipMemcpyToSymbol(HIP_SYMBOL(g_rs_fstat), z, sizeof(z));
+    }
+    return e;
+}
+
+hipError_t rs_prestat_read(unsigned long long* out , int reset) {
+    hipError_t e = hipDeviceSynchronize();
+    if (e != hipSuccess) return e;
+    e = hipMemcpyFromSymbol(out, HIP_SYMBOL(g_rs_fstat), 8 * sizeof(unsigned long long), 16 * sizeof(unsigned long long));
+    if (e == hipSuccess && reset) {
+        unsigned long long z[8] = {};
+        e = hipMemcpyToSymbol(HIP_SYMBOL(g_rs_fstat), z, sizeof(z), 16 * sizeof(unsigned long long));
     }
     return e;
 }
@@ -1558,8 +1755,9 @@
 constexpr int RS_LARGE_TILE_WPC = 6;
 constexpr int RS_PRIO_MIN_SCENES = 32768;
 
-hipError_t launch_rs_search(const RsParams& p, hipStream_t stream, LaunchTimer* timer) {
-    if (p.max_queue <= 0) return hipSuccess;
+hipError_t launch_rs_search(const RsParams& p_in, hipStream_t stream, LaunchTimer* timer) {
+    if (p_in.max_queue <= 0) return hipSuccess;
+    RsParams p = p_in;
     static const bool timing = getenv("HOPE_RS_TIMING") != nullptr;
     const bool exact = getenv("HOPE_RS_EXACT") != nullptr;
     const int dbg = getenv("HOPE_RS_DEBUG") ? (int)strtol(getenv("HOPE_RS_DEBUG"), nullptr, 0) : 0;
@@ -1567,7 +1765,9 @@
     size_t lds = exact ? rs_lds_bytes_exact(p.tile_cap) : rs_lds_bytes_filter(p.tile_cap);
     if (!exact && p.tile_cap > 32) lds = std::max(lds, (size_t)((158 * 1024 / RS_LARGE_TILE_WPC) & ~255));
     if (lds > 48 * 1024) {
-        hipError_t e = hipFuncSetAttribute((const void*)k_rs_validate_f<RSF_OCC, false, false, true>, hipFuncAttributeMaxDynamicSharedMemorySize, (int)lds);
+        hipError_t e = hipFuncSetAttribute((const void*)k_rs_validate_f<RSF_OCC, false, false, 1>, hipFuncAttributeMaxDynamicSharedMemorySize, (int)lds);
+        if (e == hipSuccess) e = hipFuncSetAttribute((const void*)k_rs_validate_f<RSF_OCC, false, false, 2>, hipFuncAttributeMaxDynamicSharedMemorySize, (int)lds);
+        if (e == hipSuccess) e = hipFuncSetAttribute((const void*)k_rs_validate_f<RSF_OCC, false, true, 2>, hipFuncAttributeMaxDynamicSharedMemorySize, (int)lds);
         if (e != hipSuccess) return e;
     }
     const void* vk = exact ? (timing ? (const void*)k_rs_validate<3, true> : (const void*)k_rs_validate<3, false>)
@@ -1581,11 +1781,13 @@
     if (timer) timer->begin(HOPE_K_RS_WORDS, stream);
     hipLaunchKernelGGL(k_rs_words, dim3((p.max_queue + RSA_SCENES - 1) / RSA_SCENES, RSA_GROUPS), dim3(WAVE), 0, stream, p);
     if (timer) timer->end(stream);
+    const bool split = !exact && !timing && !stats && !(dbg & 0x20000) && p.surv_count && p.surv_list &&
+                       getenv("HOPE_RS_SPLIT") && atoi(getenv("HOPE_RS_SPLIT")) == 1;
+    const bool pre = !exact && !timing && !split && !(dbg & 0x40000) && p.surv_count && p.surv_list;
+    p.prescreen = pre ? 1 : 0;
     if (timer) timer->begin(HOPE_K_RS_SEGS, stream);
     hipLaunchKernelGGL(k_rs_segs, dim3((p.max_queue + 7) / 8), dim3(WAVE), 0, stream, p);
     if (timer) timer->end(stream);
-    const bool split = !exact && !timing && !stats && !(dbg & 0x20000) && p.surv_count && p.surv_list &&
-                       getenv("HOPE_RS_SPLIT") && atoi(getenv("HOPE_RS_SPLIT")) == 1;
     if (split) {
         if (timer) timer->begin(HOPE_K_RS_SCREEN, stream);
         hipLaunchKernelGGL((k_rs_screen<false, 8>), dim3(p.max_queue), dim3(WAVE), rs_screen_lds_bytes(p.tile_cap), stream, p);
@@ -1597,7 +1799,9 @@
     if (exact) {
         if (timing) hipLaunchKernelGGL((k_rs_validate<3, true>), dim3(p.max_queue), dim3(WAVE), lds, stream, p, flags);
         else hipLaunchKernelGGL((k_rs_validate<3, false>), dim3(p.max_queue), dim3(WAVE), lds, stream, p, flags);
-    } else if (split) hipLaunchKernelGGL((k_rs_validate_f<RSF_OCC, false, false, true>), dim3(p.max_queue), dim3(WAVE), lds, stream, p, flags);
+    } else if (split) hipLaunchKernelGGL((k_rs_validate_f<RSF_OCC, false, false, 1>), dim3(p.max_queue), dim3(WAVE), lds, stream, p, flags);
+    else if (pre && stats) hipLaunchKernelGGL((k_rs_validate_f<RSF_OCC, false, true, 2>), dim3(p.max_queue), dim3(WAVE), lds, stream, p, flags);
+    else if (pre) hipLaunchKernelGGL((k_rs_validate_f<RSF_OCC, false, false, 2>), dim3(p.max_queue), dim3(WAVE), lds, stream, p, flags);
     else if (timing) hipLaunchKernelGGL((k_rs_validate_f<RSF_OCC, true, false>), dim3(p.max_queue), dim3(WAVE), lds, stream, p, flags);
     else if (stats) hipLaunchKernelGGL((k_rs_validate_f<RSF_OCC, false, true>), dim3(p.max_queue), dim3(WAVE), lds, stream, p, flags);
     else hipLaunchKernelGGL((k_rs_validate_f<RSF_OCC, false, false>), dim3(p.max_queue), dim3(WAVE), lds, stream, p, flags);
diff --git a/include/hope_env.h b/include/hope_env.h
--- a/include/hope_env.h
+++ b/include/hope_env.h
@@ -148,6 +148,7 @@
 
 int hope_debug_rs_prof(uint64_t *out , int reset);
 int hope_debug_rs_filter_stats(uint64_t *out , int reset);
+int hope_debug_rs_prescreen_stats(uint64_t *out , int reset);
 int hope_debug_rs_filter_dump(double *out );
 int hope_debug_rs_log(int32_t *out , int cap, int32_t *n, int reset);
 int hope_debug_step_prof(uint64_t *out , int reset);
```

After: 144.4 million. -10.8%, worse.
